# iDC-NEU/NeutronStarLite

Hardware: NVIDIA H100
Metric: gcn_aggregated_edges_per_sec (higher is better)
Workload: dtype f32

## Files before the change

include/nts_b200.h:

```cpp
#ifndef NTS_B200_H
#define NTS_B200_H

#include <stddef.h>
#include <stdint.h>

#ifdef __cplusplus
extern "C" {
#endif

typedef uint32_t nts_vid_t;

int nts_version(void);
const char *nts_last_error(void);
int nts_device_count(void);
int nts_set_device(int device);
int nts_device_sm_count(int *sm_count);
int nts_device_synchronize(void);
int nts_device_reset(void);

void *nts_malloc_device(size_t bytes);
int nts_free_device(void *ptr);
void *nts_malloc_pinned(size_t bytes);
int nts_free_pinned(void *ptr);
void *nts_pinned_device_pointer(void *host_ptr);
int nts_memcpy_h2d(void *dst_device, const void *src_host, size_t bytes, void *stream, int sync);
int nts_memcpy_d2h(void *dst_host, const void *src_device, size_t bytes, void *stream, int sync);
int nts_memcpy_d2d(void *dst_device, const void *src_device, size_t bytes, void *stream);
int nts_zero(void *device_ptr, size_t bytes, void *stream);

void *nts_stream_create(int non_blocking);
int nts_stream_destroy(void *stream);
int nts_stream_synchronize(void *stream);
void *nts_event_create(int with_timing);
int nts_event_destroy(void *event);
int nts_event_record(void *event, void *stream);
int nts_stream_wait_event(void *stream, void *event);
int nts_event_elapsed_ms(void *start, void *stop, float *ms);

int nts_segment_gather_sum(const float *input, float *output, const float *weight,
                           const nts_vid_t *indices, const nts_vid_t *offsets, nts_vid_t index_base,
                           nts_vid_t n_rows, uint64_t n_edges, nts_vid_t feature_size, void *stream);

int nts_gather_by_dst_from_src(const float *input, float *output, const float *weight_forward,
                               const nts_vid_t *row_indices, const nts_vid_t *column_offset,
                               nts_vid_t src_start, nts_vid_t src_end, nts_vid_t dst_start,
                               nts_vid_t dst_end, nts_vid_t edges, nts_vid_t batch_size,
                               nts_vid_t feature_size, int with_weight, void *stream);

int nts_gather_by_src_from_dst(const float *input, float *output, const float *weight_backward,
                               const nts_vid_t *row_offset, const nts_vid_t *column_indices,
                               nts_vid_t src_start, nts_vid_t src_end, nts_vid_t dst_start,
                               nts_vid_t dst_end, nts_vid_t edges, nts_vid_t batch_size,
                               nts_vid_t feature_size, int with_weight, void *stream);

int nts_segment_gather_sum_range(const float *input, float *output, const float *weight, const nts_vid_t *indices,
                                 const nts_vid_t *offsets, const nts_vid_t *slot_of, nts_vid_t index_base,
                                 nts_vid_t n_rows, uint64_t edge_begin, uint64_t edge_end, nts_vid_t feature_size,
                                 void *stream);

typedef struct nts_gather_plan nts_gather_plan;
int nts_gather_plan_pick_slabs(nts_vid_t gather_rows, uint64_t n_edges, nts_vid_t n_rows, nts_vid_t feature_size,
                               uint64_t l2_budget_bytes );
nts_gather_plan *nts_gather_plan_create_hybrid(const nts_vid_t *offsets, const nts_vid_t *indices,
                                               const float *weight, const nts_vid_t *slot_of, nts_vid_t index_base,
                                               nts_vid_t n_rows, uint64_t n_edges, nts_vid_t gather_rows, int n_slabs,
                                               int n_hub_cols, int n_hub_rows, void *stream);
nts_gather_plan *nts_gather_plan_create_tuned_ex(const nts_vid_t *offsets, const nts_vid_t *indices,
                                                 const float *weight, const nts_vid_t *slot_of, nts_vid_t index_base,
                                                 nts_vid_t n_rows, uint64_t n_edges, nts_vid_t gather_rows,
                                                 nts_vid_t feature_size, int gather_dtype, int run_flags,
                                                 void *stream);
typedef struct nts_plan_part {
  const nts_vid_t *offsets, *indices;
  const float *weight;
  const nts_vid_t *slot_of;
  nts_vid_t index_base, index_add, n_rows, row_add;
  uint64_t n_edges;
} nts_plan_part;
nts_gather_plan *nts_gather_plan_create_parts(const nts_plan_part *parts, int n_parts, nts_vid_t n_rows,
                                              nts_vid_t gather_rows, int n_slabs, nts_vid_t feature_size, void *stream);
float nts_gather_plan_tuned_ms(const nts_gather_plan *plan);
int nts_gather_plan_destroy(nts_gather_plan *plan);
int nts_gather_plan_slabs(const nts_gather_plan *plan);
int nts_gather_plan_hubs(const nts_gather_plan *plan, int *cols, int *rows);
int nts_gather_plan_overlap(const nts_gather_plan *plan);
int nts_gather_plan_set_overlap(nts_gather_plan *plan, int overlap);
uint64_t nts_gather_plan_bytes(const nts_gather_plan *plan);
enum { NTS_PLAN_ACCUMULATE = 0, NTS_PLAN_OVERWRITE = 1, NTS_PLAN_COPY_INPUT = 2 };
int nts_gather_plan_run_ex(nts_gather_plan *plan, const float *input, nts_vid_t input_ld, float *output,
                           nts_vid_t feature_size, int flags, void *stream);
int nts_gather_plan_last_launch(const nts_gather_plan *plan, int *launches, int *grid, int *k, int *u, int *outv);
enum { NTS_DTYPE_F32 = 0, NTS_DTYPE_BF16 = 1 };
int nts_gather_plan_run_bf16_ex(nts_gather_plan *plan, const void *input, int input_dtype, nts_vid_t input_ld,
                                float *output, nts_vid_t feature_size, int flags, void *stream);
int nts_gather_plan_set_tuning(int u, int min_blocks, int edges_per_warp);
int nts_gather_plan_set_variant(int variant);

int nts_segment_gather_sum_slots(const float *input, float *output, const float *weight,
                                 const nts_vid_t *indices, const nts_vid_t *offsets,
                                 const nts_vid_t *slot_of, nts_vid_t n_rows, uint64_t n_edges,
                                 nts_vid_t feature_size, void *stream);

int nts_segment_gather_sum_heads(const float *input, float *output, const float *weight,
                                 const nts_vid_t *indices, const nts_vid_t *offsets, const nts_vid_t *slot_of,
                                 nts_vid_t index_base, nts_vid_t n_rows, uint64_t n_edges,
                                 nts_vid_t feature_size, nts_vid_t heads, void *stream);

int nts_aggregate_set_variant(int variant, int edges_per_warp);
int nts_aggregate_last_launch(int *grid, int *block, int *smem_bytes, int *variant);
int nts_aggregate_last_shape(int *vec, int *k, int *u, int *min_blocks, int *tiles);
uint64_t nts_kernel_launch_count(void);

int nts_scatter_src_mirror_to_msg(float *message, const float *src_mirror_feature,
                                  const nts_vid_t *row_indices, const nts_vid_t *column_offset,
                                  const nts_vid_t *mirror_index, nts_vid_t batch_size,
                                  nts_vid_t feature_size, void *stream);
int nts_gather_msg_to_src_mirror(float *src_mirror_feature, const float *message,
                                 const nts_vid_t *row_indices, const nts_vid_t *column_offset,
                                 const nts_vid_t *mirror_index, nts_vid_t batch_size,
                                 nts_vid_t feature_size, void *stream);
int nts_scatter_dst_to_msg(float *message, const float *dst_feature, const nts_vid_t *row_indices,
                           const nts_vid_t *column_offset, nts_vid_t batch_size,
                           nts_vid_t feature_size, void *stream);
int nts_gather_msg_to_dst(float *dst_feature, const float *message, const nts_vid_t *row_indices,
                          const nts_vid_t *column_offset, nts_vid_t batch_size,
                          nts_vid_t feature_size, void *stream);
int nts_edge_softmax_forward(float *msg_output, const float *msg_input, float *msg_cached,
                             const nts_vid_t *row_indices, const nts_vid_t *column_offset,
                             nts_vid_t batch_size, nts_vid_t feature_size, void *stream);
int nts_edge_softmax_backward(float *msg_input_grad, const float *msg_output_grad,
                              const float *msg_cached, const nts_vid_t *row_indices,
                              const nts_vid_t *column_offset, nts_vid_t batch_size,
                              nts_vid_t feature_size, void *stream);
int nts_scatter_grad_back_to_message(const float *input, float *message_grad,
                                     const nts_vid_t *row_indices, const nts_vid_t *column_offset,
                                     nts_vid_t batch_size, nts_vid_t feature_size, void *stream);

int nts_aggregate_dst_fuse_weight_backward(float *mirror_grad, float *edge_weight_grad,
                                           const float *mirror, const float *edge_weight,
                                           const float *dst_grad, const nts_vid_t *row_indices,
                                           const nts_vid_t *column_offset,
                                           const nts_vid_t *mirror_index, nts_vid_t batch_size,
                                           nts_vid_t feature_size, void *stream);
int nts_aggregate_dst_fuse_weight_backward_heads(float *mirror_grad, float *edge_weight_grad,
                                                 const float *mirror, const float *edge_weight,
                                                 const float *dst_grad, const nts_vid_t *row_indices,
                                                 const nts_vid_t *column_offset,
                                                 const nts_vid_t *mirror_index, nts_vid_t batch_size,
                                                 nts_vid_t feature_size, nts_vid_t heads, void *stream);

int nts_gat_softmax_stats(float *seg_max, float *seg_sum, const float *src_score, const float *dst_score,
                          const nts_vid_t *row_indices, const nts_vid_t *column_offset,
                          const nts_vid_t *mirror_index, nts_vid_t batch_size, nts_vid_t heads,
                          float negative_slope, void *stream);
int nts_gat_fused_aggregate_forward(const float *mirror, float *output, const float *src_score,
                                    const float *dst_score, const float *seg_max, const float *seg_sum,
                                    const nts_vid_t *row_indices, const nts_vid_t *column_offset,
                                    const nts_vid_t *mirror_index, nts_vid_t batch_size, uint64_t n_edges,
                                    nts_vid_t feature_size, nts_vid_t heads, float negative_slope, void *stream);
int nts_gat_fused_aggregate_backward(float *mirror_grad, float *src_score_grad, float *dst_score_grad,
                                     const float *mirror, const float *src_score, const float *dst_score,
                                     const float *seg_max, const float *seg_sum, const float *out_dot_grad,
                                     const float *dst_grad, const nts_vid_t *row_indices,
                                     const nts_vid_t *column_offset, const nts_vid_t *mirror_index,
                                     nts_vid_t batch_size, nts_vid_t feature_size, nts_vid_t heads,
                                     float negative_slope, void *stream);
int nts_gat_fused_aggregate_backward_two_pass(float *mirror_grad, float *src_score_grad, float *dst_score_grad,
                                              float *dst_pack, const float *mirror, const float *src_score,
                                              const float *dst_score, const float *seg_max, const float *seg_sum,
                                              const float *out_dot_grad, const float *dst_grad,
                                              const nts_vid_t *row_indices, const nts_vid_t *column_offset,
                                              const nts_vid_t *mirror_index, const nts_vid_t *slot_row_offset,
                                              const nts_vid_t *slot_column_indices, nts_vid_t batch_size,
                                              nts_vid_t mirror_size, nts_vid_t feature_size, nts_vid_t heads,
                                              float negative_slope, void *stream);
int nts_gat_fused_aggregate_forward_bf16(const void *mirror, float *output, const float *src_score,
                                         const float *dst_score, const float *seg_max, const float *seg_sum,
                                         const nts_vid_t *row_indices, const nts_vid_t *column_offset,
                                         const nts_vid_t *mirror_index, nts_vid_t batch_size, uint64_t n_edges,
                                         nts_vid_t feature_size, nts_vid_t ld, nts_vid_t heads, float negative_slope,
                                         void *stream);
int nts_gat_fused_aggregate_backward_two_pass_bf16(float *mirror_grad, float *src_score_grad, float *dst_score_grad,
                                                   float *dst_pack, const void *mirror, const float *src_score,
                                                   const float *dst_score, const float *seg_max, const float *seg_sum,
                                                   const float *out_dot_grad, const void *dst_grad,
                                                   const nts_vid_t *row_indices, const nts_vid_t *column_offset,
                                                   const nts_vid_t *mirror_index, const nts_vid_t *slot_row_offset,
                                                   const nts_vid_t *slot_column_indices, nts_vid_t batch_size,
                                                   nts_vid_t mirror_size, nts_vid_t feature_size, nts_vid_t ld,
                                                   nts_vid_t heads, float negative_slope, void *stream);
int nts_rows_to_bf16(const void *src, int src_dtype, nts_vid_t lds, void *dst, nts_vid_t n_rows, nts_vid_t feature_size,
                     nts_vid_t ld, void *stream);

int nts_deserialize_records(float *mirror, const float *records, nts_vid_t n_records,
                            nts_vid_t feature_size, nts_vid_t partition_start,
                            nts_vid_t partition_end, void *stream);
int nts_aggregate_records(float *aggregate, const float *records, nts_vid_t n_records,
                          nts_vid_t feature_size, nts_vid_t partition_start,
                          nts_vid_t partition_end, void *stream);

int nts_gather_rows(float *dst, const float *src, const nts_vid_t *rows, nts_vid_t n_rows,
                    nts_vid_t feature_size, void *stream);
int nts_scatter_add_rows(float *dst, const float *src, const nts_vid_t *rows, nts_vid_t n_rows,
                         nts_vid_t feature_size, void *stream);
int nts_scatter_add_rows_atomic(float *dst, const float *src, const nts_vid_t *rows, nts_vid_t n_rows,
                                nts_vid_t feature_size, void *stream);

int nts_adam_update(float *W, float *M, float *V, const float *grad, uint64_t n, float weight_decay, float beta1,
                    float beta2, float alpha, float epsilon, void *stream);

#define NTS_IPC_HANDLE_BYTES 64
int nts_ipc_get_handle(void *device_ptr, unsigned char handle[NTS_IPC_HANDLE_BYTES]);
void *nts_ipc_open_handle(const unsigned char handle[NTS_IPC_HANDLE_BYTES]);
int nts_ipc_close_handle(void *peer_ptr);
int nts_signal_set(uint32_t *flag, uint32_t value, void *stream);
int nts_signal_wait_geq(const uint32_t *flag, uint32_t value, void *stream);

typedef struct nts_exchange nts_exchange;
typedef struct nts_exchange_chunk {
  const nts_vid_t *column_offset;
  const nts_vid_t *slots;
  const float *weight_forward;
  const nts_vid_t *row_offset_compact;
  const nts_vid_t *column_indices;
  const float *weight_backward;
  uint64_t edges;
} nts_exchange_chunk;
typedef struct nts_exchange_desc {
  int partitions, rank;
  nts_vid_t owned_vertices, dst_start;
  const nts_vid_t *local_column_offset, *local_row_indices, *local_row_offset, *local_column_indices;
  const float *local_weight_forward, *local_weight_backward;
  nts_vid_t local_edges;
  const nts_exchange_chunk *chunks;
  const nts_vid_t *need_count;
  const nts_vid_t *send_count;
  const nts_vid_t *send_rows_all;
  const nts_vid_t *fwd_push_offset;
  const nts_vid_t *bwd_push_offset;
  const nts_vid_t *local_need;
  nts_vid_t local_need_count;
} nts_exchange_desc;

nts_exchange *nts_exchange_create(const nts_exchange_desc *desc);
int nts_exchange_destroy(nts_exchange *ex);
uint64_t nts_exchange_required_floats(const nts_exchange *ex, nts_vid_t feature_size);
uint64_t nts_exchange_required_floats_bf16(const nts_exchange *ex, nts_vid_t feature_size);
// ... 132 lines not shown
```

neutronstarlite_b200/_lib.py:

```python
from __future__ import annotations

import ctypes as C
import os
import re

PKG = os.path.dirname(os.path.abspath(__file__))
ROOT = os.path.dirname(PKG)
LIB_PATH = os.path.join(PKG, "lib", "libnts_b200.so")
HEADER = os.path.join(ROOT, "include", "nts_b200.h")

_vp = C.c_void_p
_u32 = C.c_uint32
_u64 = C.c_uint64
_int = C.c_int
_sz = C.c_size_t

SIGNATURES = {
    "nts_version": (_int, []),
    "nts_last_error": (C.c_char_p, []),
    "nts_device_count": (_int, []),
    "nts_set_device": (_int, [_int]),
    "nts_device_sm_count": (_int, [C.POINTER(_int)]),
    "nts_device_synchronize": (_int, []),
    "nts_device_reset": (_int, []),
    "nts_malloc_device": (_vp, [_sz]),
    "nts_free_device": (_int, [_vp]),
    "nts_malloc_pinned": (_vp, [_sz]),
    "nts_free_pinned": (_int, [_vp]),
    "nts_pinned_device_pointer": (_vp, [_vp]),
    "nts_memcpy_h2d": (_int, [_vp, _vp, _sz, _vp, _int]),
    "nts_memcpy_d2h": (_int, [_vp, _vp, _sz, _vp, _int]),
    "nts_memcpy_d2d": (_int, [_vp, _vp, _sz, _vp]),
    "nts_zero": (_int, [_vp, _sz, _vp]),
    "nts_stream_create": (_vp, [_int]),
    "nts_stream_destroy": (_int, [_vp]),
    "nts_stream_synchronize": (_int, [_vp]),
    "nts_event_create": (_vp, [_int]),
    "nts_event_destroy": (_int, [_vp]),
    "nts_event_record": (_int, [_vp, _vp]),
    "nts_stream_wait_event": (_int, [_vp, _vp]),
    "nts_event_elapsed_ms": (_int, [_vp, _vp, C.POINTER(C.c_float)]),
    "nts_segment_gather_sum": (_int, [_vp, _vp, _vp, _vp, _vp, _u32, _u32, _u64, _u32, _vp]),
    "nts_gather_by_dst_from_src": (_int, [_vp, _vp, _vp, _vp, _vp, _u32, _u32, _u32, _u32, _u32, _u32, _u32, _int, _vp]),
    "nts_gather_by_src_from_dst": (_int, [_vp, _vp, _vp, _vp, _vp, _u32, _u32, _u32, _u32, _u32, _u32, _u32, _int, _vp]),
    "nts_segment_gather_sum_range": (_int, [_vp, _vp, _vp, _vp, _vp, _vp, _u32, _u32, _u64, _u64, _u32, _vp]),
    "nts_gather_plan_pick_slabs": (_int, [_u32, _u64, _u32, _u32, _u64]),
    "nts_gather_plan_create_hybrid": (_vp, [_vp, _vp, _vp, _vp, _u32, _u32, _u64, _u32, _int, _int, _int, _vp]),
    "nts_gather_plan_create_parts": (_vp, [_vp, _int, _u32, _u32, _int, _u32, _vp]),
    "nts_gather_plan_tuned_ms": (C.c_float, [_vp]),
    "nts_gather_plan_destroy": (_int, [_vp]),
    "nts_gather_plan_slabs": (_int, [_vp]),
    "nts_gather_plan_hubs": (_int, [_vp, C.POINTER(_int), C.POINTER(_int)]),
    "nts_gather_plan_overlap": (_int, [_vp]),
    "nts_gather_plan_set_overlap": (_int, [_vp, _int]),
    "nts_gather_plan_bytes": (_u64, [_vp]),
    "nts_gather_plan_run_ex": (_int, [_vp, _vp, _u32, _vp, _u32, _int, _vp]),
    "nts_gather_plan_run_bf16_ex": (_int, [_vp, _vp, _int, _u32, _vp, _u32, _int, _vp]),
    "nts_gather_plan_create_tuned_ex": (_vp, [_vp, _vp, _vp, _vp, _u32, _u32, _u64, _u32, _u32, _int, _int, _vp]),
    "nts_gather_plan_last_launch": (_int, [_vp] + [C.POINTER(_int)] * 5),
    "nts_gather_plan_set_tuning": (_int, [_int, _int, _int]),
    "nts_gather_plan_set_variant": (_int, [_int]),
    "nts_segment_gather_sum_slots": (_int, [_vp, _vp, _vp, _vp, _vp, _vp, _u32, _u64, _u32, _vp]),
    "nts_segment_gather_sum_heads": (_int, [_vp, _vp, _vp, _vp, _vp, _vp, _u32, _u32, _u64, _u32, _u32, _vp]),
    "nts_aggregate_set_variant": (_int, [_int, _int]),
    "nts_aggregate_last_launch": (_int, [C.POINTER(_int)] * 4),
    "nts_aggregate_last_shape": (_int, [C.POINTER(_int)] * 5),
    "nts_kernel_launch_count": (_u64, []),
    "nts_scatter_src_mirror_to_msg": (_int, [_vp, _vp, _vp, _vp, _vp, _u32, _u32, _vp]),
    "nts_gather_msg_to_src_mirror": (_int, [_vp, _vp, _vp, _vp, _vp, _u32, _u32, _vp]),
    "nts_scatter_dst_to_msg": (_int, [_vp, _vp, _vp, _vp, _u32, _u32, _vp]),
    "nts_gather_msg_to_dst": (_int, [_vp, _vp, _vp, _vp, _u32, _u32, _vp]),
    "nts_edge_softmax_forward": (_int, [_vp, _vp, _vp, _vp, _vp, _u32, _u32, _vp]),
    "nts_edge_softmax_backward": (_int, [_vp, _vp, _vp, _vp, _vp, _u32, _u32, _vp]),
    "nts_scatter_grad_back_to_message": (_int, [_vp, _vp, _vp, _vp, _u32, _u32, _vp]),
    "nts_aggregate_dst_fuse_weight_backward": (_int, [_vp, _vp, _vp, _vp, _vp, _vp, _vp, _vp, _u32, _u32, _vp]),
    "nts_aggregate_dst_fuse_weight_backward_heads": (_int, [_vp] * 8 + [_u32, _u32, _u32, _vp]),
    "nts_gat_softmax_stats": (_int, [_vp] * 7 + [_u32, _u32, C.c_float, _vp]),
    "nts_gat_fused_aggregate_forward": (_int, [_vp] * 9 + [_u32, _u64, _u32, _u32, C.c_float, _vp]),
    "nts_gat_fused_aggregate_backward": (_int, [_vp] * 13 + [_u32, _u32, _u32, C.c_float, _vp]),
    "nts_gat_fused_aggregate_backward_two_pass": (_int, [_vp] * 16 + [_u32, _u32, _u32, _u32, C.c_float, _vp]),
    "nts_gat_fused_aggregate_forward_bf16": (_int, [_vp] * 9 + [_u32, _u64, _u32, _u32, _u32, C.c_float, _vp]),
    "nts_gat_fused_aggregate_backward_two_pass_bf16": (_int, [_vp] * 16 + [_u32] * 5 + [C.c_float, _vp]),
    "nts_rows_to_bf16": (_int, [_vp, _int, _u32, _vp, _u32, _u32, _u32, _vp]),
    "nts_deserialize_records": (_int, [_vp, _vp, _u32, _u32, _u32, _u32, _vp]),
    "nts_aggregate_records": (_int, [_vp, _vp, _u32, _u32, _u32, _u32, _vp]),
    "nts_gather_rows": (_int, [_vp, _vp, _vp, _u32, _u32, _vp]),
    "nts_scatter_add_rows": (_int, [_vp, _vp, _vp, _u32, _u32, _vp]),
    "nts_scatter_add_rows_atomic": (_int, [_vp, _vp, _vp, _u32, _u32, _vp]),
    "nts_ipc_get_handle": (_int, [_vp, C.c_char_p]),
    "nts_ipc_open_handle": (_vp, [C.c_char_p]),
    "nts_ipc_close_handle": (_int, [_vp]),
    "nts_adam_update": (_int, [_vp, _vp, _vp, _vp, _u64] + [C.c_float] * 5 + [_vp]),
    "nts_signal_set": (_int, [_vp, _u32, _vp]),
    "nts_signal_wait_geq": (_int, [_vp, _u32, _vp]),
    "nts_host_degrees": (_int, [_vp, _u64, _u32, _vp, _vp]),
    "nts_host_partition_offsets": (_int, [_vp, _u64, _u32, _int, _vp]),
    "nts_host_chunk_edge_counts": (_int, [_vp, _u64, _vp, _int, _int, _vp]),
    "nts_host_build_chunk": (_int, [_vp, _u64, _u32, _vp, _int, _int, _int, _vp, _vp, _vp, _vp, _vp, _vp, _vp, _vp, _vp]),
    "nts_host_mirror_index": (_int, [_vp, _u64, _u32, _vp, _int, _vp, _vp]),
    "nts_host_read_feature_label_mask": (_int, [C.c_char_p, C.c_char_p, C.c_char_p, _u32, _u32, _u32, _vp, _vp, _vp]),
    "nts_host_read_feature_binary": (_int, [C.c_char_p, _u32, _u32, _u32, _vp]),
    "nts_graph_build_from_file": (_vp, [C.c_char_p, _u32, _int, _int, _vp, _u64, _int, _vp]),
    "nts_graph_build_from_device": (_vp, [_vp, _vp, _int, _u64, _u32, _int, _int, _vp, _vp, _vp, _int, _vp]),
    "nts_graph_build_info": (_int, [_vp] * 6),
    "nts_graph_build_export_chunk": (_int, [_vp, _int] + [_vp] * 8),
    "nts_graph_build_export_dist": (_int, [_vp] * 5),
    "nts_graph_build_export_degrees": (_int, [_vp] * 4),
    "nts_graph_build_destroy": (_int, [_vp]),
}



class ExchangeChunk(C.Structure):
    _fields_ = [
        ("column_offset", _vp), ("slots", _vp), ("weight_forward", _vp), ("row_offset_compact", _vp),
        ("column_indices", _vp), ("weight_backward", _vp), ("edges", _u64),
    ]


class ExchangeDesc(C.Structure):
    _fields_ = [
        ("partitions", _int), ("rank", _int), ("owned_vertices", _u32), ("dst_start", _u32),
        ("local_column_offset", _vp), ("local_row_indices", _vp), ("local_row_offset", _vp),
        ("local_column_indices", _vp), ("local_weight_forward", _vp), ("local_weight_backward", _vp),
        ("local_edges", _u32),
        ("chunks", C.POINTER(ExchangeChunk)),
        ("need_count", C.POINTER(_u32)), ("send_count", C.POINTER(_u32)),
        ("send_rows_all", _vp), ("fwd_push_offset", C.POINTER(_u32)), ("bwd_push_offset", C.POINTER(_u32)),
        ("local_need", _vp), ("local_need_count", _u32),
    ]


class DeviceChunk(C.Structure):
    _fields_ = [
        ("column_offset", _vp), ("row_indices", _vp), ("row_offset", _vp), ("column_indices", _vp),
        ("edge_weight_forward", _vp), ("edge_weight_backward", _vp),
    ]


SIGNATURES.update({
    "nts_exchange_create": (_vp, [C.POINTER(ExchangeDesc)]),
    "nts_exchange_destroy": (_int, [_vp]),
    "nts_exchange_required_floats": (_u64, [_vp, _u32]),
    "nts_exchange_capacity_floats": (_u64, [_vp]),
    "nts_exchange_release_peers": (_int, [_vp]),
    "nts_exchange_reserve": (_int, [_vp, _u64, _int]),
    "nts_exchange_handles": (_int, [_vp, C.c_char_p, C.c_char_p]),
    "nts_exchange_open_peers": (_int, [_vp, C.c_char_p, C.c_char_p]),
    "nts_exchange_forward": (_int, [_vp, _vp, _vp, _u32, _vp]),
    "nts_exchange_backward": (_int, [_vp, _vp, _vp, _u32, _vp]),
    "nts_exchange_forward_bf16": (_int, [_vp, _vp, _int, _vp, _u32, _vp]),
    "nts_exchange_backward_bf16": (_int, [_vp, _vp, _vp, _u32, _vp]),
    "nts_exchange_required_floats_bf16": (_u64, [_vp, _u32]),
    "nts_exchange_set_trace": (_int, [_vp, _int]),
    "nts_exchange_last_timeline": (_int, [_vp, C.POINTER(C.c_float), _int]),
    "nts_exchange_fetch_mirrors": (_int, [_vp, _vp, _vp, _u32, _vp]),
    "nts_exchange_return_mirror_grads": (_int, [_vp, _vp, _vp, _u32, _vp]),
})



class HostChunk(C.Structure):
    _fields_ = [
        ("column_offset", _vp), ("row_indices", _vp), ("row_offset", _vp), ("column_indices", _vp),
        ("edge_weight_forward", _vp), ("edge_weight_backward", _vp),
        ("src_start", _u32), ("src_end", _u32), ("dst_start", _u32), ("dst_end", _u32), ("edges", _u64),
    ]


class ExchangePlanView(C.Structure):
    _fields_ = [
        ("partitions", _int), ("rank", _int),
        ("owned_vertices", _u32), ("recv_total", _u32), ("send_total", _u32), ("backward_rows", _u32),
        ("remote_edges", _u64),
        ("need_count", C.POINTER(_u32)), ("send_count", C.POINTER(_u32)), ("peer_bwd_offset", C.POINTER(_u32)),
        ("fwd_push_offset", C.POINTER(_u32)), ("bwd_push_offset", C.POINTER(_u32)),
        ("remote_column_offset", C.POINTER(_u32)), ("remote_slots", C.POINTER(_u32)),
        ("remote_weight", C.POINTER(C.c_float)),
        ("backward_offsets", C.POINTER(_u32)), ("backward_indices", C.POINTER(_u32)),
        ("backward_weight", C.POINTER(C.c_float)),
        ("send_rows_all", C.POINTER(_u32)),
    ]


SIGNATURES.update({
    "nts_exchange_plan_create": (_vp, [C.POINTER(HostChunk), _int, _int]),
    "nts_exchange_plan_destroy": (None, [_vp]),
    "nts_exchange_plan_need": (C.POINTER(_u32), [_vp, _int, C.POINTER(_u32)]),
    "nts_exchange_plan_packed_rows": (_u64, [_vp]),
    "nts_exchange_plan_pack_needs": (_int, [_vp, _vp, _vp]),
    "nts_exchange_plan_set_peer_needs": (_int, [_vp, _int, _vp, _vp]),
    "nts_exchange_plan_finalize": (_int, [_vp]),
    "nts_exchange_plan_get_view": (_int, [_vp, C.POINTER(ExchangePlanView)]),
    "nts_exchange_plan_chunk": (_int, [_vp, _int, C.POINTER(C.POINTER(_u32)), C.POINTER(C.POINTER(_u32))]),
    "nts_exchange_create_from_plan": (_vp, [_vp, C.POINTER(DeviceChunk)]),
})


class SampleHopView(C.Structure):
    _fields_ = [
        ("n_dst", _u32), ("n_src", _u32), ("n_edges", _u64),
        ("dst", _vp), ("column_offset", _vp), ("row_indices", _vp), ("row_global", _vp), ("weight", _vp),
        ("src", _vp), ("row_offset", _vp), ("column_indices", _vp), ("weight_backward", _vp),
    ]


SIGNATURES.update({
    "nts_sampler_create": (_vp, [_vp, _vp, _vp, _u32, _u64, _u32, _int, C.POINTER(_int), _vp]),
    "nts_sampler_create_ex": (_vp, [_vp, _vp, _vp, _u32, _u64, _u32, _int, C.POINTER(_int), _u32, _vp]),
    "nts_sampler_sample": (_int, [_vp, _vp, _u32, _u64, _u64, _vp]),
# ... 46 lines not shown
```

neutronstarlite_b200/csrc/nts_common.cuh:

```cuda
#pragma once
#include <cuda_bf16.h>
#include <cuda_runtime.h>
#include <stdint.h>
#include <stdio.h>
#include <stdlib.h>
#include <string.h>

#include <functional>

#include "nts_b200.h"

namespace nts {

char *last_error_buffer();
bool abort_on_error();
void count_launch();

inline int fail(int code, const char *what, const char *file, int line) {
  snprintf(last_error_buffer(), 512, "%s (%s:%d)", what, file, line);
  if (abort_on_error()) {
    fprintf(stderr, "libnts_b200: %s\n", last_error_buffer());
    exit(1);
  }
  return code;
}

#define NTS_CUDA_OK(expr)                                                                         \
  do {                                                                                            \
    cudaError_t nts_e_ = (expr);                                                                  \
    if (nts_e_ != cudaSuccess)                                                                    \
      return ::nts::fail((int)nts_e_, cudaGetErrorString(nts_e_), __FILE__, __LINE__);            \
  } while (0)

#define NTS_ARG_CHECK(cond, msg)                                                                  \
  do {                                                                                            \
    if (!(cond))                                                                                  \
      return ::nts::fail(-1, msg, __FILE__, __LINE__);                                            \
  } while (0)

#define NTS_LAUNCH_CHECK()                                                                        \
  do {                                                                                            \
    ::nts::count_launch();                                                                        \
    NTS_CUDA_OK(cudaGetLastError());                                                              \
  } while (0)

inline cudaStream_t as_stream(void *s) { return reinterpret_cast<cudaStream_t>(s); }

inline bool aligned_to(const void *p, size_t a) { return (reinterpret_cast<uintptr_t>(p) & (a - 1)) == 0; }

int sm_count();

int time_min_of_two(const std::function<int()> &run, cudaStream_t st, float *ms);

int run_plan(nts_gather_plan *pl, const float *input, uint32_t lds, float *output, uint32_t F, int flags,
             cudaStream_t st);
int run_plan_bf16(nts_gather_plan *pl, const void *input, int dtype, uint32_t lds, float *output, uint32_t F,
                  cudaStream_t st, int flags = 0);
int to_bf16_rows(const void *src, int dtype, uint32_t lds, void *dst, uint32_t n_rows, uint32_t F, uint32_t ld,
                 cudaStream_t st);

int check_gat_bf16_layout(uint32_t F, uint32_t ld, uint32_t heads);

struct __align__(16) float8v {
  float4 lo, hi;
};

template <int VEC> struct Vec;
template <> struct Vec<1> { using type = float; };
template <> struct Vec<2> { using type = float2; };
template <> struct Vec<4> { using type = float4; };
template <> struct Vec<8> { using type = float8v; };

template <class T, int VEC> struct Ld { using type = typename Vec<VEC>::type; };
template <> struct Ld<__nv_bfloat16, 2> { using type = uint32_t; };
template <> struct Ld<__nv_bfloat16, 4> { using type = uint2; };
template <> struct Ld<__nv_bfloat16, 8> { using type = uint4; };
__device__ __forceinline__ float widen(float v) { return v; }
__device__ __forceinline__ float2 widen(float2 v) { return v; }
__device__ __forceinline__ float4 widen(float4 v) { return v; }
__device__ __forceinline__ float2 widen(uint32_t u) {
  return make_float2(__uint_as_float(u << 16), __uint_as_float(u & 0xffff0000u));
}
__device__ __forceinline__ float4 widen(uint2 u) {
  const float2 a = widen(u.x), b = widen(u.y);
  return make_float4(a.x, a.y, b.x, b.y);
}
__device__ __forceinline__ float8v widen(uint4 u) { return {widen(make_uint2(u.x, u.y)), widen(make_uint2(u.z, u.w))}; }

nts_gather_plan *tune_plan(const nts_plan_part *parts, int n_parts, nts_vid_t n_rows, nts_vid_t gather_rows,
                           nts_vid_t feature_size, bool bf16, int run_flags, bool hubs_allowed, cudaStream_t st);

}
```

neutronstarlite_b200/csrc/nts_exchange.cu:

```cuda
#include <algorithm>
#include <vector>

#include "nts_common.cuh"

namespace nts {
constexpr int kMaxPeers = 32;

struct PushTarget {
  const uint32_t *rows;
  uint32_t n_rows, src_row0;
  float *dst;
  uint32_t *pushed_flag;
  const uint32_t *consumed_flag;
};
struct PushArgs {
  PushTarget t[kMaxPeers];
  int n;
  uint32_t epoch, wait_epoch;
};
}

struct nts_exchange {
  int P = 1, p = 0;
  nts_exchange_desc d;
// ... 173 lines not shown

#define NTS_TRY(expr)                                                                                               \
  do {                                                                                                              \
    int nts_rc_ = (expr);                                                                                           \
    if (nts_rc_ != 0)                                                                                               \
      return nts_rc_;                                                                                               \
  } while (0)

static int grow(float **buf, size_t *cap, size_t floats) {
  if (floats <= *cap)
    return 0;
  if (*buf)
    NTS_CUDA_OK(cudaFree(*buf));
  *buf = nullptr;
  NTS_CUDA_OK(cudaMalloc(reinterpret_cast<void **>(buf), floats * sizeof(float)));
  *cap = floats;
  return 0;
}

static int check_wait_error(nts_exchange *ex, int rc) {
  if (ex->err_host && ex->err_host[0]) {
    char msg[256];
    snprintf(msg, sizeof(msg),
             "exchange wait timed out on rank %d: %s %d (wanted epoch %d, saw %d) - a peer died, failed or fell out of step",
             ex->p, ex->err_host[0] == 1 ? "no rows pushed by partition" : "window not consumed by push target",
             ex->err_host[1], ex->err_host[2], ex->err_host[3]);
    return fail(rc ? rc : -1, msg, __FILE__, __LINE__);
  }
  return rc;
}

static int launch_push(nts_exchange *ex, const PushArgs &a, const float *src, uint32_t F, cudaStream_t st) {
  int vec = 1;
  bool a16 = aligned_to(src, 16), a8 = aligned_to(src, 8);
  for (int k = 0; k < a.n; k++) {
    a16 = a16 && aligned_to(a.t[k].dst, 16);
    a8 = a8 && aligned_to(a.t[k].dst, 8);
  }
  if (F % 4 == 0 && a16)
    vec = 4;
  else if (F % 2 == 0 && a8)
    vec = 2;
  const int ctas = ex->push_ctas;
  if (vec == 4)
    push_rows_kernel<4><<<ctas, 256, 0, st>>>(a, src, F, ex->tickets, ex->timeout_ns, ex->err_dev);
  else if (vec == 2)
    push_rows_kernel<2><<<ctas, 256, 0, st>>>(a, src, F, ex->tickets, ex->timeout_ns, ex->err_dev);
  else
    push_rows_kernel<1><<<ctas, 256, 0, st>>>(a, src, F, ex->tickets, ex->timeout_ns, ex->err_dev);
  NTS_LAUNCH_CHECK();
  return 0;
}

static int dma_push(nts_exchange *ex, int j, const float *src, size_t dst_row, uint32_t n_rows, uint32_t F, size_t buf,
                    uint32_t epoch, uint32_t wait_epoch, cudaStream_t from) {
  cudaStream_t st = ex->dma[j];
  NTS_CUDA_OK(cudaEventRecord(ex->ev_dma[j], from));
  NTS_CUDA_OK(cudaStreamWaitEvent(st, ex->ev_dma[j], 0));
  ex->dma_used[j] = 1;
  if (n_rows) {
    if (wait_epoch) {
      wait_consumed_kernel<<<1, 1, 0, st>>>(ex->flags + ex->P + j, wait_epoch, ex->timeout_ns, ex->err_dev, j);
      NTS_LAUNCH_CHECK();
    }
    NTS_CUDA_OK(cudaMemcpyAsync(ex->peer_window[j] + buf + dst_row * F, src, (size_t)n_rows * F * sizeof(float),
                                cudaMemcpyDeviceToDevice, st));
  }
  signal_pushed_kernel<<<1, 1, 0, st>>>(ex->peer_flags[j] + ex->p, epoch);
  NTS_LAUNCH_CHECK();
  return 0;
}

static int dma_join(nts_exchange *ex, cudaStream_t into) {
  for (int j = 0; j < ex->P; j++)
    if (ex->dma_used[j]) {
      NTS_CUDA_OK(cudaEventRecord(ex->ev_dma[j], ex->dma[j]));
      NTS_CUDA_OK(cudaStreamWaitEvent(into, ex->ev_dma[j], 0));
      ex->dma_used[j] = 0;
    }
  return 0;
}

static int push_my_rows(nts_exchange *ex, const float *x, uint32_t F, size_t buf, uint32_t epoch, uint32_t wait_epoch) {
  const int P = ex->P, p = ex->p;
  PushArgs a;
  a.n = 0;
  a.epoch = epoch;
  a.wait_epoch = wait_epoch;
  for (int s = 1; s < P; s++) {
    const int j = (p - s + P) % P;
    if (ex->send_all[j]) {
      if (a.n) {
        NTS_TRY(launch_push(ex, a, x, F, ex->comm));
        a.n = 0;
      }
      NTS_TRY(dma_push(ex, j, x, ex->fwd_push_off[j], ex->send_count[j], F, buf, epoch, wait_epoch, ex->comm));
      continue;
    }
    PushTarget &t = a.t[a.n++];
    t.rows = ex->d.send_rows_all + ex->srecv_offs[j];
    t.n_rows = ex->send_count[j];
    t.src_row0 = 0;
    t.dst = ex->peer_window[j] + buf + (size_t)ex->fwd_push_off[j] * F;
    t.pushed_flag = ex->peer_flags[j] + p;
    t.consumed_flag = ex->flags + P + j;
  }
  if (a.n)
    NTS_TRY(launch_push(ex, a, x, F, ex->comm));
  return 0;
}

struct GatherType {
  bool bf16;
  uint32_t ld;
};
static int plan_key(uint32_t F, bool bf16) { return bf16 ? -(int)F : (int)F; }

static int aggregate_chunk(nts_exchange *ex, int i, bool forward, const void *in_rows, float *out, uint32_t F,
                           cudaStream_t st, GatherType gt = {false, 0}) {
  const float *in = static_cast<const float *>(in_rows);
  const nts_exchange_chunk &c = ex->chunks[i];
  const bool local = i == ex->p;
  const uint32_t n_rows = (forward || local) ? ex->d.owned_vertices : ex->need_count[i];
  const uint32_t gather_rows = (forward && !local) ? ex->need_count[i] : ex->d.owned_vertices;
  if (!c.edges || !n_rows)
    return 0;
  const nts_vid_t *off = forward ? c.column_offset : c.row_offset_compact;
  const nts_vid_t *idx = forward ? c.slots : c.column_indices;
  const float *w = forward ? c.weight_forward : c.weight_backward;
  const uint32_t base = (forward && !local) ? 0u : ex->d.dst_start;
  if (c.edges >= ex->plan_min_edges || gt.bf16) {
    std::vector<std::pair<int, nts_gather_plan *>> &plans = (forward ? ex->plan_fwd : ex->plan_bwd)[i];
    nts_gather_plan *pl = nullptr;
    for (auto &e : plans)
      if (e.first == plan_key(F, gt.bf16))
        pl = e.second;
    if (!pl) {
      const nts_plan_part pt = {off, idx, w, nullptr, base, 0, n_rows, 0, c.edges};
      pl = tune_plan(&pt, 1, n_rows, gather_rows, F, gt.bf16, 0, true, st);
      if (!pl)
        return -1;
      int hc = 0, hr = 0, ehc = 0, ehr = 0;
      nts_gather_plan_hubs(pl, &hc, &hr);
      for (auto &e : plans)
        if (nts_gather_plan_slabs(e.second) == nts_gather_plan_slabs(pl) &&
            nts_gather_plan_hubs(e.second, &ehc, &ehr) == 0 && ehc == hc && ehr == hr) {
          nts_gather_plan_destroy(pl);
          pl = e.second;
          break;
        }
      plans.emplace_back(plan_key(F, gt.bf16), pl);
    }
    if (gt.bf16)
      return run_plan_bf16(pl, in_rows, NTS_DTYPE_BF16, gt.ld, out, F, st);
    return run_plan(pl, in, F, out, F, 0, st);
  }
  return nts_segment_gather_sum(in, out, w, idx, off, base, n_rows, c.edges, F, st);
}

static int decide_mode(nts_exchange *ex, bool forward, uint32_t F, cudaStream_t st, nts_exchange::Mode **out,
                       GatherType gt = {false, 0}) {
  std::vector<nts_exchange::Mode> &modes = forward ? ex->mode_fwd : ex->mode_bwd;
  for (auto &m : modes)
    if (m.F == (int)F && m.bf16 == gt.bf16) {
      *out = &m;
      return 0;
    }
  modes.push_back({(int)F, 1, gt.bf16, nullptr, 0.f, 0.f});
  nts_exchange::Mode &m = modes.back();
  *out = &m;
  const int P = ex->P, p = ex->p;
  const uint32_t Vp = ex->d.owned_vertices;
  uint64_t remote_edges = 0;
  int n_remote = 0;
  for (int i = 0; i < P; i++)
    if (i != p && ex->chunks[i].edges && ex->need_count[i]) {
      remote_edges += ex->chunks[i].edges;
      n_remote++;
    }
  if (ex->forced_mode == 1 || n_remote < 2 || !Vp || !ex->recv_total)
    return 0;
  std::vector<nts_plan_part> parts;
  for (int i = 0; i < P; i++) {
    if (i == p || !ex->chunks[i].edges || !ex->need_count[i])
      continue;
    const nts_exchange_chunk &c = ex->chunks[i];
    nts_plan_part pt = {};
    if (forward) {
      pt.offsets = c.column_offset, pt.indices = c.slots, pt.weight = c.weight_forward;
      pt.index_base = 0, pt.index_add = ex->recv_offs[i], pt.n_rows = Vp, pt.row_add = 0;
    } else {
      pt.offsets = c.row_offset_compact, pt.indices = c.column_indices, pt.weight = c.weight_backward;
      pt.index_base = ex->d.dst_start, pt.index_add = 0, pt.n_rows = ex->need_count[i], pt.row_add = ex->recv_offs[i];
    }
    pt.n_edges = c.edges;
    parts.push_back(pt);
  }
  const uint32_t out_rows = forward ? Vp : ex->recv_total, in_rows = forward ? ex->recv_total : Vp;
  m.merged = tune_plan(parts.data(), (int)parts.size(), out_rows, in_rows, F, gt.bf16, 0, false, st);
  if (!m.merged)
    return -1;
  if (ex->forced_mode == 2) {
    m.mode = 2;
    return 0;
  }
  const size_t rows_max = std::max<size_t>(ex->recv_total, Vp);
  const size_t a_bytes = rows_max * std::max<size_t>((size_t)F * sizeof(float), gt.bf16 ? (size_t)gt.ld * 2 : 0);
  float *a = nullptr, *b = nullptr;
  NTS_CUDA_OK(cudaMalloc(reinterpret_cast<void **>(&a), a_bytes));
  if (cudaMalloc(reinterpret_cast<void **>(&b), rows_max * F * sizeof(float)) != cudaSuccess) {
    cudaFree(a);
    return fail(-1, "scratch allocation for the exchange mode measurement failed", __FILE__, __LINE__);
  }
  cudaMemsetAsync(a, 0, a_bytes, st);
  cudaMemsetAsync(b, 0, rows_max * F * sizeof(float), st);
  float L = 0.f, M = 0.f, sum_c = 0.f;
  int rc = time_min_of_two([&]() { return aggregate_chunk(ex, p, forward, a, b, F, st, gt); }, st, &L);
  if (!rc)
    rc = time_min_of_two([&]() {
      return gt.bf16 ? run_plan_bf16(m.merged, a, NTS_DTYPE_BF16, gt.ld, b, F, st) : run_plan(m.merged, a, F, b, F, 0, st);
    }, st, &M);
  for (int i = 0; i < P && !rc; i++) {
    if (i == p || !ex->chunks[i].edges || !ex->need_count[i])
      continue;
    float c = 0.f;
    rc = time_min_of_two([&]() { return aggregate_chunk(ex, i, forward, a, b, F, st, gt); }, st, &c);
    sum_c += c;
  }
  cudaFree(a);
  cudaFree(b);
  if (rc)
    return rc;
  if (!ex->chunks[p].edges)
    L = 0.f;
  const double row_bytes = (forward && gt.bf16) ? gt.ld * 2.0 : F * 4.0;
  const float T = (float)((double)ex->recv_total * row_bytes / 300e9 * 1e3);
  if (forward) {
    m.pipeline_ms = L + std::max(sum_c, T - L);
    m.merged_ms = std::max(L, T) + M;
  } else {
    m.pipeline_ms = sum_c + std::max(L, T / (float)(P - 1));
    m.merged_ms = M + std::max(L, T);
  }
  m.mode = m.merged_ms < m.pipeline_ms ? 2 : 1;
  if (m.mode == 1) {
    nts_gather_plan_destroy(m.merged);
    m.merged = nullptr;
  }
  return 0;
}

extern "C" {

nts_exchange *nts_exchange_create(const nts_exchange_desc *desc) {
  if (!desc || desc->partitions < 1 || desc->partitions > kMaxPeers || desc->rank < 0 ||
      desc->rank >= desc->partitions) {
    fail(-1, "bad exchange descriptor (1 <= partitions <= 32)", __FILE__, __LINE__);
    return nullptr;
  }
  nts_exchange *ex = new nts_exchange();
  ex->d = *desc;
  const int P = ex->P = desc->partitions, p = ex->p = desc->rank;
  if (P > 1 && !(desc->chunks && desc->need_count && desc->send_count && desc->fwd_push_offset &&
                 desc->bwd_push_offset)) {
    fail(-1, "exchange descriptor lacks the per-partition arrays", __FILE__, __LINE__);
    delete ex;
    return nullptr;
  }
  ex->need_count.assign(P, 0), ex->send_count.assign(P, 0), ex->fwd_push_off.assign(P, 0), ex->bwd_push_off.assign(P, 0);
  ex->chunks.assign(P, nts_exchange_chunk{});
  for (int i = 0; i < P && P > 1; i++) {
    if (i == p)
      continue;
    ex->need_count[i] = desc->need_count[i];
    ex->send_count[i] = desc->send_count[i];
    ex->fwd_push_off[i] = desc->fwd_push_offset[i];
    ex->bwd_push_off[i] = desc->bwd_push_offset[i];
    ex->chunks[i] = desc->chunks[i];
  }
  {
    nts_exchange_chunk &c = ex->chunks[p];
    c.column_offset = desc->local_column_offset;
    c.slots = desc->local_row_indices;
    c.weight_forward = desc->local_weight_forward;
    c.row_offset_compact = desc->local_row_offset;
    c.column_indices = desc->local_column_indices;
    c.weight_backward = desc->local_weight_backward;
    c.edges = desc->local_edges;
  }
  ex->recv_offs.assign(P + 1, 0), ex->srecv_offs.assign(P + 1, 0);
  for (int i = 0; i < P; i++) {
    ex->recv_offs[i + 1] = ex->recv_offs[i] + ex->need_count[i];
    ex->srecv_offs[i + 1] = ex->srecv_offs[i] + ex->send_count[i];
  }
  ex->recv_total = ex->recv_offs[P];
  ex->send_total = ex->srecv_offs[P];
  ex->send_all.assign(P, 0);
  if (P > 1 && ex->send_total && desc->send_rows_all && !getenv("NTS_EXCHANGE_NO_DMA")) {
    std::vector<uint32_t> rows(ex->send_total);
    if (cudaMemcpy(rows.data(), desc->send_rows_all, rows.size() * sizeof(uint32_t), cudaMemcpyDeviceToHost) == cudaSuccess)
      for (int j = 0; j < P; j++) {
        if (j == p || ex->send_count[j] != desc->owned_vertices || !desc->owned_vertices)
          continue;
        bool ident = true;
        const uint32_t *r = rows.data() + ex->srecv_offs[j];
        for (uint32_t k = 0; k < ex->send_count[j] && ident; k++)
          ident = r[k] == k;
        ex->send_all[j] = ident;
      }
  }
  ex->peer_window.assign(P, nullptr);
  ex->peer_flags.assign(P, nullptr);
  ex->plan_fwd.resize(P), ex->plan_bwd.resize(P);
  ex->ev_peer.assign(P, nullptr);
  if (const char *t = getenv("NTS_EXCHANGE_TIMEOUT_MS")) {
    const long ms = atol(t);
    if (ms > 0)
      ex->timeout_ns = (unsigned long long)ms * 1000000ull;
  }
  if (const char *t = getenv("NTS_EXCHANGE_MODE"))
    ex->forced_mode = !strcmp(t, "pipeline") ? 1 : (!strcmp(t, "merged") ? 2 : 0);
  if (const char *t = getenv("NTS_EXCHANGE_PLAN_MIN_EDGES"))
    ex->plan_min_edges = strtoull(t, nullptr, 10);
  ex->push_ctas = std::max(8, sm_count() / 2);
  if (const char *t = getenv("NTS_EXCHANGE_PUSH_CTAS")) {
    const int n = atoi(t);
    if (n > 0)
      ex->push_ctas = n;
  }
  int lo = 0, hi = 0;
  bool ok = cudaDeviceGetStreamPriorityRange(&lo, &hi) == cudaSuccess &&
            cudaMalloc(reinterpret_cast<void **>(&ex->flags), sizeof(uint32_t) * 2 * P) == cudaSuccess &&
            cudaMemset(ex->flags, 0, sizeof(uint32_t) * 2 * P) == cudaSuccess &&
            cudaMalloc(reinterpret_cast<void **>(&ex->tickets), sizeof(uint32_t) * kMaxPeers) == cudaSuccess &&
            cudaMemset(ex->tickets, 0, sizeof(uint32_t) * kMaxPeers) == cudaSuccess &&
            cudaMalloc(reinterpret_cast<void **>(&ex->d_peer_flags), sizeof(uint32_t *) * P) == cudaSuccess &&
            cudaHostAlloc(reinterpret_cast<void **>(&ex->err_host), 4 * sizeof(int), cudaHostAllocMapped) == cudaSuccess &&
            cudaHostGetDevicePointer(reinterpret_cast<void **>(&ex->err_dev), ex->err_host, 0) == cudaSuccess &&
            cudaStreamCreateWithPriority(&ex->comm, cudaStreamNonBlocking, hi) == cudaSuccess &&
            cudaEventCreateWithFlags(&ex->ev_main, cudaEventDisableTiming) == cudaSuccess &&
            cudaEventCreateWithFlags(&ex->ev_comm, cudaEventDisableTiming) == cudaSuccess;
  for (int i = 0; i < P && ok; i++)
    ok = cudaEventCreateWithFlags(&ex->ev_peer[i], cudaEventDisableTiming) == cudaSuccess;
  ex->dma.assign(P, nullptr), ex->ev_dma.assign(P, nullptr), ex->dma_used.assign(P, 0);
  for (int i = 0; i < P && ok && P > 1; i++)
    ok = cudaStreamCreateWithPriority(&ex->dma[i], cudaStreamNonBlocking, hi) == cudaSuccess &&
         cudaEventCreateWithFlags(&ex->ev_dma[i], cudaEventDisableTiming) == cudaSuccess;
  if (ok) {
    memset(ex->err_host, 0, 4 * sizeof(int));
    ok = cudaDeviceSynchronize() == cudaSuccess;
  }
  if (!ok) {
    fail(-1, "exchange resource allocation failed", __FILE__, __LINE__);
    delete ex;
    return nullptr;
  }
  return ex;
}

int nts_exchange_release_peers(nts_exchange *ex) {
  NTS_ARG_CHECK(ex != nullptr, "null engine");
  NTS_CUDA_OK(cudaDeviceSynchronize());
  if (ex->peers_open) {
    for (int j = 0; j < ex->P; j++)
      if (j != ex->p) {
        NTS_CUDA_OK(cudaIpcCloseMemHandle(ex->peer_window[j]));
        NTS_CUDA_OK(cudaIpcCloseMemHandle(ex->peer_flags[j]));
      }
    ex->peers_open = false;
  }
  return 0;
}

// ... 32 lines not shown
  if (ex->ev_main)
    cudaEventDestroy(ex->ev_main);
  if (ex->ev_comm)
    cudaEventDestroy(ex->ev_comm);
  for (cudaEvent_t e : ex->ev_peer)
    if (e)
      cudaEventDestroy(e);
  for (cudaEvent_t e : ex->tev)
    if (e)
      cudaEventDestroy(e);
  for (cudaStream_t q : ex->dma)
    if (q)
      cudaStreamDestroy(q);
  for (cudaEvent_t e : ex->ev_dma)
    if (e)
      cudaEventDestroy(e);
  delete ex;
  return 0;
}

uint64_t nts_exchange_required_floats(const nts_exchange *ex, nts_vid_t feature_size) {
  uint64_t rows = std::max(ex->recv_total, ex->send_total);
  if (rows == 0)
    rows = 1;
  return rows * (uint64_t)feature_size;
}

uint64_t nts_exchange_required_floats_bf16(const nts_exchange *ex, nts_vid_t feature_size) {
  const uint64_t row16 = ((feature_size + 7ull) / 8ull) * 4ull;
  return std::max<uint64_t>(std::max<uint64_t>(ex->recv_total, 1) * row16, nts_exchange_required_floats(ex, feature_size));
}

uint64_t nts_exchange_capacity_floats(const nts_exchange *ex) { return ex ? ex->buf_floats : 0; }

int nts_exchange_reserve(nts_exchange *ex, uint64_t floats_per_buffer, int n_buffers) {
  NTS_ARG_CHECK(ex && (n_buffers == 1 || n_buffers == 2), "bad argument (n_buffers must be 1 or 2)");
  NTS_ARG_CHECK(!ex->peers_open, "nts_exchange_release_peers (and a barrier) must precede nts_exchange_reserve");
  NTS_CUDA_OK(cudaDeviceSynchronize());
  if (ex->window)
    NTS_CUDA_OK(cudaFree(ex->window));
  ex->window = nullptr;
  ex->buf_floats = 0;
  NTS_CUDA_OK(cudaMalloc(reinterpret_cast<void **>(&ex->window), floats_per_buffer * n_buffers * sizeof(float)));
  ex->buf_floats = floats_per_buffer;
  ex->n_buffers = n_buffers;
  return 0;
}

int nts_exchange_handles(nts_exchange *ex, unsigned char window_handle[NTS_IPC_HANDLE_BYTES],
                         unsigned char flags_handle[NTS_IPC_HANDLE_BYTES]) {
  NTS_ARG_CHECK(ex && ex->window && ex->flags, "window not allocated");
  cudaIpcMemHandle_t h;
  NTS_CUDA_OK(cudaIpcGetMemHandle(&h, ex->window));
  memcpy(window_handle, &h, sizeof(h));
  NTS_CUDA_OK(cudaIpcGetMemHandle(&h, ex->flags));
  memcpy(flags_handle, &h, sizeof(h));
  return 0;
}

int nts_exchange_open_peers(nts_exchange *ex, const unsigned char *window_handles, const unsigned char *flag_handles) {
  NTS_ARG_CHECK(ex && window_handles && flag_handles, "null argument");
  NTS_ARG_CHECK(!ex->peers_open, "peers already open");
  const int P = ex->P, p = ex->p;
  for (int j = 0; j < P; j++) {
    if (j == p) {
      ex->peer_window[j] = ex->window;
      ex->peer_flags[j] = ex->flags;
      continue;
    }
    cudaIpcMemHandle_t h;
    void *ptr = nullptr;
    memcpy(&h, window_handles + (size_t)j * NTS_IPC_HANDLE_BYTES, sizeof(h));
    NTS_CUDA_OK(cudaIpcOpenMemHandle(&ptr, h, cudaIpcMemLazyEnablePeerAccess));
    ex->peer_window[j] = static_cast<float *>(ptr);
    memcpy(&h, flag_handles + (size_t)j * NTS_IPC_HANDLE_BYTES, sizeof(h));
    NTS_CUDA_OK(cudaIpcOpenMemHandle(&ptr, h, cudaIpcMemLazyEnablePeerAccess));
    ex->peer_flags[j] = static_cast<uint32_t *>(ptr);
  }
  NTS_CUDA_OK(cudaMemcpy(ex->d_peer_flags, ex->peer_flags.data(), sizeof(uint32_t *) * P, cudaMemcpyHostToDevice));
  ex->peers_open = true;
  return 0;
}

static int ready_for(nts_exchange *ex, nts_vid_t F, bool bf16 = false) {
  NTS_ARG_CHECK(ex->peers_open && ex->n_buffers >= 1 &&
                    (bf16 ? nts_exchange_required_floats_bf16(ex, F) : nts_exchange_required_floats(ex, F)) <=
                        ex->buf_floats,
                "exchange window not reserved / peers not opened for this feature width");
  return 0;
}

static int stage_bf16(nts_exchange *ex, const void *src, int dtype, uint32_t F, GatherType gt, cudaStream_t st,
                      const void **rows) {
  const uint32_t n = ex->d.owned_vertices;
  if (dtype == NTS_DTYPE_BF16 && gt.ld == F && aligned_to(src, 16)) {
    *rows = src;
    return 0;
  }
  NTS_TRY(grow(&ex->stage16, &ex->stage16_cap, (size_t)(n ? n : 1) * (gt.ld / 2)));
  NTS_TRY(to_bf16_rows(src, dtype, F, ex->stage16, n, F, gt.ld, st));
  *rows = ex->stage16;
  return 0;
}

static int forward_impl(nts_exchange *ex, const void *x_in, int x_dtype, float *y, nts_vid_t F, void *stream,
                        bool bf16 = false) {
  const nts_exchange_desc &d = ex->d;
  const float *x = static_cast<const float *>(x_in);
  NTS_ARG_CHECK(d.owned_vertices == 0 || (x && y), "null feature pointer");
  cudaStream_t st = as_stream(stream);
  const int P = ex->P, p = ex->p;
  NTS_ARG_CHECK(!bf16 || P > 1, "BF16 gathers on one partition run through nts_gather_plan_run_bf16_ex");
  if (P == 1)
    return nts_gather_by_dst_from_src(x, y, d.local_weight_forward, d.local_row_indices, d.local_column_offset,
                                      d.dst_start, d.dst_start + d.owned_vertices, d.dst_start,
                                      d.dst_start + d.owned_vertices, d.local_edges, d.owned_vertices, F, 1, stream);
  NTS_TRY(ready_for(ex, F, bf16));
  const GatherType gt = {bf16, bf16 ? ((F + 7u) & ~7u) : F};
  const uint32_t Fw = bf16 ? gt.ld / 2 : F;
  if (bf16 && d.owned_vertices) {
    const void *rows = nullptr;
    NTS_TRY(stage_bf16(ex, x_in, x_dtype, F, gt, st, &rows));
    x = static_cast<const float *>(rows);
  }
  const uint32_t epoch = ++ex->epoch;
  const size_t buf = (size_t)(epoch % ex->n_buffers) * ex->buf_floats;
  const uint32_t wait_epoch = epoch > (uint32_t)ex->n_buffers ? epoch - ex->n_buffers : 0u;
  const bool tr = ex->trace && (int)ex->tev.size() >= 4 + 2 * (P - 1);
  NTS_CUDA_OK(cudaEventRecord(ex->ev_main, st));
  if (tr)
    NTS_CUDA_OK(cudaEventRecord(ex->tev[0], st));
  NTS_CUDA_OK(cudaStreamWaitEvent(ex->comm, ex->ev_main, 0));
  if (tr)
    NTS_CUDA_OK(cudaEventRecord(ex->tev[1], ex->comm));
  NTS_TRY(push_my_rows(ex, x, Fw, buf, epoch, wait_epoch));
  NTS_TRY(dma_join(ex, ex->comm));
  if (tr)
    NTS_CUDA_OK(cudaEventRecord(ex->tev[2], ex->comm));
  nts_exchange::Mode *mode = nullptr;
  NTS_TRY(decide_mode(ex, true, F, st, &mode, gt));
  NTS_TRY(aggregate_chunk(ex, p, true, x, y, F, st, gt));
  if (tr)
    NTS_CUDA_OK(cudaEventRecord(ex->tev[3], st));
  if (mode->mode == 2) {
    uint32_t mask = 0;
    for (int j = 0; j < P; j++)
      if (j != p)
        mask |= 1u << j;
    wait_pushed_kernel<<<1, 32, 0, st>>>(ex->flags, mask, epoch, ex->timeout_ns, ex->err_dev);
    NTS_LAUNCH_CHECK();
    if (tr)
      NTS_CUDA_OK(cudaEventRecord(ex->tev[4], st));
    if (bf16)
      NTS_TRY(run_plan_bf16(mode->merged, ex->window + buf, NTS_DTYPE_BF16, gt.ld, y, F, st));
    else
      NTS_TRY(run_plan(mode->merged, ex->window + buf, F, y, F, 0, st));
    if (tr)
      for (int s = 1; s < P; s++) {
        NTS_CUDA_OK(cudaEventRecord(ex->tev[5 + 2 * (s - 1)], st));
        if (s + 1 < P)
          NTS_CUDA_OK(cudaEventRecord(ex->tev[4 + 2 * s], st));
      }
  } else {
    for (int s = 1; s < P; s++) {
      const int i = (p + s) % P;
      wait_pushed_kernel<<<1, 32, 0, st>>>(ex->flags, 1u << i, epoch, ex->timeout_ns, ex->err_dev);
      NTS_LAUNCH_CHECK();
      if (tr)
        NTS_CUDA_OK(cudaEventRecord(ex->tev[4 + 2 * (s - 1)], st));
      if (ex->need_count[i])
        NTS_TRY(aggregate_chunk(ex, i, true, ex->window + buf + (size_t)ex->recv_offs[i] * Fw, y, F, st, gt));
      if (tr)
        NTS_CUDA_OK(cudaEventRecord(ex->tev[5 + 2 * (s - 1)], st));
    }
  }
  signal_consumed_kernel<<<1, 32, 0, st>>>(ex->d_peer_flags, P, p, epoch);
  NTS_LAUNCH_CHECK();
  NTS_CUDA_OK(cudaEventRecord(ex->ev_comm, ex->comm));
  NTS_CUDA_OK(cudaStreamWaitEvent(st, ex->ev_comm, 0));
  return 0;
}

static int backward_impl(nts_exchange *ex, const float *g, float *dx, nts_vid_t F, void *stream, bool bf16 = false) {
  const nts_exchange_desc &d = ex->d;
  NTS_ARG_CHECK(d.owned_vertices == 0 || (g && dx), "null gradient pointer");
  cudaStream_t st = as_stream(stream);
  const int P = ex->P, p = ex->p;
  NTS_ARG_CHECK(!bf16 || P > 1, "BF16 gathers on one partition run through nts_gather_plan_run_bf16_ex");
  if (P == 1)
    return nts_gather_by_src_from_dst(g, dx, d.local_weight_backward, d.local_row_offset, d.local_column_indices,
                                      d.dst_start, d.dst_start + d.owned_vertices, d.dst_start,
                                      d.dst_start + d.owned_vertices, d.local_edges, d.owned_vertices, F, 1, stream);
  NTS_TRY(ready_for(ex, F, bf16));
  const GatherType gt = {bf16, bf16 ? ((F + 7u) & ~7u) : F};
  const void *gin = g;
  if (bf16 && d.owned_vertices)
    NTS_TRY(stage_bf16(ex, g, NTS_DTYPE_F32, F, gt, st, &gin));
  const uint32_t epoch = ++ex->epoch;
  const size_t buf = (size_t)(epoch % ex->n_buffers) * ex->buf_floats;
  const uint32_t wait_epoch = epoch > (uint32_t)ex->n_buffers ? epoch - ex->n_buffers : 0u;
  NTS_TRY(grow(&ex->bsend, &ex->bsend_cap, (size_t)(ex->recv_total ? ex->recv_total : 1) * F));
  if (ex->recv_total)
    NTS_CUDA_OK(cudaMemsetAsync(ex->bsend, 0, (size_t)ex->recv_total * F * sizeof(float), st));
  nts_exchange::Mode *mode = nullptr;
  NTS_TRY(decide_mode(ex, false, F, st, &mode, gt));
  if (mode->mode == 2) {
    if (bf16)
      NTS_TRY(run_plan_bf16(mode->merged, gin, NTS_DTYPE_BF16, gt.ld, ex->bsend, F, st));
    else
      NTS_TRY(run_plan(mode->merged, g, F, ex->bsend, F, 0, st));
    NTS_CUDA_OK(cudaEventRecord(ex->ev_peer[p], st));
    NTS_CUDA_OK(cudaStreamWaitEvent(ex->comm, ex->ev_peer[p], 0));
    for (int s = 1; s < P; s++) {
      const int i = (p + s) % P;
      NTS_TRY(dma_push(ex, i, ex->bsend + (size_t)ex->recv_offs[i] * F, ex->bwd_push_off[i], ex->need_count[i], F, buf,
                       epoch, wait_epoch, ex->comm));
    }
  } else {
    for (int s = 1; s < P; s++) {
      const int i = (p + s) % P;
      float *slice = ex->bsend + (size_t)ex->recv_offs[i] * F;
      if (ex->need_count[i])
        NTS_TRY(aggregate_chunk(ex, i, false, gin, slice, F, st, gt));
      NTS_CUDA_OK(cudaEventRecord(ex->ev_peer[i], st));
      NTS_CUDA_OK(cudaStreamWaitEvent(ex->comm, ex->ev_peer[i], 0));
      NTS_TRY(dma_push(ex, i, ex->bsend + (size_t)ex->recv_offs[i] * F, ex->bwd_push_off[i], ex->need_count[i], F, buf,
                       epoch, wait_epoch, ex->comm));
    }
  }
  NTS_TRY(aggregate_chunk(ex, p, false, gin, dx, F, st, gt));
  uint32_t mask = 0;
  for (int j = 0; j < P; j++)
    if (j != p)
      mask |= 1u << j;
  wait_pushed_kernel<<<1, 32, 0, st>>>(ex->flags, mask, epoch, ex->timeout_ns, ex->err_dev);
  NTS_LAUNCH_CHECK();
  if (ex->send_total)
    NTS_TRY(nts_scatter_add_rows_atomic(dx, ex->window + buf, d.send_rows_all, ex->send_total, F, st));
  signal_consumed_kernel<<<1, 32, 0, st>>>(ex->d_peer_flags, P, p, epoch);
  NTS_LAUNCH_CHECK();
  NTS_TRY(dma_join(ex, ex->comm));
  NTS_CUDA_OK(cudaEventRecord(ex->ev_comm, ex->comm));
  NTS_CUDA_OK(cudaStreamWaitEvent(st, ex->ev_comm, 0));
  return 0;
}

static int fetch_impl(nts_exchange *ex, const float *x, float *mirror, nts_vid_t F, void *stream) {
  const nts_exchange_desc &d = ex->d;
  cudaStream_t st = as_stream(stream);
  const int P = ex->P, p = ex->p;
  const uint32_t own = d.local_need_count;
  NTS_ARG_CHECK(own == 0 || d.local_need, "exchange descriptor lacks local_need (rows of this partition it reads itself)");
  if (P == 1)
    return own ? nts_gather_rows(mirror, x, d.local_need, own, F, stream) : 0;
  NTS_TRY(ready_for(ex, F));
  const uint32_t epoch = ++ex->epoch;
  const size_t buf = (size_t)(epoch % ex->n_buffers) * ex->buf_floats;
  const uint32_t wait_epoch = epoch > (uint32_t)ex->n_buffers ? epoch - ex->n_buffers : 0u;
  NTS_CUDA_OK(cudaEventRecord(ex->ev_main, st));
  NTS_CUDA_OK(cudaStreamWaitEvent(ex->comm, ex->ev_main, 0));
  NTS_TRY(push_my_rows(ex, x, F, buf, epoch, wait_epoch));
  NTS_TRY(dma_join(ex, ex->comm));
  const size_t before = ex->recv_offs[p];
  if (own)
    NTS_TRY(nts_gather_rows(mirror + before * F, x, d.local_need, own, F, st));
  uint32_t mask = 0;
  for (int j = 0; j < P; j++)
    if (j != p)
      mask |= 1u << j;
  wait_pushed_kernel<<<1, 32, 0, st>>>(ex->flags, mask, epoch, ex->timeout_ns, ex->err_dev);
  NTS_LAUNCH_CHECK();
  if (before)
    NTS_CUDA_OK(cudaMemcpyAsync(mirror, ex->window + buf, before * F * sizeof(float), cudaMemcpyDeviceToDevice, st));
  if (ex->recv_total > before)
    NTS_CUDA_OK(cudaMemcpyAsync(mirror + (before + own) * F, ex->window + buf + before * F,
                                (ex->recv_total - before) * (size_t)F * sizeof(float), cudaMemcpyDeviceToDevice, st));
  signal_consumed_kernel<<<1, 32, 0, st>>>(ex->d_peer_flags, P, p, epoch);
  NTS_LAUNCH_CHECK();
  NTS_CUDA_OK(cudaEventRecord(ex->ev_comm, ex->comm));
  NTS_CUDA_OK(cudaStreamWaitEvent(st, ex->ev_comm, 0));
  return 0;
}

static int return_impl(nts_exchange *ex, const float *gm, float *dx, nts_vid_t F, void *stream) {
  const nts_exchange_desc &d = ex->d;
  cudaStream_t st = as_stream(stream);
  const int P = ex->P, p = ex->p;
  const uint32_t own = d.local_need_count;
  NTS_ARG_CHECK(own == 0 || d.local_need, "exchange descriptor lacks local_need");
  if (P == 1)
    return own ? nts_scatter_add_rows(dx, gm, d.local_need, own, F, stream) : 0;
  NTS_TRY(ready_for(ex, F));
  const uint32_t epoch = ++ex->epoch;
  const size_t buf = (size_t)(epoch % ex->n_buffers) * ex->buf_floats;
  const size_t before = ex->recv_offs[p];
  const uint32_t wait_epoch = epoch > (uint32_t)ex->n_buffers ? epoch - ex->n_buffers : 0u;
  NTS_CUDA_OK(cudaEventRecord(ex->ev_main, st));
  NTS_CUDA_OK(cudaStreamWaitEvent(ex->comm, ex->ev_main, 0));
  for (int s = 1; s < P; s++) {
    const int i = (p + s) % P;
    NTS_TRY(dma_push(ex, i, gm + (size_t)(ex->recv_offs[i] + (i > p ? own : 0u)) * F, ex->bwd_push_off[i],
                     ex->need_count[i], F, buf, epoch, wait_epoch, ex->comm));
  }
  if (own)
    NTS_TRY(nts_scatter_add_rows(dx, gm + before * F, d.local_need, own, F, st));
  uint32_t mask = 0;
  for (int j = 0; j < P; j++)
    if (j != p)
      mask |= 1u << j;
  wait_pushed_kernel<<<1, 32, 0, st>>>(ex->flags, mask, epoch, ex->timeout_ns, ex->err_dev);
  NTS_LAUNCH_CHECK();
  if (ex->send_total)
    NTS_TRY(nts_scatter_add_rows_atomic(dx, ex->window + buf, d.send_rows_all, ex->send_total, F, st));
  signal_consumed_kernel<<<1, 32, 0, st>>>(ex->d_peer_flags, P, p, epoch);
  NTS_LAUNCH_CHECK();
  NTS_TRY(dma_join(ex, ex->comm));
  NTS_CUDA_OK(cudaEventRecord(ex->ev_comm, ex->comm));
  NTS_CUDA_OK(cudaStreamWaitEvent(st, ex->ev_comm, 0));
  return 0;
}

int nts_exchange_set_trace(nts_exchange *ex, int enable) {
  NTS_ARG_CHECK(ex != nullptr, "null engine");
  if (enable && ex->tev.empty()) {
    ex->tev.assign(4 + 2 * (ex->P > 1 ? ex->P - 1 : 0), nullptr);
    for (cudaEvent_t &e : ex->tev)
      NTS_CUDA_OK(cudaEventCreate(&e));
  }
  ex->trace = enable != 0;
  return 0;
}

int nts_exchange_last_timeline(nts_exchange *ex, float *ms, int capacity) {
  NTS_ARG_CHECK(ex && ms && ex->trace && !ex->tev.empty(), "tracing is not enabled");
  const int P = ex->P, n = 2 * P + 1;
  NTS_ARG_CHECK(capacity >= n, "timeline buffer too small (2P+1 floats)");
  NTS_CUDA_OK(cudaDeviceSynchronize());
  NTS_CUDA_OK(cudaEventElapsedTime(&ms[0], ex->tev[1], ex->tev[2]));
  NTS_CUDA_OK(cudaEventElapsedTime(&ms[1], ex->tev[0], ex->tev[3]));
  cudaEvent_t prev = ex->tev[3];
  for (int s = 1; s < P; s++) {
    NTS_CUDA_OK(cudaEventElapsedTime(&ms[2 * s], prev, ex->tev[4 + 2 * (s - 1)]));
    NTS_CUDA_OK(cudaEventElapsedTime(&ms[2 * s + 1], ex->tev[4 + 2 * (s - 1)], ex->tev[5 + 2 * (s - 1)]));
    prev = ex->tev[5 + 2 * (s - 1)];
  }
  NTS_CUDA_OK(cudaEventElapsedTime(&ms[2 * P], ex->tev[0], prev));
  return 0;
}

int nts_exchange_fetch_mirrors(nts_exchange *ex, const float *x, float *mirror, nts_vid_t F, void *stream) {
  NTS_ARG_CHECK(ex && (x || ex->d.owned_vertices == 0) && (mirror || ex->recv_total + ex->d.local_need_count == 0),
                "null argument");
  return check_wait_error(ex, fetch_impl(ex, x, mirror, F, stream));
}

int nts_exchange_return_mirror_grads(nts_exchange *ex, const float *mirror_grad, float *dx, nts_vid_t F, void *stream) {
  NTS_ARG_CHECK(ex && (mirror_grad || ex->recv_total + ex->d.local_need_count == 0) &&
                    (dx || ex->d.owned_vertices == 0),
                "null argument");
  return check_wait_error(ex, return_impl(ex, mirror_grad, dx, F, stream));
}

int nts_exchange_forward(nts_exchange *ex, const float *x, float *y, nts_vid_t F, void *stream) {
// ... 22 lines not shown
```

neutronstarlite_b200/csrc/nts_plan.cu:

```cuda
#include <cub/cub.cuh>
#include <cuda_bf16.h>

#include <algorithm>
#include <type_traits>
#include <vector>

#include "nts_common.cuh"

struct nts_gather_plan {
  uint32_t n_rows = 0;
  uint64_t n_edges = 0;
  uint32_t gather_rows = 0;
  int slabs = 1;
  uint32_t slab_rows = 0;
  uint2 *pairs = nullptr;
  uint32_t *voff = nullptr;
  std::vector<uint64_t> slab_edge;
  float *workspace = nullptr;
  size_t workspace_floats = 0;
  __nv_bfloat16 *workspace_bf16 = nullptr;
  size_t workspace_bf16_elems = 0;
  int hub_cols = 0, hub_rows = 0;
  uint32_t *hub_col_ids = nullptr;
  uint32_t *hub_row_ids = nullptr;
// ... 104 lines not shown
    for (int o = 16; o > 0; o >>= 1)
      s += __shfl_xor_sync(0xffffffffu, s, o);
    if (lane == 0)
      dense[__ldg(cell_key + run) - n_keys] = s;
  }
}

__global__ void pad_rows_kernel(const float *__restrict__ src, uint32_t lds, float *__restrict__ dst, uint32_t n_rows,
                                uint32_t F, uint32_t ld) {
  const uint64_t total = (uint64_t)n_rows * ld;
  for (uint64_t i = (uint64_t)blockIdx.x * blockDim.x + threadIdx.x; i < total; i += (uint64_t)gridDim.x * blockDim.x) {
    const uint64_t r = i / ld;
    const uint32_t c = (uint32_t)(i - r * ld);
    dst[i] = c < F ? __ldg(src + r * lds + c) : 0.f;
  }
}

template <class S>
__global__ void bf16_rows_kernel(const S *__restrict__ src, uint32_t lds, uint4 *__restrict__ dst, uint32_t n_rows,
                                 uint32_t F, uint32_t ld) {
  const uint32_t ld8 = ld / 8;
  const uint64_t total = (uint64_t)n_rows * ld8;
  for (uint64_t i = (uint64_t)blockIdx.x * blockDim.x + threadIdx.x; i < total; i += (uint64_t)gridDim.x * blockDim.x) {
    const uint64_t r = i / ld8;
    const uint32_t c = (uint32_t)(i - r * ld8) * 8;
    const S *s = src + r * lds;
    uint32_t w[4];
#pragma unroll
    for (int j = 0; j < 4; j++) {
      const uint32_t c0 = c + 2 * j, c1 = c0 + 1;
      if constexpr (std::is_same<S, float>::value) {
        const __nv_bfloat162 h = __floats2bfloat162_rn(c0 < F ? __ldg(s + c0) : 0.f, c1 < F ? __ldg(s + c1) : 0.f);
        w[j] = *reinterpret_cast<const uint32_t *>(&h);
      } else {
        const uint16_t *u = reinterpret_cast<const uint16_t *>(s);
        w[j] = (c0 < F ? (uint32_t)__ldg(u + c0) : 0u) | ((c1 < F ? (uint32_t)__ldg(u + c1) : 0u) << 16);
      }
    }
    dst[i] = make_uint4(w[0], w[1], w[2], w[3]);
  }
}

__device__ __forceinline__ uint32_t p_smem_u32(const void *p) { return (uint32_t)__cvta_generic_to_shared(p); }
__device__ __forceinline__ void p_mbar_init(uint64_t *bar, uint32_t count) {
  asm volatile("mbarrier.init.shared::cta.b64 [%0], %1;" ::"r"(p_smem_u32(bar)), "r"(count));
}
__device__ __forceinline__ void p_mbar_expect_tx(uint64_t *bar, uint32_t bytes) {
  asm volatile("mbarrier.arrive.expect_tx.shared::cta.b64 _, [%0], %1;" ::"r"(p_smem_u32(bar)), "r"(bytes) : "memory");
}
__device__ __forceinline__ void p_mbar_wait(uint64_t *bar, uint32_t parity) {
  asm volatile("{\n\t"
               ".reg .pred p;\n\t"
               "WAIT_%=:\n\t"
               "mbarrier.try_wait.parity.shared::cta.b64 p, [%0], %1;\n\t"
               "@p bra DONE_%=;\n\t"
               "bra WAIT_%=;\n\t"
               "DONE_%=:\n\t"
               "}" ::"r"(p_smem_u32(bar)),
               "r"(parity)
               : "memory");
}
__device__ __forceinline__ void p_bulk_g2s(void *smem_dst, const void *gmem_src, uint32_t bytes, uint64_t *bar) {
  asm volatile("cp.async.bulk.shared::cluster.global.mbarrier::complete_tx::bytes [%0], [%1], %2, [%3];" ::"r"(
                   p_smem_u32(smem_dst)),
               "l"(gmem_src), "r"(bytes), "r"(p_smem_u32(bar))
               : "memory");
}

constexpr int kPlanWarps = 8;

template <int OUTV, bool ATOMIC>
__device__ __forceinline__ void flush_chunk(float *__restrict__ orow, uint32_t col, uint32_t F, float4 a) {
  if constexpr (OUTV == 4) {
    float4 *p = reinterpret_cast<float4 *>(orow + col);
    if constexpr (ATOMIC) {
      asm volatile("red.global.add.v4.f32 [%0], {%1, %2, %3, %4};" ::"l"(p), "f"(a.x), "f"(a.y), "f"(a.z), "f"(a.w)
                   : "memory");
    } else {
      float4 o = *p;
      o.x += a.x, o.y += a.y, o.z += a.z, o.w += a.w;
      *p = o;
    }
  } else if constexpr (OUTV == 2) {
    float2 *p = reinterpret_cast<float2 *>(orow + col);
    if constexpr (ATOMIC) {
      asm volatile("red.global.add.v2.f32 [%0], {%1, %2};" ::"l"(p), "f"(a.x), "f"(a.y) : "memory");
      if (col + 2 < F)
        asm volatile("red.global.add.v2.f32 [%0], {%1, %2};" ::"l"(p + 1), "f"(a.z), "f"(a.w) : "memory");
    } else {
      float2 o = p[0];
      o.x += a.x, o.y += a.y;
      p[0] = o;
      if (col + 2 < F) {
        float2 o1 = p[1];
        o1.x += a.z, o1.y += a.w;
        p[1] = o1;
      }
    }
  } else {
    const float v[4] = {a.x, a.y, a.z, a.w};
#pragma unroll
    for (int i = 0; i < 4; i++)
      if (col + i < F) {
        if constexpr (ATOMIC)
          atomicAdd(orow + col + i, v[i]);
        else
          orow[col + i] += v[i];
      }
  }
}

template <int OUTV>
__device__ __forceinline__ void store_chunk(float *__restrict__ orow, uint32_t col, uint32_t F, float4 a) {
  if constexpr (OUTV == 4) {
    *reinterpret_cast<float4 *>(orow + col) = a;
  } else if constexpr (OUTV == 2) {
    float2 *p = reinterpret_cast<float2 *>(orow + col);
    p[0] = make_float2(a.x, a.y);
    if (col + 2 < F)
      p[1] = make_float2(a.z, a.w);
  } else {
    const float v[4] = {a.x, a.y, a.z, a.w};
#pragma unroll
    for (int i = 0; i < 4; i++)
      if (col + i < F)
        orow[col + i] = v[i];
  }
}

template <class T> struct GatherT;
template <> struct GatherT<float> {
  using chunk = float4;
  static constexpr int V = 4;
  __device__ static __forceinline__ void widen(const float4 &c, float (&v)[4]) {
    v[0] = c.x, v[1] = c.y, v[2] = c.z, v[3] = c.w;
  }
};
template <> struct GatherT<__nv_bfloat16> {
  using chunk = uint4;
  static constexpr int V = 8;
  __device__ static __forceinline__ void widen(const uint4 &c, float (&v)[8]) {
    const uint32_t u[4] = {c.x, c.y, c.z, c.w};
#pragma unroll
    for (int i = 0; i < 4; i++) {
      v[2 * i] = __uint_as_float(u[i] << 16);
      v[2 * i + 1] = __uint_as_float(u[i] & 0xffff0000u);
    }
  }
};

template <class T, int K, int U, int OUTV, int G>
__device__ __forceinline__ void planned_gather_body(unsigned char *smem_raw, uint32_t vblock,
                                                    const typename GatherT<T>::chunk *__restrict__ in, uint32_t ldc,
                                                    float *__restrict__ out, uint32_t F,
                                                    const uint2 *__restrict__ pairs, const uint32_t *__restrict__ off,
                                                    uint32_t n_rows, uint32_t e_begin, uint32_t e_end, uint32_t Q,
                                                    uint32_t tiles, uint32_t tile_vecs) {
  static_assert(G == 1 || K == 1, "virtual warps are for rows narrower than a warp");
  using Chunk = typename GatherT<T>::chunk;
  constexpr int V = GatherT<T>::V;
  constexpr uint32_t GS = 32 / G;
  const uint32_t lane = threadIdx.x & (GS - 1);
  const uint32_t vwarp_in_block = threadIdx.x / GS;
  const uint64_t gwarp = (uint64_t)vblock * (kPlanWarps * G) + vwarp_in_block;
  const uint32_t tile = (uint32_t)(gwarp % tiles);
  const uint64_t q = gwarp / tiles;
  const uint64_t e0_64 = e_begin + q * (uint64_t)Q;

  uint64_t *bar = reinterpret_cast<uint64_t *>(smem_raw);
  uint2 *s_pair = reinterpret_cast<uint2 *>(smem_raw + 16);
  uint32_t cta_e_base = 0, bulk_bytes = 0;
  {
    const uint64_t cta_w0 = (uint64_t)vblock * (kPlanWarps * G);
    const uint64_t first_q = cta_w0 / tiles;
    const uint64_t last_q = (cta_w0 + kPlanWarps * G - 1) / tiles;
    uint64_t ce0 = e_begin + first_q * (uint64_t)Q;
    uint64_t ce1 = e_begin + (last_q + 1) * (uint64_t)Q;
    if (ce1 > e_end)
      ce1 = e_end;
    if (ce0 < ce1) {
      cta_e_base = (uint32_t)(ce0 & ~1ull);
      const uint32_t n_el = (uint32_t)(ce1 - cta_e_base);
      bulk_bytes = (n_el * 8u) & ~15u;
      if (threadIdx.x == 0) {
        p_mbar_init(bar, 1);
        asm volatile("fence.mbarrier_init.release.cluster;" ::: "memory");
        if (n_el & 1u)
          s_pair[n_el - 1] = __ldg(pairs + cta_e_base + n_el - 1);
      }
      __syncthreads();
      if (threadIdx.x == 0 && bulk_bytes) {
        p_mbar_expect_tx(bar, bulk_bytes);
        p_bulk_g2s(s_pair, pairs + cta_e_base, bulk_bytes, bar);
      }
    }
  }
  if (e0_64 >= e_end)
    return;
  const uint32_t e0 = (uint32_t)e0_64;
  const uint32_t e1 = (e0_64 + Q < e_end) ? e0 + Q : e_end;

  const uint32_t c0 = tile * tile_vecs + lane;
  bool act[K];
#pragma unroll
  for (int k = 0; k < K; k++)
    act[k] = (k * GS + lane) < tile_vecs && (c0 + k * GS) < ldc;

  uint32_t row = plan_find_row(off, n_rows, e0);
  uint32_t row_end = __ldg(off + row + 1);
  bool row_started_inside = __ldg(off + row) >= e0;

  float acc[K][V];
#pragma unroll
  for (int k = 0; k < K; k++)
#pragma unroll
    for (int j = 0; j < V; j++)
      acc[k][j] = 0.f;

  auto flush = [&](bool whole) {
    float *orow = out + (size_t)row * F;
#pragma unroll
    for (int k = 0; k < K; k++) {
#pragma unroll
      for (int h = 0; h < V; h += 4) {
        const uint32_t col = (c0 + k * GS) * V + h;
        const float4 a = make_float4(acc[k][h], acc[k][h + 1], acc[k][h + 2], acc[k][h + 3]);
        if (act[k] && col < F) {
          if (whole)
            flush_chunk<OUTV, false>(orow, col, F, a);
          else
            flush_chunk<OUTV, true>(orow, col, F, a);
        }
      }
#pragma unroll
      for (int j = 0; j < V; j++)
        acc[k][j] = 0.f;
    }
  };
  auto advance = [&](uint32_t ee) {
    flush(row_started_inside);
    do {
      row++;
      row_end = __ldg(off + row + 1);
    } while (ee >= row_end);
    row_started_inside = true;
  };

  if (bulk_bytes)
    p_mbar_wait(bar, 0);

  const uint2 *sp = s_pair - cta_e_base;
  uint32_t e = e0;
  auto fma_chunk = [&](int k, float w, const Chunk &c) {
    float x[V];
    GatherT<T>::widen(c, x);
#pragma unroll
    for (int j = 0; j < V; j++)
      acc[k][j] = fmaf(w, x[j], acc[k][j]);
  };
  for (; e + U <= e1; e += U) {
    Chunk v[U][K];
    float wu[U];
#pragma unroll
    for (int u = 0; u < U; u++) {
      const uint2 pr = sp[e + u];
      wu[u] = __uint_as_float(pr.y);
      const Chunk *p = in + (size_t)pr.x * ldc + c0;
#pragma unroll
      for (int k = 0; k < K; k++)
        if (act[k])
          v[u][k] = __ldg(p + k * GS);
    }
#pragma unroll
    for (int u = 0; u < U; u++) {
      if (e + u >= row_end)
        advance(e + u);
#pragma unroll
      for (int k = 0; k < K; k++)
        if (act[k])
          fma_chunk(k, wu[u], v[u][k]);
    }
  }
  for (; e < e1; e++) {
    const uint2 pr = sp[e];
    const float wj = __uint_as_float(pr.y);
    const Chunk *p = in + (size_t)pr.x * ldc + c0;
    Chunk v1[K];
#pragma unroll
    for (int k = 0; k < K; k++)
      if (act[k])
        v1[k] = __ldg(p + k * GS);
    if (e >= row_end)
      advance(e);
#pragma unroll
    for (int k = 0; k < K; k++)
      if (act[k])
        fma_chunk(k, wj, v1[k]);
  }
  flush(row_started_inside && row_end <= e1);
}

template <class T, int K, int U, int OUTV, int MINB, int G = 1>
__global__ void __launch_bounds__(kPlanWarps * 32, MINB)
    planned_gather_sum_kernel(const typename GatherT<T>::chunk *__restrict__ in, uint32_t ldc, float *__restrict__ out,
                              uint32_t F, const uint2 *__restrict__ pairs, const uint32_t *__restrict__ off,
                              uint32_t n_rows, uint32_t e_begin, uint32_t e_end, uint32_t Q, uint32_t tiles,
                              uint32_t tile_vecs) {
  extern __shared__ __align__(16) unsigned char smem_raw[];
  planned_gather_body<T, K, U, OUTV, G>(smem_raw, blockIdx.x, in, ldc, out, F, pairs, off, n_rows, e_begin, e_end, Q,
                                        tiles, tile_vecs);
}

struct PlanShape;
template <int K, int STAGES, int OUTV, int MINB>
__global__ void __launch_bounds__(kPlanWarps * 32, MINB)
    planned_gather_sum_tma_kernel(const float4 *__restrict__ in, uint32_t ld4, float *__restrict__ out, uint32_t F,
                                  const uint2 *__restrict__ pairs, const uint32_t *__restrict__ off, uint32_t n_rows,
                                  uint32_t e_begin, uint32_t e_end, uint32_t Q, uint32_t tiles, uint32_t tile_vecs,
                                  uint32_t pair_bytes) {
  const uint32_t lane = threadIdx.x & 31;
  const uint32_t warp_in_block = threadIdx.x >> 5;
  const uint64_t gwarp = (uint64_t)blockIdx.x * kPlanWarps + warp_in_block;
  const uint32_t tile = (uint32_t)(gwarp % tiles);
  const uint64_t q = gwarp / tiles;
  const uint64_t e0_64 = e_begin + q * (uint64_t)Q;

  extern __shared__ __align__(16) unsigned char smem_raw[];
  uint64_t *bar = reinterpret_cast<uint64_t *>(smem_raw);
  uint2 *s_pair = reinterpret_cast<uint2 *>(smem_raw + 16);
  const uint32_t ring_bytes = 8u * STAGES + 8u * (STAGES & 1) + STAGES * tile_vecs * 16u;
  unsigned char *ring = smem_raw + 16 + pair_bytes + (size_t)warp_in_block * ring_bytes;
  uint64_t *sbar = reinterpret_cast<uint64_t *>(ring);
  float4 *sbuf = reinterpret_cast<float4 *>(ring + 8u * STAGES + 8u * (STAGES & 1));
  uint32_t cta_e_base = 0, bulk_bytes = 0;
  {
    const uint64_t cta_w0 = (uint64_t)blockIdx.x * kPlanWarps;
    const uint64_t first_q = cta_w0 / tiles;
    const uint64_t last_q = (cta_w0 + kPlanWarps - 1) / tiles;
    uint64_t ce0 = e_begin + first_q * (uint64_t)Q;
    uint64_t ce1 = e_begin + (last_q + 1) * (uint64_t)Q;
    if (ce1 > e_end)
      ce1 = e_end;
    if (lane == 0)
      for (int s = 0; s < STAGES; s++)
        p_mbar_init(sbar + s, 1);
    if (ce0 < ce1) {
      cta_e_base = (uint32_t)(ce0 & ~1ull);
      const uint32_t n_el = (uint32_t)(ce1 - cta_e_base);
      bulk_bytes = (n_el * 8u) & ~15u;
      if (threadIdx.x == 0) {
        p_mbar_init(bar, 1);
        if (n_el & 1u)
          s_pair[n_el - 1] = __ldg(pairs + cta_e_base + n_el - 1);
      }
    }
    asm volatile("fence.mbarrier_init.release.cluster;" ::: "memory");
    __syncthreads();
    if (threadIdx.x == 0 && bulk_bytes) {
      p_mbar_expect_tx(bar, bulk_bytes);
      p_bulk_g2s(s_pair, pairs + cta_e_base, bulk_bytes, bar);
    }
  }
  if (e0_64 >= e_end)
    return;
  const uint32_t e0 = (uint32_t)e0_64;
  const uint32_t e1 = (e0_64 + Q < e_end) ? e0 + Q : e_end;
  const uint32_t c0 = tile * tile_vecs + lane;
  const uint32_t my_vecs = min(tile_vecs, ld4 - tile * tile_vecs);
  const uint32_t row_bytes = my_vecs * 16u;
  bool act[K];
#pragma unroll
  for (int k = 0; k < K; k++)
    act[k] = (k * 32 + lane) < my_vecs;

  uint32_t row = plan_find_row(off, n_rows, e0);
  uint32_t row_end = __ldg(off + row + 1);
  bool row_started_inside = __ldg(off + row) >= e0;
  float4 acc[K];
#pragma unroll
  for (int k = 0; k < K; k++)
    acc[k] = make_float4(0.f, 0.f, 0.f, 0.f);
  auto flush = [&](bool whole) {
    float *orow = out + (size_t)row * F;
#pragma unroll
    for (int k = 0; k < K; k++) {
      const uint32_t col = (c0 + k * 32) * 4;
      if (act[k] && col < F) {
        if (whole)
          flush_chunk<OUTV, false>(orow, col, F, acc[k]);
        else
          flush_chunk<OUTV, true>(orow, col, F, acc[k]);
      }
      acc[k] = make_float4(0.f, 0.f, 0.f, 0.f);
    }
  };
  auto advance = [&](uint32_t ee) {
    flush(row_started_inside);
    do {
      row++;
      row_end = __ldg(off + row + 1);
    } while (ee >= row_end);
    row_started_inside = true;
  };
  if (bulk_bytes)
    p_mbar_wait(bar, 0);
  const uint2 *sp = s_pair - cta_e_base;
  auto issue = [&](uint32_t e, uint32_t stage) {
    const uint32_t src_row = sp[e].x;
    p_mbar_expect_tx(sbar + stage, row_bytes);
    p_bulk_g2s(sbuf + (size_t)stage * tile_vecs, in + (size_t)src_row * ld4 + tile * tile_vecs, row_bytes, sbar + stage);
  };
  if (lane == 0)
    for (uint32_t s = 0; s < STAGES && e0 + s < e1; s++)
      issue(e0 + s, s);
  uint32_t stage = 0, parity = 0;
  for (uint32_t e = e0; e < e1; e++) {
    const float w = __uint_as_float(sp[e].y);
    p_mbar_wait(sbar + stage, parity);
    const float4 *b = sbuf + (size_t)stage * tile_vecs + lane;
    float4 v[K];
#pragma unroll
    for (int k = 0; k < K; k++)
      if (act[k])
        v[k] = b[k * 32];
    if (e >= row_end)
      advance(e);
#pragma unroll
    for (int k = 0; k < K; k++)
      if (act[k]) {
        acc[k].x = fmaf(w, v[k].x, acc[k].x);
        acc[k].y = fmaf(w, v[k].y, acc[k].y);
        acc[k].z = fmaf(w, v[k].z, acc[k].z);
        acc[k].w = fmaf(w, v[k].w, acc[k].w);
      }
    __syncwarp();
    if (lane == 0 && e + STAGES < e1)
      issue(e + STAGES, stage);
    if (++stage == STAGES) {
      stage = 0;
      parity ^= 1u;
    }
  }
  flush(row_started_inside && row_end <= e1);
}

template <int K, int STAGES, int OUTV, int MINB>
static int launch_planned_tma(nts_gather_plan *pl, const PlanShape &sh, const float4 *in, uint32_t ld4, float *out,
                              uint32_t F, uint32_t Q, cudaStream_t st);

struct PlanShape {
  int k, u, outv, minb, g;
  uint32_t tiles, tile_vecs;
};

template <class T, int K, int U, int OUTV, int MINB, int G = 1>
static int launch_planned(nts_gather_plan *pl, const PlanShape &sh, const T *in_rows, uint32_t ldc, float *out,
                          uint32_t F, uint32_t Q, cudaStream_t st) {
  auto kern = planned_gather_sum_kernel<T, K, U, OUTV, MINB, G>;
  const auto *in = reinterpret_cast<const typename GatherT<T>::chunk *>(in_rows);
  const size_t smem = 16 + ((size_t)kPlanWarps * G * Q + 4) * 8;
  NTS_CUDA_OK(cudaFuncSetAttribute(kern, cudaFuncAttributeMaxDynamicSharedMemorySize, (int)smem));
  pl->last_launches = 0;
  for (int s = 0; s < pl->slabs; s++) {
    const uint64_t eb = pl->slab_edge[s], ee = pl->slab_edge[s + 1];
    if (ee <= eb)
      continue;
    const uint64_t quanta = (ee - eb + Q - 1) / Q;
    const uint64_t blocks = (quanta * sh.tiles + kPlanWarps * G - 1) / (kPlanWarps * G);
    NTS_ARG_CHECK(blocks <= 0x7fffffffull, "aggregation grid too large");
    kern<<<(unsigned)blocks, kPlanWarps * 32, smem, st>>>(in, ldc, out, F, pl->pairs, pl->voff + (size_t)s * pl->n_rows,
                                                          pl->n_rows, (uint32_t)eb, (uint32_t)ee, Q, sh.tiles,
                                                          sh.tile_vecs);
    NTS_LAUNCH_CHECK();
    pl->last_grid = (int)blocks;
    pl->last_launches++;
  }
  return 0;
}

template <int K, int STAGES, int OUTV, int MINB>
static int launch_planned_tma(nts_gather_plan *pl, const PlanShape &sh, const float4 *in, uint32_t ld4, float *out,
                              uint32_t F, uint32_t Q, cudaStream_t st) {
  auto kern = planned_gather_sum_tma_kernel<K, STAGES, OUTV, MINB>;
  const uint32_t pair_bytes = (kPlanWarps * Q + 4) * 8;
  const uint32_t ring_bytes = 8u * STAGES + 8u * (STAGES & 1) + STAGES * sh.tile_vecs * 16u;
  const size_t smem = 16 + pair_bytes + (size_t)kPlanWarps * ring_bytes;
  NTS_ARG_CHECK(smem <= 227 * 1024, "row-staging ring does not fit shared memory");
  NTS_CUDA_OK(cudaFuncSetAttribute(kern, cudaFuncAttributeMaxDynamicSharedMemorySize, (int)smem));
  pl->last_launches = 0;
  for (int s = 0; s < pl->slabs; s++) {
    const uint64_t eb = pl->slab_edge[s], ee = pl->slab_edge[s + 1];
    if (ee <= eb)
      continue;
    const uint64_t quanta = (ee - eb + Q - 1) / Q;
    const uint64_t blocks = (quanta * sh.tiles + kPlanWarps - 1) / kPlanWarps;
    NTS_ARG_CHECK(blocks <= 0x7fffffffull, "aggregation grid too large");
    kern<<<(unsigned)blocks, kPlanWarps * 32, smem, st>>>(in, ld4, out, F, pl->pairs, pl->voff + (size_t)s * pl->n_rows,
                                                          pl->n_rows, (uint32_t)eb, (uint32_t)ee, Q, sh.tiles,
                                                          sh.tile_vecs, pair_bytes);
    NTS_LAUNCH_CHECK();
    pl->last_grid = (int)blocks;
    pl->last_launches++;
  }
  return 0;
}

#define NTS_PLAN_TMA_CASE(K_, S_, B_)                                                                               \
  if (sh.k == K_ && stages == S_ && sh.minb == B_) {                                                                \
    if (sh.outv == 4)                                                                                               \
      return launch_planned_tma<K_, S_, 4, B_>(pl, sh, in4, ld4, out, F, Q, st);                                    \
    if (sh.outv == 2)                                                                                               \
      return launch_planned_tma<K_, S_, 2, B_>(pl, sh, in4, ld4, out, F, Q, st);                                    \
    return launch_planned_tma<K_, S_, 1, B_>(pl, sh, in4, ld4, out, F, Q, st);                                      \
  }

#define NTS_PLAN_CASE_G(U_, B_, G_)                                                                                 \
  if (sh.k == 1 && sh.u == U_ && sh.minb == B_ && sh.g == G_) {                                                     \
    if (sh.outv == 4)                                                                                               \
      return launch_planned<T, 1, U_, 4, B_, G_>(pl, sh, in, ldc, out, F, Q, st);                                   \
    if (sh.outv == 2)                                                                                               \
      return launch_planned<T, 1, U_, 2, B_, G_>(pl, sh, in, ldc, out, F, Q, st);                                   \
    return launch_planned<T, 1, U_, 1, B_, G_>(pl, sh, in, ldc, out, F, Q, st);                                     \
  }

#define NTS_PLAN_CASE(K_, U_, B_)                                                                                   \
  if (sh.k == K_ && sh.u == U_ && sh.minb == B_) {                                                                  \
    if (sh.outv == 4)                                                                                               \
      return launch_planned<T, K_, U_, 4, B_>(pl, sh, in, ldc, out, F, Q, st);                                       \
    if (sh.outv == 2)                                                                                               \
      return launch_planned<T, K_, U_, 2, B_>(pl, sh, in, ldc, out, F, Q, st);                                       \
    return launch_planned<T, K_, U_, 1, B_>(pl, sh, in, ldc, out, F, Q, st);                                         \
  }

constexpr int kHubBM = 128, kHubBN = 128, kHubBK = 16, kHubThreads = 256;

__device__ __forceinline__ void p_cp_async16(void *smem_dst, const void *gmem_src, bool full) {
  asm volatile("cp.async.cg.shared.global [%0], [%1], 16, %2;" ::"r"(p_smem_u32(smem_dst)), "l"(gmem_src),
               "r"(full ? 16 : 0)
               : "memory");
}

template <int TN, class TB> struct HubSmem {
  static constexpr uint32_t kBN = 16 * TN;
  float As[2][kHubBK][kHubBM];
  TB Bs[2][kHubBK][kBN];
};

template <class TB, int OUTV, bool SPLIT, bool STORE, int TN, int KKU>
__device__ __forceinline__ void hub_gemm_tile(HubSmem<TN, TB> &sm, uint32_t tile, const float *__restrict__ At,
                                              uint32_t lda, uint32_t M, uint32_t k_lo, uint32_t k_hi, uint32_t k_split,
                                              const TB *__restrict__ B, uint32_t ldb,
                                              const uint32_t *__restrict__ colmap, float *__restrict__ out, uint32_t F,
                                              const uint32_t *__restrict__ rowmap, uint32_t m_tiles, uint32_t n_tiles) {
  static_assert(!(SPLIT && STORE), "split-K partials must be added, not stored");
  constexpr bool kBf16 = std::is_same<TB, __nv_bfloat16>::value;
  constexpr uint32_t kBV = 16 / sizeof(TB);
  constexpr uint32_t kBN = HubSmem<TN, TB>::kBN;
  constexpr uint32_t kBChunks = kHubBK * kBN / kBV;
  auto &As = sm.As;
  auto &Bs = sm.Bs;
  const uint32_t t = threadIdx.x;
  const uint32_t n_tile = tile % n_tiles, rest = tile / n_tiles;
  const uint32_t m0 = (rest % m_tiles) * kHubBM, n0 = n_tile * kBN;
  const uint32_t k_begin = k_lo + (rest / m_tiles) * k_split;
  const uint32_t k_end = min(k_hi, k_begin + k_split);
  if (k_begin >= k_end)
    return;
  const uint32_t n_kt = (k_end - k_begin + kHubBK - 1) / kHubBK;

  auto load = [&](uint32_t kt, int buf) {
#pragma unroll
    for (int i = 0; i < 2; i++) {
      const uint32_t c = t + i * kHubThreads, kk = c >> 5, c4 = (c & 31) * 4;
      const uint32_t k = k_begin + kt * kHubBK + kk;
      const bool a_ok = k < k_end && m0 + c4 < lda;
      p_cp_async16(&As[buf][kk][c4], a_ok ? At + (size_t)k * lda + m0 + c4 : At, a_ok);
    }
#pragma unroll
    for (int i = 0; i < (int)((kBChunks + kHubThreads - 1) / kHubThreads); i++) {
      constexpr uint32_t kRowChunks = kBN / kBV;
      const uint32_t c = t + i * kHubThreads, kk = c / kRowChunks, cv = (c % kRowChunks) * kBV;
      if (kBChunks % kHubThreads != 0 && c >= kBChunks)
        break;
      const uint32_t k = k_begin + kt * kHubBK + kk;
      const bool b_ok = k < k_end && n0 + cv < ldb;
      const uint32_t brow = b_ok ? (colmap ? __ldg(colmap + k) : k) : 0;
      p_cp_async16(&Bs[buf][kk][cv], B + (size_t)brow * ldb + (b_ok ? n0 + cv : 0), b_ok);
    }
    asm volatile("cp.async.commit_group;" ::: "memory");
  };
  auto read_b4 = [&](int buf, int kk, uint32_t n) -> float4 {
    if constexpr (kBf16) {
      const uint2 u = *reinterpret_cast<const uint2 *>(&Bs[buf][kk][n]);
      return make_float4(__uint_as_float(u.x << 16), __uint_as_float(u.x & 0xffff0000u), __uint_as_float(u.y << 16),
                         __uint_as_float(u.y & 0xffff0000u));
    } else {
      return *reinterpret_cast<const float4 *>(&Bs[buf][kk][n]);
    }
  };

  const uint32_t tx = t & 15, ty = t >> 4;
  float acc[8][TN];
#pragma unroll
  for (int i = 0; i < 8; i++)
#pragma unroll
    for (int j = 0; j < TN; j++)
      acc[i][j] = 0.f;

  load(0, 0);
  for (uint32_t kt = 0; kt < n_kt; kt++) {
    const int buf = kt & 1;
    if (kt + 1 < n_kt) {
      load(kt + 1, buf ^ 1);
      asm volatile("cp.async.wait_group 1;" ::: "memory");
    } else {
      asm volatile("cp.async.wait_group 0;" ::: "memory");
    }
    __syncthreads();
#pragma unroll(KKU)
    for (int kk = 0; kk < kHubBK; kk++) {
      const float4 a0 = *reinterpret_cast<const float4 *>(&As[buf][kk][ty * 4]);
      const float4 a1 = *reinterpret_cast<const float4 *>(&As[buf][kk][64 + ty * 4]);
      const float a[8] = {a0.x, a0.y, a0.z, a0.w, a1.x, a1.y, a1.z, a1.w};
      float b[TN];
#pragma unroll
      for (int h = 0; h < TN / 4; h++) {
        const float4 bh = read_b4(buf, kk, h * 64 + tx * 4);
        b[4 * h] = bh.x, b[4 * h + 1] = bh.y, b[4 * h + 2] = bh.z, b[4 * h + 3] = bh.w;
      }
#pragma unroll
      for (int i = 0; i < 8; i++)
#pragma unroll
        for (int j = 0; j < TN; j++)
          acc[i][j] = fmaf(a[i], b[j], acc[i][j]);
    }
    __syncthreads();
  }

#pragma unroll
  for (int i = 0; i < 8; i++) {
    const uint32_t m = m0 + (i >> 2) * 64 + ty * 4 + (i & 3);
    if (m >= M)
      continue;
    float *orow = out + (size_t)(rowmap ? __ldg(rowmap + m) : m) * F;
#pragma unroll
    for (int j = 0; j < TN / 4; j++) {
      const uint32_t col = n0 + j * 64 + tx * 4;
      const float4 a = make_float4(acc[i][j * 4], acc[i][j * 4 + 1], acc[i][j * 4 + 2], acc[i][j * 4 + 3]);
      if (col < F) {
        if constexpr (STORE)
          store_chunk<OUTV>(orow, col, F, a);
        else
          flush_chunk<OUTV, SPLIT>(orow, col, F, a);
      }
    }
  }
}

template <class TB, int OUTV, bool SPLIT, bool STORE>
__global__ void __launch_bounds__(kHubThreads, 2)
    hub_block_gemm_kernel(const float *__restrict__ At, uint32_t lda, uint32_t M, uint32_t K, uint32_t k_split,
                          const TB *__restrict__ B, uint32_t ldb, const uint32_t *__restrict__ colmap,
                          float *__restrict__ out, uint32_t F, const uint32_t *__restrict__ rowmap, uint32_t m_tiles,
                          uint32_t n_tiles) {
  __shared__ __align__(16) HubSmem<8, TB> sm;
  hub_gemm_tile<TB, OUTV, SPLIT, STORE, 8, kHubBK>(sm, blockIdx.x, At, lda, M, 0, K, k_split, B, ldb, colmap, out, F,
                                                   rowmap, m_tiles, n_tiles);
}

static uint32_t hub_row_k_split(uint32_t K, uint32_t m_tiles, uint32_t n_tiles) {
  const uint64_t want = (uint64_t)sm_count() * 2 * 4;
  const uint64_t splits = (want + (uint64_t)m_tiles * n_tiles - 1) / ((uint64_t)m_tiles * n_tiles);
  const uint32_t k_split = (uint32_t)((K + splits - 1) / splits);
  return std::max<uint32_t>((k_split + kHubBK - 1) / kHubBK * kHubBK, 16 * kHubBK);
}

template <class TB, int OUTV>
static int launch_hub_blocks(nts_gather_plan *pl, const TB *in, uint32_t ldb, float *out, uint32_t F, bool rows,
                             bool overwrite, cudaStream_t st) {
  const uint32_t n_tiles = (F + kHubBN - 1) / kHubBN;
  if (pl->hub_cols) {
    const uint32_t m_tiles = (pl->n_rows + kHubBM - 1) / kHubBM;
    const uint64_t blocks = (uint64_t)m_tiles * n_tiles;
    NTS_ARG_CHECK(blocks <= 0x7fffffffull, "hub column block grid too large");
    auto kern = overwrite ? hub_block_gemm_kernel<TB, OUTV, false, true> : hub_block_gemm_kernel<TB, OUTV, false, false>;
    kern<<<(unsigned)blocks, kHubThreads, 0, st>>>(pl->dense, pl->lda_c, pl->n_rows, (uint32_t)pl->hub_cols,
                                                   (uint32_t)pl->hub_cols, in, ldb, pl->hub_col_ids, out, F, nullptr,
                                                   m_tiles, n_tiles);
    NTS_LAUNCH_CHECK();
  }
  if (pl->hub_rows && rows) {
    const uint32_t m_tiles = (pl->hub_rows + kHubBM - 1) / kHubBM;
    const uint32_t K = pl->gather_rows;
    const uint32_t k_split = hub_row_k_split(K, m_tiles, n_tiles);
    const uint64_t splits = (K + k_split - 1) / k_split;
    hub_block_gemm_kernel<TB, OUTV, true, false><<<(unsigned)(splits * m_tiles * n_tiles), kHubThreads, 0, st>>>(
        pl->dense + (size_t)pl->hub_cols * pl->lda_c, pl->lda_r, (uint32_t)pl->hub_rows, K, k_split, in, ldb, nullptr,
        out, F, pl->hub_row_ids, m_tiles, n_tiles);
    NTS_LAUNCH_CHECK();
  }
  return 0;
}

struct HubRowArgs {
  const float *At;
  uint32_t lda, M;
  uint32_t k_lo, k_hi, k_split;
  const uint32_t *rowmap;
  uint32_t m_tiles, n_tiles, n_gemm;
  uint32_t period;
};

template <class T, int K, int U, int OUTV, int MINB, int G>
__global__ void __launch_bounds__(kPlanWarps * 32, MINB)
    planned_slab_hub_kernel(const typename GatherT<T>::chunk *__restrict__ in, uint32_t ldc, float *__restrict__ out,
                            uint32_t F, const uint2 *__restrict__ pairs, const uint32_t *__restrict__ off,
                            uint32_t n_rows, uint32_t e_begin, uint32_t e_end, uint32_t Q, uint32_t tiles,
                            uint32_t tile_vecs, const HubRowArgs hub) {
  static_assert(kPlanWarps * 32 == kHubThreads, "both bodies run 256 threads");
  constexpr int TN = MINB <= 2 ? 8 : 4;
  extern __shared__ __align__(16) unsigned char smem_raw[];
  const uint32_t b = blockIdx.x, grp = b / hub.period;
  if (grp < hub.n_gemm && b - grp * hub.period == hub.period - 1)
    hub_gemm_tile<T, OUTV, true, false, TN, TN == 8 ? kHubBK : 4>(
        *reinterpret_cast<HubSmem<TN, T> *>(smem_raw), grp, hub.At, hub.lda, hub.M, hub.k_lo, hub.k_hi, hub.k_split,
        reinterpret_cast<const T *>(in), ldc * GatherT<T>::V, nullptr, out, F, hub.rowmap, hub.m_tiles, hub.n_tiles);
  else
    planned_gather_body<T, K, U, OUTV, G>(smem_raw, b - min(grp, hub.n_gemm), in, ldc, out, F, pairs, off, n_rows,
                                          e_begin, e_end, Q, tiles, tile_vecs);
}

template <class T, int K, int U, int OUTV, int MINB, int G = 1>
static int launch_fused(nts_gather_plan *pl, const PlanShape &sh, const T *in_rows, uint32_t ldc, float *out,
                        uint32_t F, uint32_t Q, cudaStream_t st) {
  constexpr int TN = MINB <= 2 ? 8 : 4;
  auto kern = planned_slab_hub_kernel<T, K, U, OUTV, MINB, G>;
  const auto *in = reinterpret_cast<const typename GatherT<T>::chunk *>(in_rows);
  const size_t smem = std::max(16 + ((size_t)kPlanWarps * G * Q + 4) * 8, sizeof(HubSmem<TN, T>));
  NTS_CUDA_OK(cudaFuncSetAttribute(kern, cudaFuncAttributeMaxDynamicSharedMemorySize, (int)smem));
  HubRowArgs hub;
  hub.At = pl->dense + (size_t)pl->hub_cols * pl->lda_c;
  hub.lda = pl->lda_r;
  hub.M = (uint32_t)pl->hub_rows;
  hub.rowmap = pl->hub_row_ids;
  hub.m_tiles = (hub.M + kHubBM - 1) / kHubBM;
  hub.n_tiles = (F + 16 * TN - 1) / (16 * TN);
  hub.k_split = hub_row_k_split(pl->gather_rows, hub.m_tiles, hub.n_tiles);
  pl->last_launches = 0;
  for (int s = 0; s < pl->slabs; s++) {
    hub.k_lo = (uint32_t)std::min<uint64_t>((uint64_t)s * pl->slab_rows, pl->gather_rows);
    hub.k_hi = s + 1 == pl->slabs ? pl->gather_rows
                                  : (uint32_t)std::min<uint64_t>((uint64_t)(s + 1) * pl->slab_rows, pl->gather_rows);
    const uint64_t splits = hub.k_hi > hub.k_lo ? (hub.k_hi - hub.k_lo + hub.k_split - 1) / hub.k_split : 0;
    const uint64_t n_gemm = splits * hub.m_tiles * hub.n_tiles;
    const uint64_t eb = pl->slab_edge[s], ee = pl->slab_edge[s + 1];
    const uint64_t quanta = ee > eb ? (ee - eb + Q - 1) / Q : 0;
    const uint64_t blocks = n_gemm + (quanta * sh.tiles + kPlanWarps * G - 1) / (kPlanWarps * G);
    if (!blocks)
      continue;
    NTS_ARG_CHECK(blocks <= 0x7fffffffull, "aggregation grid too large");
    hub.n_gemm = (uint32_t)n_gemm;
    hub.period = n_gemm ? (uint32_t)(blocks / n_gemm) : 1;
    kern<<<(unsigned)blocks, kPlanWarps * 32, smem, st>>>(in, ldc, out, F, pl->pairs, pl->voff + (size_t)s * pl->n_rows,
                                                          pl->n_rows, (uint32_t)eb, (uint32_t)ee, Q, sh.tiles,
                                                          sh.tile_vecs, hub);
    NTS_LAUNCH_CHECK();
    pl->last_grid = (int)blocks;
    pl->last_launches++;
  }
  return 0;
}

#define NTS_PLAN_FUSED_CASE(K_, U_, B_, G_)                                                                         \
  if (sh.k == K_ && sh.u == U_ && sh.minb == B_ && sh.g == G_) {                                                    \
    if (sh.outv == 4)                                                                                               \
      return launch_fused<T, K_, U_, 4, B_, G_>(pl, sh, in, ldc, out, F, Q, st);                                    \
    if (sh.outv == 2)                                                                                               \
      return launch_fused<T, K_, U_, 2, B_, G_>(pl, sh, in, ldc, out, F, Q, st);                                    \
    return launch_fused<T, K_, U_, 1, B_, G_>(pl, sh, in, ldc, out, F, Q, st);                                      \
  }

template <class T>
static int run_gather(nts_gather_plan *pl, const T *in, uint32_t ld, float *output, uint32_t F, bool overwrite,
                      cudaStream_t st) {
  constexpr bool kBf16 = std::is_same<T, __nv_bfloat16>::value;
  PlanShape sh;
  const uint32_t ldc = ld / GatherT<T>::V;
  const uint32_t chunks = (ldc + 31) / 32;
  const uint32_t kmax = 5;
  sh.tiles = (chunks + kmax - 1) / kmax;
  sh.tile_vecs = (ldc + sh.tiles - 1) / sh.tiles;
  sh.k = (int)((sh.tile_vecs + 31) / 32);
  sh.tiles = (ldc + sh.tile_vecs - 1) / sh.tile_vecs;
  sh.outv = (F % 4 == 0 && aligned_to(output, 16)) ? 4 : ((F % 2 == 0 && aligned_to(output, 8)) ? 2 : 1);
  const bool fused = pl->overlap && pl->hub_rows;
  NTS_ARG_CHECK(!fused || g_plan_variant == 0, "the fused slab launches use the register-staging gather (variant 0)");
  if (overwrite && !pl->hub_cols)
    NTS_CUDA_OK(cudaMemsetAsync(output, 0, (size_t)pl->n_rows * F * sizeof(float), st));
  if (pl->hub_cols || pl->hub_rows) {
    const int rc = sh.outv == 4   ? launch_hub_blocks<T, 4>(pl, in, ld, output, F, !fused, overwrite, st)
                   : sh.outv == 2 ? launch_hub_blocks<T, 2>(pl, in, ld, output, F, !fused, overwrite, st)
                                  : launch_hub_blocks<T, 1>(pl, in, ld, output, F, !fused, overwrite, st);
    if (rc)
      return rc;
  }
  sh.g = ldc <= 8 ? 4 : (ldc <= 16 ? 2 : 1);
  if (g_plan_variant == 1 || getenv("NTS_PLAN_NO_SUBWARP"))
    sh.g = 1;
  sh.minb = sh.k >= 3 ? 2 : (sh.k == 2 ? 3 : 4);
  sh.u = sh.k == 4 ? 2 : 4;
  if constexpr (kBf16) {
    sh.minb = sh.k >= 4 ? 2 : (sh.k >= 2 ? 3 : 4);
    sh.u = sh.k == 1 ? 4 : 2;
  }
  {
    static int env_read = 0;
    if (!env_read) {
      env_read = 1;
      if (const char *t = getenv("NTS_PLAN_TUNE"))
        sscanf(t, "%d,%d,%d", &g_plan_u, &g_plan_minb, &g_plan_q);
    }
    if (g_plan_u > 0)
      sh.u = g_plan_u;
    if (g_plan_minb > 0)
      sh.minb = g_plan_minb;
  }
  uint32_t Q = g_plan_q > 0 ? (uint32_t)g_plan_q : 512u / sh.g;
  if (g_plan_q <= 0) {
    const uint64_t per_slab = pl->slab_edge[pl->slabs] / (uint64_t)pl->slabs + 1;
    const uint64_t want_warps = (uint64_t)sm_count() * 64 * sh.g;
    while (Q > 32 && ((per_slab + Q - 1) / Q) * sh.tiles < want_warps)
      Q >>= 1;
  }
  Q = (Q + 31u) & ~31u;
  if (Q * sh.g > 1024)
    Q = (1024 / sh.g) & ~31u;
  pl->last_k = sh.k, pl->last_u = sh.u, pl->last_outv = sh.outv;
  float *out = output;
  if (fused) {
    if constexpr (kBf16) {
      NTS_PLAN_FUSED_CASE(1, 4, 4, 2)
      NTS_PLAN_FUSED_CASE(1, 4, 4, 4)
      NTS_PLAN_FUSED_CASE(1, 4, 4, 1)
      NTS_PLAN_FUSED_CASE(2, 2, 3, 1)
      NTS_PLAN_FUSED_CASE(3, 2, 3, 1)
      NTS_PLAN_FUSED_CASE(4, 2, 2, 1)
      NTS_PLAN_FUSED_CASE(5, 2, 2, 1)
    } else {
      NTS_PLAN_FUSED_CASE(1, 4, 4, 2)
      NTS_PLAN_FUSED_CASE(1, 4, 4, 4)
      NTS_PLAN_FUSED_CASE(1, 4, 4, 1)
      NTS_PLAN_FUSED_CASE(2, 4, 3, 1)
      NTS_PLAN_FUSED_CASE(3, 4, 2, 1)
      NTS_PLAN_FUSED_CASE(4, 2, 2, 1)
      NTS_PLAN_FUSED_CASE(5, 4, 2, 1)
    }
    return fail(-1, "no fused slab/hub-row instantiation for this (chunks, U, occupancy) point", __FILE__, __LINE__);
  }
  if constexpr (kBf16) {
    NTS_PLAN_CASE_G(4, 4, 2)
    NTS_PLAN_CASE_G(4, 4, 4)
    NTS_PLAN_CASE_G(8, 2, 2)
    NTS_PLAN_CASE_G(8, 2, 4)
    if (sh.g != 1)
      return fail(-1, "no BF16 virtual-warp instantiation for this (U, occupancy) point", __FILE__, __LINE__);
    NTS_PLAN_CASE(1, 4, 4)
    NTS_PLAN_CASE(1, 8, 2)
    NTS_PLAN_CASE(2, 2, 3)
    NTS_PLAN_CASE(2, 4, 2)
    NTS_PLAN_CASE(3, 4, 2)
    NTS_PLAN_CASE(3, 2, 3)
    NTS_PLAN_CASE(3, 6, 1)
    NTS_PLAN_CASE(4, 2, 2)
    NTS_PLAN_CASE(4, 4, 2)
    NTS_PLAN_CASE(5, 2, 2)
    return fail(-1, "no BF16 planned-aggregation instantiation for this (chunks, U, occupancy) point", __FILE__,
                __LINE__);
  } else {
  const float4 *in4 = reinterpret_cast<const float4 *>(in);
  const uint32_t ld4 = ldc;
  if (g_plan_variant == 1) {
    const int stages = sh.u >= 8 ? 8 : (sh.u >= 4 ? 4 : 2);
    NTS_PLAN_TMA_CASE(1, 8, 4)
    NTS_PLAN_TMA_CASE(1, 4, 4)
    NTS_PLAN_TMA_CASE(1, 8, 3)
    NTS_PLAN_TMA_CASE(2, 4, 3)
    NTS_PLAN_TMA_CASE(2, 4, 2)
    NTS_PLAN_TMA_CASE(3, 4, 2)
    NTS_PLAN_TMA_CASE(4, 4, 2)
    NTS_PLAN_TMA_CASE(4, 2, 2)
    NTS_PLAN_TMA_CASE(5, 4, 2)
    NTS_PLAN_TMA_CASE(5, 2, 2)
    NTS_PLAN_TMA_CASE(5, 4, 1)
    NTS_PLAN_TMA_CASE(5, 8, 1)
    return fail(-1, "no TMA row-staging instantiation for this (chunks, stages, occupancy) point", __FILE__, __LINE__);
  }
  NTS_PLAN_CASE_G(4, 4, 2)
  NTS_PLAN_CASE_G(4, 4, 4)
  NTS_PLAN_CASE_G(8, 3, 2)
  NTS_PLAN_CASE_G(8, 3, 4)
  if (sh.g != 1)
    return fail(-1, "no virtual-warp instantiation for this (U, occupancy) point", __FILE__, __LINE__);
  NTS_PLAN_CASE(1, 8, 4)
  NTS_PLAN_CASE(1, 4, 4)
  NTS_PLAN_CASE(1, 8, 3)
  NTS_PLAN_CASE(1, 16, 2)
  NTS_PLAN_CASE(2, 4, 3)
  NTS_PLAN_CASE(2, 8, 2)
  NTS_PLAN_CASE(3, 4, 3)
  NTS_PLAN_CASE(3, 4, 2)
  NTS_PLAN_CASE(4, 2, 2)
  NTS_PLAN_CASE(4, 4, 2)
  NTS_PLAN_CASE(5, 2, 2)
  NTS_PLAN_CASE(5, 1, 3)
  NTS_PLAN_CASE(5, 2, 3)
  NTS_PLAN_CASE(5, 4, 1)
  NTS_PLAN_CASE(5, 4, 2)
  return fail(-1, "no planned-aggregation instantiation for this (chunks, U, occupancy) point", __FILE__, __LINE__);
  }
}

template <class E> static int ensure_workspace(E *&ws, size_t &have, size_t elems) {
  if (elems <= have)
    return 0;
  if (ws)
    NTS_CUDA_OK(cudaFree(ws));
  ws = nullptr;
  have = 0;
  NTS_CUDA_OK(cudaMalloc(reinterpret_cast<void **>(&ws), elems * sizeof(E)));
  have = elems;
  return 0;
}

static int run_prologue(nts_gather_plan *pl, const void *input, uint32_t lds, float *output, uint32_t F, int flags,
                        bool *done, cudaStream_t st) {
  *done = true;
  NTS_ARG_CHECK((flags & ~(NTS_PLAN_OVERWRITE | NTS_PLAN_COPY_INPUT)) == 0, "unknown plan run flags");
  if (pl->n_rows == 0 || F == 0)
    return 0;
  if (pl->n_edges == 0) {
    if (flags & NTS_PLAN_OVERWRITE) {
      NTS_ARG_CHECK(output != nullptr, "null output pointer");
      NTS_CUDA_OK(cudaMemsetAsync(output, 0, (size_t)pl->n_rows * F * sizeof(float), st));
    }
    return 0;
  }
  NTS_ARG_CHECK(input && output, "null feature pointer");
  NTS_ARG_CHECK(lds >= F, "row stride below the feature width");
  *done = false;
  return 0;
}

int run_plan(nts_gather_plan *pl, const float *input, uint32_t lds, float *output, uint32_t F, int flags,
             cudaStream_t st) {
  bool done = false;
  if (const int rc = run_prologue(pl, input, lds, output, F, flags, &done, st))
    return rc;
  if (done)
    return 0;
  if (lds % 4 == 0 && aligned_to(input, 16) && !(flags & NTS_PLAN_COPY_INPUT))
    return run_gather<float>(pl, input, lds, output, F, flags & NTS_PLAN_OVERWRITE, st);
  const uint32_t ld = (F + 3u) & ~3u;
  if (const int rc = ensure_workspace(pl->workspace, pl->workspace_floats, (size_t)pl->gather_rows * ld))
    return rc;
  const uint64_t total = (uint64_t)pl->gather_rows * ld;
  const unsigned blocks = (unsigned)std::min<uint64_t>((total + 255) / 256, (uint64_t)sm_count() * 32);
  pad_rows_kernel<<<blocks, 256, 0, st>>>(input, lds, pl->workspace, pl->gather_rows, F, ld);
  NTS_LAUNCH_CHECK();
  return run_gather<float>(pl, pl->workspace, ld, output, F, flags & NTS_PLAN_OVERWRITE, st);
}

int to_bf16_rows(const void *src, int dtype, uint32_t lds, void *dst, uint32_t n_rows, uint32_t F, uint32_t ld,
                 cudaStream_t st) {
  NTS_ARG_CHECK(dtype == NTS_DTYPE_F32 || dtype == NTS_DTYPE_BF16, "input dtype must be NTS_DTYPE_F32 or NTS_DTYPE_BF16");
  NTS_ARG_CHECK(ld % 8 == 0 && ld >= F && lds >= F && aligned_to(dst, 16), "bad BF16 row layout");
  if (!n_rows || !F)
    return 0;
  const uint64_t total = (uint64_t)n_rows * (ld / 8);
  const unsigned blocks = (unsigned)std::min<uint64_t>((total + 255) / 256, (uint64_t)sm_count() * 32);
  uint4 *d = static_cast<uint4 *>(dst);
  if (dtype == NTS_DTYPE_F32)
    bf16_rows_kernel<float><<<blocks, 256, 0, st>>>(static_cast<const float *>(src), lds, d, n_rows, F, ld);
  else
    bf16_rows_kernel<__nv_bfloat16><<<blocks, 256, 0, st>>>(static_cast<const __nv_bfloat16 *>(src), lds, d, n_rows,
                                                            F, ld);
  NTS_LAUNCH_CHECK();
  return 0;
}

int run_plan_bf16(nts_gather_plan *pl, const void *input, int dtype, uint32_t lds, float *output, uint32_t F,
                  cudaStream_t st, int flags) {
  NTS_ARG_CHECK(dtype == NTS_DTYPE_F32 || dtype == NTS_DTYPE_BF16, "input dtype must be NTS_DTYPE_F32 or NTS_DTYPE_BF16");
  NTS_ARG_CHECK(g_plan_variant == 0, "the TMA row-staging variant (nts_gather_plan_set_variant(1)) gathers FP32 rows only");
  bool done = false;
  if (const int rc = run_prologue(pl, input, lds, output, F, flags, &done, st))
    return rc;
  if (done)
    return 0;
  const bool overwrite = flags & NTS_PLAN_OVERWRITE;
  if (dtype == NTS_DTYPE_BF16 && lds % 8 == 0 && aligned_to(input, 16) && !(flags & NTS_PLAN_COPY_INPUT))
    return run_gather<__nv_bfloat16>(pl, static_cast<const __nv_bfloat16 *>(input), lds, output, F, overwrite, st);
  const uint32_t ld = (F + 7u) & ~7u;
  if (const int rc = ensure_workspace(pl->workspace_bf16, pl->workspace_bf16_elems, (size_t)pl->gather_rows * ld))
    return rc;
  if (const int rc = to_bf16_rows(input, dtype, lds, pl->workspace_bf16, pl->gather_rows, F, ld, st))
    return rc;
  return run_gather<__nv_bfloat16>(pl, pl->workspace_bf16, ld, output, F, overwrite, st);
}

static int pick_slabs_for_rows(nts_vid_t gather_rows, uint64_t n_edges, nts_vid_t n_rows, uint64_t row_bytes,
                               uint64_t l2_budget_bytes) {
  if (!l2_budget_bytes)
    l2_budget_bytes = 16ull << 20;
  const uint64_t bytes = (uint64_t)gather_rows * row_bytes;
  uint64_t s = (bytes + l2_budget_bytes - 1) / l2_budget_bytes;
  const uint64_t by_degree = n_rows ? n_edges / ((uint64_t)n_rows * 16ull) : 1;
  if (s > by_degree)
    s = by_degree;
  if (s > 64)
    s = 64;
  return s < 1 ? 1 : (int)s;
}

static bool hub_counts(const nts_vid_t *offsets, const nts_vid_t *indices, const nts_vid_t *slot_of, nts_vid_t base,
                       uint32_t n_rows, uint32_t E, uint32_t gather_rows, std::vector<uint32_t> &col_cnt,
                       std::vector<uint32_t> &seg, cudaStream_t st) {
  uint32_t *cnt = nullptr;
  std::vector<uint32_t> off(n_rows + 1);
  col_cnt.assign(gather_rows, 0);
  const unsigned blocks = (unsigned)std::min<uint64_t>(((uint64_t)E + 255) / 256, (uint64_t)sm_count() * 32);
  bool ok = cudaMalloc(reinterpret_cast<void **>(&cnt), (size_t)gather_rows * 4) == cudaSuccess &&
            cudaMemsetAsync(cnt, 0, (size_t)gather_rows * 4, st) == cudaSuccess;
  if (ok && E) {
    plan_ref_count_kernel<<<blocks, 256, 0, st>>>(indices, slot_of, base, E, cnt);
    count_launch();
  }
  ok = ok && cudaMemcpyAsync(col_cnt.data(), cnt, (size_t)gather_rows * 4, cudaMemcpyDeviceToHost, st) == cudaSuccess &&
       cudaMemcpyAsync(off.data(), offsets, ((size_t)n_rows + 1) * 4, cudaMemcpyDeviceToHost, st) == cudaSuccess &&
       cudaStreamSynchronize(st) == cudaSuccess;
  cudaFree(cnt);
  seg.resize(n_rows);
  for (uint32_t r = 0; r < n_rows; r++)
    seg[r] = off[r + 1] - off[r];
  return ok;
}

static std::vector<uint32_t> top_ids(const std::vector<uint32_t> &cnt, size_t h) {
  std::vector<uint32_t> ids(cnt.size());
  for (size_t i = 0; i < ids.size(); i++)
    ids[i] = (uint32_t)i;
  h = std::min(h, ids.size());
  std::partial_sort(ids.begin(), ids.begin() + h, ids.end(),
                    [&](uint32_t a, uint32_t b) { return cnt[a] != cnt[b] ? cnt[a] > cnt[b] : a < b; });
  ids.resize(h);
  return ids;
}

static nts_gather_plan *refuse_plan(const char *what) {
  fail(-1, what, __FILE__, __LINE__);
  return nullptr;
}

template <class KeyT>
static bool sort_plan(nts_gather_plan *pl, const nts_plan_part *parts, int n_parts, const nts_plan_part *d_parts,
                      int n_hub_cols, int n_hub_rows, cudaStream_t st) {
  constexpr bool hubs = sizeof(KeyT) == 8;
  const uint32_t E = (uint32_t)pl->n_edges, n_rows = pl->n_rows, G = pl->gather_rows;
  const uint64_t n_keys = (uint64_t)pl->slabs * n_rows;
  uint64_t dc_cells = 0;
  uint32_t *d_col_slot = nullptr, *d_row_slot = nullptr, *d_runs = nullptr;
  bool ok = true;
  if (hubs) {
    const nts_plan_part &pt = parts[0];
    std::vector<uint32_t> col_cnt, seg;
    if (!hub_counts(pt.offsets, pt.indices, pt.slot_of, pt.index_base, n_rows, E, G, col_cnt, seg, st))
      return false;
    const std::vector<uint32_t> cols = top_ids(col_cnt, (size_t)n_hub_cols), rows = top_ids(seg, (size_t)n_hub_rows);
    pl->hub_cols = (int)cols.size();
    pl->hub_rows = (int)rows.size();
    pl->lda_c = (n_rows + 3u) & ~3u;
    pl->lda_r = ((uint32_t)pl->hub_rows + 3u) & ~3u;
    dc_cells = (uint64_t)pl->hub_cols * pl->lda_c;
    pl->dense_floats = dc_cells + (pl->hub_rows ? (uint64_t)G * pl->lda_r : 0);
    std::vector<uint32_t> col_slot(G, kNoHub), row_slot(n_rows, kNoHub);
    for (size_t i = 0; i < cols.size(); i++)
      col_slot[cols[i]] = (uint32_t)i;
    for (size_t i = 0; i < rows.size(); i++)
      row_slot[rows[i]] = (uint32_t)i;
    ok = cudaMalloc(reinterpret_cast<void **>(&pl->dense), pl->dense_floats * 4) == cudaSuccess &&
         cudaMalloc(reinterpret_cast<void **>(&pl->hub_col_ids), cols.size() * 4 + 4) == cudaSuccess &&
         cudaMalloc(reinterpret_cast<void **>(&pl->hub_row_ids), rows.size() * 4 + 4) == cudaSuccess &&
         cudaMalloc(reinterpret_cast<void **>(&d_col_slot), (size_t)G * 4 + 4) == cudaSuccess &&
         cudaMalloc(reinterpret_cast<void **>(&d_row_slot), (size_t)n_rows * 4 + 4) == cudaSuccess &&
         cudaMalloc(reinterpret_cast<void **>(&d_runs), 4) == cudaSuccess &&
         cudaMemcpyAsync(pl->hub_col_ids, cols.data(), cols.size() * 4, cudaMemcpyHostToDevice, st) == cudaSuccess &&
         cudaMemcpyAsync(pl->hub_row_ids, rows.data(), rows.size() * 4, cudaMemcpyHostToDevice, st) == cudaSuccess &&
         cudaMemcpyAsync(d_col_slot, col_slot.data(), (size_t)G * 4, cudaMemcpyHostToDevice, st) == cudaSuccess &&
         cudaMemcpyAsync(d_row_slot, row_slot.data(), (size_t)n_rows * 4, cudaMemcpyHostToDevice, st) == cudaSuccess &&
         cudaMemsetAsync(pl->dense, 0, pl->dense_floats * 4, st) == cudaSuccess;
  }
  int bits = 1;
  while (bits < (int)(8 * sizeof(KeyT)) && (1ull << bits) < n_keys + pl->dense_floats)
    bits++;
  KeyT *key_in = nullptr, *key_out = nullptr;
  uint32_t *val_in = nullptr, *val_out = nullptr;
  void *tmp = nullptr;
  size_t tmp_bytes = 0;
  ok = ok && cudaMalloc(reinterpret_cast<void **>(&key_in), (size_t)E * sizeof(KeyT)) == cudaSuccess &&
       cudaMalloc(reinterpret_cast<void **>(&key_out), (size_t)E * sizeof(KeyT)) == cudaSuccess &&
       cudaMalloc(reinterpret_cast<void **>(&val_in), (size_t)E * 4) == cudaSuccess &&
       cudaMalloc(reinterpret_cast<void **>(&val_out), (size_t)E * 4) == cudaSuccess &&
       cub::DeviceRadixSort::SortPairs(nullptr, tmp_bytes, key_in, key_out, val_in, val_out, (int64_t)E, 0, bits, st) ==
           cudaSuccess &&
       cudaMalloc(&tmp, tmp_bytes ? tmp_bytes : 16) == cudaSuccess;
  uint32_t e_off = 0;
  for (int k = 0; k < n_parts && ok; k++) {
    const nts_plan_part &pt = parts[k];
    if (!pt.n_edges)
      continue;
    const unsigned blocks = (unsigned)std::min<uint64_t>((pt.n_edges + 255) / 256, (uint64_t)sm_count() * 32);
    plan_keys_kernel<KeyT><<<blocks, 256, 0, st>>>(pt, e_off, n_rows, pl->slab_rows, (uint32_t)pl->slabs, d_col_slot,
                                                   d_row_slot, pl->lda_c, dc_cells, pl->lda_r, key_in, val_in);
    count_launch();
    e_off += (uint32_t)pt.n_edges;
  }
  ok = ok && cub::DeviceRadixSort::SortPairs(tmp, tmp_bytes, key_in, key_out, val_in, val_out, (int64_t)E, 0, bits,
                                             st) == cudaSuccess;
  if (ok) {
    const unsigned kb = (unsigned)std::min<uint64_t>((n_keys + 256) / 256, (uint64_t)sm_count() * 32);
    plan_offsets_kernel<KeyT><<<kb, 256, 0, st>>>(key_out, E, (uint32_t)n_keys, pl->voff);
    count_launch();
    std::vector<uint32_t> h(pl->slabs + 1);
    ok = cudaStreamSynchronize(st) == cudaSuccess;
    for (int s = 0; s <= pl->slabs && ok; s++)
      ok = cudaMemcpy(&h[s], pl->voff + (size_t)s * n_rows, 4, cudaMemcpyDeviceToHost) == cudaSuccess;
    for (int s = 0; s <= pl->slabs; s++)
      pl->slab_edge[s] = h[s];
  }
  const uint32_t n_res = (uint32_t)pl->slab_edge[pl->slabs], n_dense = E - n_res;
  if (ok && n_res) {
    const unsigned blocks = (unsigned)std::min<uint64_t>(((uint64_t)n_res + 255) / 256, (uint64_t)sm_count() * 32);
    plan_pairs_kernel<<<blocks, 256, 0, st>>>(val_out, d_parts, n_res, pl->pairs);
    count_launch();
  }
  if constexpr (hubs) {
    if (ok && n_dense) {
      uint32_t n_runs = 0;
      size_t b1 = 0, b2 = 0;
      ok = cub::DeviceRunLengthEncode::Encode(nullptr, b1, key_out + n_res, key_in, val_in, d_runs, (int64_t)n_dense,
                                              st) == cudaSuccess &&
           cub::DeviceScan::ExclusiveSum(nullptr, b2, val_in, d_col_slot, (int64_t)n_dense, st) == cudaSuccess;
      if (ok && std::max(b1, b2) > tmp_bytes) {
        cudaFree(tmp);
        tmp_bytes = std::max(b1, b2);
        ok = cudaMalloc(&tmp, tmp_bytes) == cudaSuccess;
      }
      uint32_t *run_start = nullptr;
      ok = ok && cudaMalloc(reinterpret_cast<void **>(&run_start), (size_t)n_dense * 4) == cudaSuccess &&
           cub::DeviceRunLengthEncode::Encode(tmp, b1, key_out + n_res, key_in, val_in, d_runs, (int64_t)n_dense, st) ==
               cudaSuccess &&
           cudaMemcpyAsync(&n_runs, d_runs, 4, cudaMemcpyDeviceToHost, st) == cudaSuccess &&
           cudaStreamSynchronize(st) == cudaSuccess &&
           cub::DeviceScan::ExclusiveSum(tmp, b2, val_in, run_start, (int64_t)n_runs, st) == cudaSuccess;
      if (ok) {
        const unsigned rb = (unsigned)std::min<uint64_t>(((uint64_t)n_runs * 32 + 255) / 256, (uint64_t)sm_count() * 32);
        plan_cell_sum_kernel<<<rb, 256, 0, st>>>(key_in, run_start, val_in, n_runs, val_out + n_res, parts[0].weight,
                                                 n_keys, pl->dense);
        count_launch();
        ok = cudaStreamSynchronize(st) == cudaSuccess;
      }
      cudaFree(run_start);
    }
  }
  cudaFree(key_in), cudaFree(key_out), cudaFree(val_in), cudaFree(val_out), cudaFree(tmp);
  cudaFree(d_col_slot), cudaFree(d_row_slot), cudaFree(d_runs);
  return ok;
}

static nts_gather_plan *build_plan(const nts_plan_part *parts, int n_parts, nts_vid_t n_rows, nts_vid_t gather_rows,
                                   int n_slabs, int n_hub_cols, int n_hub_rows, cudaStream_t st) {
  uint64_t total = 0;
  for (int k = 0; k < n_parts; k++)
    total += parts[k].n_edges;
  if (total >= 0xffffffffull)
    return refuse_plan("plan edge count must fit uint32 offsets");
  if (n_slabs < 1 || gather_rows == 0)
    n_slabs = 1;
  if ((uint64_t)n_slabs * n_rows >= 0xffffffffull)
    return refuse_plan("slabs * rows must fit 32-bit segment keys");
  const bool hubs = gather_rows > 0 && (n_hub_cols > 0 || n_hub_rows > 0);
  if (hubs && n_parts != 1)
    return refuse_plan("hub blocks need a plan of a single part");
  nts_gather_plan *pl = new nts_gather_plan();
  pl->n_rows = n_rows;
  pl->n_edges = total;
  pl->gather_rows = gather_rows;
  pl->slabs = n_slabs;
  pl->slab_rows = gather_rows ? (gather_rows + n_slabs - 1) / n_slabs : 1;
  pl->slab_edge.assign(n_slabs + 1, 0);
  if (n_rows == 0 || total == 0)
    return pl;
  const uint32_t E = (uint32_t)total;
  nts_plan_part *d_parts = nullptr;
  bool ok = cudaMalloc(reinterpret_cast<void **>(&pl->pairs), (size_t)E * sizeof(uint2)) == cudaSuccess &&
            cudaMalloc(reinterpret_cast<void **>(&pl->voff), ((size_t)n_slabs * n_rows + 1) * 4) == cudaSuccess &&
            cudaMalloc(reinterpret_cast<void **>(&d_parts), n_parts * sizeof(nts_plan_part)) == cudaSuccess &&
            cudaMemcpyAsync(d_parts, parts, n_parts * sizeof(nts_plan_part), cudaMemcpyHostToDevice, st) == cudaSuccess;
  if (ok && n_slabs == 1 && !hubs && n_parts == 1 && parts[0].row_add == 0 && parts[0].n_rows == n_rows) {
    const unsigned blocks = (unsigned)std::min<uint64_t>(((uint64_t)E + 255) / 256, (uint64_t)sm_count() * 32);
    plan_pairs_kernel<<<blocks, 256, 0, st>>>(nullptr, d_parts, E, pl->pairs);
    count_launch();
    ok = cudaMemcpyAsync(pl->voff, parts[0].offsets, ((size_t)n_rows + 1) * 4, cudaMemcpyDeviceToDevice, st) ==
         cudaSuccess;
    pl->slab_edge[1] = E;
  } else if (ok) {
    ok = hubs ? sort_plan<uint64_t>(pl, parts, n_parts, d_parts, n_hub_cols, n_hub_rows, st)
              : sort_plan<uint32_t>(pl, parts, n_parts, d_parts, 0, 0, st);
  }
  if (ok)
    ok = cudaStreamSynchronize(st) == cudaSuccess && cudaGetLastError() == cudaSuccess;
  cudaFree(d_parts);
  if (!ok) {
    nts_gather_plan_destroy(pl);
    return refuse_plan("nts_gather_plan: device allocation or preprocessing failed");
  }
  return pl;
}

static constexpr double kHubFloor = 0.05;
static constexpr int kHubMax = 512;

nts_gather_plan *tune_plan(const nts_plan_part *parts, int n_parts, nts_vid_t n_rows, nts_vid_t gather_rows,
                           nts_vid_t feature_size, bool bf16, int run_flags, bool hubs_allowed, cudaStream_t st) {
  uint64_t n_edges = 0;
  for (int k = 0; k < n_parts; k++)
    n_edges += parts[k].n_edges;
  const uint64_t row_bytes = bf16 ? ((feature_size + 7ull) & ~7ull) * 2ull : ((feature_size + 3ull) & ~3ull) * 4ull;
  const int s_max = pick_slabs_for_rows(gather_rows, n_edges, n_rows, row_bytes, 16ull << 20);
  const char *hub_env = getenv("NTS_PLAN_HUBS");
  const bool try_hubs = hubs_allowed && !(hub_env && strcmp(hub_env, "0") == 0) && n_rows > 0 && gather_rows > 0;
  nts_gather_plan *best = build_plan(parts, n_parts, n_rows, gather_rows, 1, 0, 0, st);
  if (!best || (s_max <= 1 && !try_hubs) || n_edges == 0 || feature_size == 0)
    return best;
  float *x = nullptr, *y = nullptr;
  const size_t xb = (size_t)gather_rows * feature_size * (bf16 ? 2 : sizeof(float)),
               yb = (size_t)n_rows * feature_size * sizeof(float);
  bool ok = cudaMalloc(reinterpret_cast<void **>(&x), xb) == cudaSuccess &&
            cudaMalloc(reinterpret_cast<void **>(&y), yb) == cudaSuccess &&
            cudaMemsetAsync(x, 0, xb, st) == cudaSuccess && cudaMemsetAsync(y, 0, yb, st) == cudaSuccess;
  auto time_plan = [&](nts_gather_plan *pl, float *ms) {
    return time_min_of_two([&] {
      return bf16 ? run_plan_bf16(pl, x, NTS_DTYPE_BF16, feature_size, y, feature_size, st, run_flags)
                  : run_plan(pl, x, feature_size, y, feature_size, run_flags, st);
    }, st, ms) == 0;
  };
  float best_ms = 0.f;
  ok = ok && time_plan(best, &best_ms);
  auto consider = [&](int s, int hc, int hr, float *ms, int overlap = 0) -> int {
    nts_gather_plan *pl = build_plan(parts, n_parts, n_rows, gather_rows, s, hc, hr, st);
    if (pl)
      pl->overlap = overlap;
    if (!pl || !time_plan(pl, ms)) {
      nts_gather_plan_destroy(pl);
      return -1;
    }
    if (*ms < best_ms) {
      nts_gather_plan_destroy(best);
      best = pl;
      best_ms = *ms;
      return 1;
    }
    nts_gather_plan_destroy(pl);
    return 0;
  };
  for (int s = 2; ok && s_max > 1; s *= 2) {
    const int cand = s > s_max ? s_max : s;
    float ms = 0.f;
    const int r = consider(cand, 0, 0, &ms);
    if (r < 0 || (r == 0 && ms > 1.1f * best_ms))
      break;
    if (cand == s_max)
      break;
  }
  if (ok && try_hubs) {
    const nts_plan_part &pt = parts[0];
    std::vector<uint32_t> col_cnt, seg;
    ok = hub_counts(pt.offsets, pt.indices, pt.slot_of, pt.index_base, n_rows, (uint32_t)n_edges, gather_rows, col_cnt,
                    seg, st);
    int n_c = 0, n_r = 0;
    for (uint32_t c : col_cnt)
      n_c += c > kHubFloor * n_rows;
    for (uint32_t s : seg)
      n_r += s > kHubFloor * gather_rows;
    const int plain_slabs = best->slabs;
    float ms = 0.f;
    for (int c = 32; ok && c <= std::min(n_c, kHubMax); c *= 2)
      if (consider(best->slabs, c, 0, &ms) != 1)
        break;
    for (int r = 32; ok && r <= std::min(n_r, kHubMax); r *= 2)
      if (consider(best->slabs, best->hub_cols, r, &ms) != 1)
        break;
    if (best->hub_cols || best->hub_rows) {
      const int hc = best->hub_cols, hr = best->hub_rows;
      for (int s : {plain_slabs / 2, std::min(plain_slabs * 2, s_max)})
        if (s >= 1 && s != plain_slabs && s != best->slabs)
          consider(s, hc, hr, &ms);
    }
    const char *ov_env = getenv("NTS_PLAN_OVERLAP");
    if (ok && best->hub_rows && !(ov_env && strcmp(ov_env, "0") == 0)) {
      best->overlap = 1;
      float fused_ms = 0.f;
      if (time_plan(best, &fused_ms) && fused_ms < best_ms) {
        best_ms = fused_ms;
        for (int r = 2 * best->hub_rows; r <= std::min(n_r, kHubMax); r *= 2)
          if (consider(best->slabs, best->hub_cols, r, &ms, 1) != 1)
            break;
      } else {
        best->overlap = 0;
      }
    }
  }
  cudaFree(x), cudaFree(y);
  best->tuned_ms = best_ms;
  return best;
}

}

using namespace nts;

extern "C" {

int nts_gather_plan_pick_slabs(nts_vid_t gather_rows, uint64_t n_edges, nts_vid_t n_rows, nts_vid_t feature_size,
                               uint64_t l2_budget_bytes) {
  return pick_slabs_for_rows(gather_rows, n_edges, n_rows, ((feature_size + 3ull) & ~3ull) * 4ull, l2_budget_bytes);
}

static bool chunk_part(const nts_vid_t *offsets, const nts_vid_t *indices, const float *weight,
                       const nts_vid_t *slot_of, nts_vid_t index_base, nts_vid_t n_rows, uint64_t n_edges,
                       nts_plan_part *pt) {
  if (n_rows && n_edges && !(offsets && indices)) {
    refuse_plan("null graph array");
    return false;
  }
  *pt = {offsets, indices, weight, slot_of, index_base, 0, n_rows, 0, n_edges};
  return true;
}

nts_gather_plan *nts_gather_plan_create_hybrid(const nts_vid_t *offsets, const nts_vid_t *indices,
                                               const float *weight, const nts_vid_t *slot_of, nts_vid_t index_base,
                                               nts_vid_t n_rows, uint64_t n_edges, nts_vid_t gather_rows, int n_slabs,
                                               int n_hub_cols, int n_hub_rows, void *stream) {
  nts_plan_part pt;
  if (!chunk_part(offsets, indices, weight, slot_of, index_base, n_rows, n_edges, &pt))
    return nullptr;
  if (n_hub_cols < 0 || n_hub_rows < 0)
    return refuse_plan("negative hub count");
  return build_plan(&pt, 1, n_rows, gather_rows, n_slabs, n_hub_cols, n_hub_rows, as_stream(stream));
}

nts_gather_plan *nts_gather_plan_create_tuned_ex(const nts_vid_t *offsets, const nts_vid_t *indices,
                                                 const float *weight, const nts_vid_t *slot_of, nts_vid_t index_base,
                                                 nts_vid_t n_rows, uint64_t n_edges, nts_vid_t gather_rows,
                                                 nts_vid_t feature_size, int gather_dtype, int run_flags,
                                                 void *stream) {
  if ((gather_dtype != NTS_DTYPE_F32 && gather_dtype != NTS_DTYPE_BF16) || (run_flags & ~NTS_PLAN_OVERWRITE))
    return refuse_plan("nts_gather_plan_create_tuned_ex: gather_dtype must be NTS_DTYPE_F32 or NTS_DTYPE_BF16, "
                       "run_flags 0 or NTS_PLAN_OVERWRITE");
  nts_plan_part pt;
  if (!chunk_part(offsets, indices, weight, slot_of, index_base, n_rows, n_edges, &pt))
    return nullptr;
  return tune_plan(&pt, 1, n_rows, gather_rows, feature_size, gather_dtype == NTS_DTYPE_BF16, run_flags, true,
                   as_stream(stream));
}

nts_gather_plan *nts_gather_plan_create_parts(const nts_plan_part *parts, int n_parts, nts_vid_t n_rows,
                                              nts_vid_t gather_rows, int n_slabs, nts_vid_t feature_size, void *stream) {
  if (!parts || n_parts < 1)
    return refuse_plan("no plan parts");
  for (int k = 0; k < n_parts; k++) {
    if (parts[k].n_edges && !(parts[k].offsets && parts[k].indices))
      return refuse_plan("null graph array in a plan part");
    if ((uint64_t)parts[k].row_add + parts[k].n_rows > n_rows)
      return refuse_plan("plan part rows exceed the output rows");
  }
  if (n_slabs >= 1)
    return build_plan(parts, n_parts, n_rows, gather_rows, n_slabs, 0, 0, as_stream(stream));
  return tune_plan(parts, n_parts, n_rows, gather_rows, feature_size, false, 0, false, as_stream(stream));
}

float nts_gather_plan_tuned_ms(const nts_gather_plan *pl) { return pl ? pl->tuned_ms : 0.f; }

int nts_gather_plan_destroy(nts_gather_plan *pl) {
  if (!pl)
    return 0;
  cudaFree(pl->pairs);
  cudaFree(pl->voff);
  cudaFree(pl->workspace);
  cudaFree(pl->workspace_bf16);
  cudaFree(pl->dense);
  cudaFree(pl->hub_col_ids);
  cudaFree(pl->hub_row_ids);
  delete pl;
  return 0;
}

int nts_gather_plan_slabs(const nts_gather_plan *pl) { return pl ? pl->slabs : 0; }

int nts_gather_plan_hubs(const nts_gather_plan *pl, int *cols, int *rows) {
  NTS_ARG_CHECK(pl != nullptr, "null plan");
  if (cols)
    *cols = pl->hub_cols;
  if (rows)
    *rows = pl->hub_rows;
  return 0;
}

int nts_gather_plan_overlap(const nts_gather_plan *pl) { return pl ? pl->overlap : 0; }

int nts_gather_plan_set_overlap(nts_gather_plan *pl, int overlap) {
  NTS_ARG_CHECK(pl != nullptr, "null plan");
  NTS_ARG_CHECK(overlap == 0 || overlap == 1, "overlap must be 0 (sequential) or 1 (fused slab launches)");
  pl->overlap = overlap;
  return 0;
}

uint64_t nts_gather_plan_bytes(const nts_gather_plan *pl) {
  if (!pl)
    return 0;
  return pl->n_edges * 8ull + ((uint64_t)pl->slabs * pl->n_rows + 1) * 4ull + pl->workspace_floats * 4ull +
         pl->workspace_bf16_elems * 2ull + pl->dense_floats * 4ull + ((uint64_t)pl->hub_cols + pl->hub_rows) * 4ull;
}

int nts_gather_plan_last_launch(const nts_gather_plan *pl, int *launches, int *grid, int *k, int *u, int *outv) {
  NTS_ARG_CHECK(pl != nullptr, "null plan");
  if (launches)
    *launches = pl->last_launches;
  if (grid)
    *grid = pl->last_grid;
  if (k)
    *k = pl->last_k;
  if (u)
    *u = pl->last_u;
  if (outv)
    *outv = pl->last_outv;
  return 0;
}

int nts_gather_plan_run_ex(nts_gather_plan *pl, const float *input, nts_vid_t input_ld, float *output,
                           nts_vid_t feature_size, int flags, void *stream) {
  NTS_ARG_CHECK(input_ld >= feature_size, "input row pitch below the feature width");
  NTS_ARG_CHECK(output != nullptr || feature_size == 0, "null output pointer");
  NTS_ARG_CHECK(pl != nullptr, "null plan");
  return run_plan(pl, input, input_ld, output, feature_size, flags, as_stream(stream));
}

int nts_gather_plan_run_bf16_ex(nts_gather_plan *pl, const void *input, int input_dtype, nts_vid_t input_ld,
                                float *output, nts_vid_t feature_size, int flags, void *stream) {
  NTS_ARG_CHECK(input_ld >= feature_size, "input row pitch below the feature width");
  NTS_ARG_CHECK(output != nullptr || feature_size == 0, "null output pointer");
  NTS_ARG_CHECK(pl != nullptr, "null plan");
  return run_plan_bf16(pl, input, input_dtype, input_ld, output, feature_size, as_stream(stream), flags);
}

int nts_rows_to_bf16(const void *src, int src_dtype, nts_vid_t lds, void *dst, nts_vid_t n_rows, nts_vid_t feature_size,
                     nts_vid_t ld, void *stream) {
  NTS_ARG_CHECK((src && dst) || n_rows == 0 || feature_size == 0, "null pointer passed to nts_rows_to_bf16");
  return to_bf16_rows(src, src_dtype, lds, dst, n_rows, feature_size, ld, as_stream(stream));
}

int nts_gather_plan_set_variant(int variant) {
  NTS_ARG_CHECK(variant == 0 || variant == 1, "variant must be 0 (register staging) or 1 (TMA row staging)");
  g_plan_variant = variant;
  return 0;
}

int nts_gather_plan_set_tuning(int u, int min_blocks, int edges_per_warp) {
  NTS_ARG_CHECK(u >= 0 && min_blocks >= 0 && edges_per_warp >= 0 && edges_per_warp <= 4096, "bad tuning point");
  g_plan_u = u;
  g_plan_minb = min_blocks;
  g_plan_q = edges_per_warp;
  return 0;
}

}
```

neutronstarlite_b200/ops.py:

```python
from __future__ import annotations

import ctypes as C
import time as _time

import torch

from . import _lib


def _stream():
    return torch.cuda.current_stream().cuda_stream


def row_pitched(t):
    return t.dim() == 2 and (t.is_contiguous() or (t.stride(1) == 1 and t.stride(0) >= t.shape[1]))


def _check_input(t, name="input", pitched=False):
    if not t.is_cuda:
        raise _lib.NtsError("%s must be a CUDA tensor (libnts_b200 has no CPU fallback)" % name)
    if t.dtype != torch.float32 or t.dim() != 2:
        raise _lib.NtsError("%s must be a 2-D float32 tensor" % name)
    if not (t.is_contiguous() or (pitched and row_pitched(t))):
        raise _lib.NtsError("%s must be contiguous" % name + (" or row-pitched" if pitched else ""))
    return t


def _check_gather_dtype(gather_dtype):
    if gather_dtype is not None and gather_dtype != torch.bfloat16:
        raise _lib.NtsError("gather_dtype must be None or torch.bfloat16, not %s" % (gather_dtype,))
    return gather_dtype


def _check_gathered(t, name, gather_dtype, pitched=False):
    if gather_dtype is None or (t.is_cuda and t.dtype == torch.float32):
        return _check_input(t, name, pitched)
    if not t.is_cuda:
        raise _lib.NtsError("%s must be a CUDA tensor (libnts_b200 has no CPU fallback)" % name)
    if t.dtype != torch.bfloat16 or t.dim() != 2:
        raise _lib.NtsError("%s must be a 2-D float32 or bfloat16 tensor" % name)
    if not (t.is_contiguous() or (pitched and row_pitched(t))):
        raise _lib.NtsError("%s must be contiguous" % name + (" or row-pitched" if pitched else ""))
    return t


_DTYPE_CODE = {torch.float32: 0, torch.bfloat16: 1}
PLAN_OVERWRITE, PLAN_COPY_INPUT = 1, 2


def _ptr(t):
    return 0 if t is None else t.data_ptr()


class KernelTimer:

    def __init__(self):
        self.records = []

    def bracket(self, tag, F, edges, rows):
        start = torch.cuda.Event(enable_timing=True)
        stop = torch.cuda.Event(enable_timing=True)
        self.records.append((tag, int(F), int(edges), int(rows), start, stop))
        return start, stop

    def summary(self):
        torch.cuda.synchronize()
        out = {}
        for tag, F, edges, rows, a, b in self.records:
            d = out.setdefault((tag, F), {"calls": 0, "ms": 0.0, "edges": 0, "rows": 0})
            d["calls"] += 1
            d["ms"] += a.elapsed_time(b)
            d["edges"] += edges
            d["rows"] += rows
        return out


_timer = None


def set_kernel_timer(timer):
    global _timer
    _timer = timer


class _timed:

    def __init__(self, tag, F, edges, rows):
        self.ev = _timer.bracket(tag, F, edges, rows) if _timer else None

    def __enter__(self):
        if self.ev:
            self.ev[0].record()

    def __exit__(self, *exc):
        if self.ev:
            self.ev[1].record()
        return False


def segment_gather_sum(out, x, weight, indices, offsets, index_base, n_rows, n_edges):
    _lib.call("nts_segment_gather_sum", _ptr(x), _ptr(out), _ptr(weight), _ptr(indices), _ptr(offsets),
              int(index_base), int(n_rows), int(n_edges), int(x.shape[1]), _stream())
    return out


class GatherPlan:

    def __init__(self, offsets, indices, weight, index_base, n_rows, n_edges, gather_rows, slabs, slot_of=None,
                 tune_for=0, hubs=(0, 0), gather_dtype=None, tune_accumulate=True):
        L = _lib.load()
        _check_gather_dtype(gather_dtype)
        t0 = _time.perf_counter()
        if slabs > 0:
            self.handle = L.nts_gather_plan_create_hybrid(_ptr(offsets), _ptr(indices), _ptr(weight), _ptr(slot_of),
                                                          int(index_base), int(n_rows), int(n_edges),
                                                          int(gather_rows), int(slabs), int(hubs[0]), int(hubs[1]),
                                                          _stream())
        else:
            self.handle = L.nts_gather_plan_create_tuned_ex(
                _ptr(offsets), _ptr(indices), _ptr(weight), _ptr(slot_of), int(index_base), int(n_rows), int(n_edges),
                int(gather_rows), int(tune_for), _DTYPE_CODE[gather_dtype or torch.float32],
                0 if tune_accumulate else PLAN_OVERWRITE, _stream())
        self.build_s = _time.perf_counter() - t0
        if not self.handle:
            raise _lib.NtsError("gather plan construction failed: " + L.nts_last_error().decode(errors="replace"))
        self.slabs = int(L.nts_gather_plan_slabs(self.handle))
        hc, hr = C.c_int(0), C.c_int(0)
        _lib.call("nts_gather_plan_hubs", self.handle, C.byref(hc), C.byref(hr))
        self.hub_cols, self.hub_rows = hc.value, hr.value
        self.n_rows, self.n_edges = int(n_rows), int(n_edges)

    @property
    def overlap(self):
        return bool(_lib.load().nts_gather_plan_overlap(self.handle))

    def set_overlap(self, overlap):
        _lib.call("nts_gather_plan_set_overlap", self.handle, int(bool(overlap)))

    def key(self):
        return ((self.slabs,) + ((self.hub_cols, self.hub_rows) if self.hub_cols or self.hub_rows else ())
                + (("overlap",) if self.overlap else ()))

    def run(self, x, out, gather_dtype=None, accumulate=True):
        if not row_pitched(x):
            raise _lib.NtsError("the gathered input must have contiguous rows (unit column stride)")
        F = int(x.shape[1])
        ld = F if x.is_contiguous() else int(x.stride(0))
        flags = 0 if accumulate else PLAN_OVERWRITE
        if ld != F and (x.storage_offset() + x.shape[0] * ld) * x.element_size() > x.untyped_storage().nbytes():
            flags |= PLAN_COPY_INPUT
        if _check_gather_dtype(gather_dtype) is not None:
            if x.dtype not in _DTYPE_CODE:
                raise _lib.NtsError("BF16 gathers take a float32 or bfloat16 input, not %s" % x.dtype)
            _lib.call("nts_gather_plan_run_bf16_ex", self.handle, _ptr(x), _DTYPE_CODE[x.dtype], ld, _ptr(out), F,
                      flags, _stream())
            return out
        if x.dtype == torch.bfloat16:
            raise _lib.NtsError("a bfloat16 input needs gather_dtype=torch.bfloat16")
        _lib.call("nts_gather_plan_run_ex", self.handle, _ptr(x), ld, _ptr(out), F, flags, _stream())
        return out

    def bytes(self):
        return int(_lib.load().nts_gather_plan_bytes(self.handle))

    def __del__(self):
        try:
            if getattr(self, "handle", None):
                _lib.load().nts_gather_plan_destroy(self.handle)
                self.handle = None
        except Exception:
            pass


import os as _os

PLAN_MIN_EDGES = 1 << 20
_plan_mode = {"0": "off", "1": "on"}.get(_os.environ.get("NTS_PLAN", ""), "auto")
_plan_slabs = int(_os.environ.get("NTS_PLAN_SLABS", "0"))


def set_plan_mode(mode, slabs=0):
    global _plan_mode, _plan_slabs
    if mode not in ("auto", "on", "off"):
        raise ValueError("plan mode must be auto, on or off")
    _plan_mode, _plan_slabs = mode, int(slabs)


def _chunk_plan(chunk, direction, F, gather_dtype=None):
    if gather_dtype is None and (_plan_mode == "off" or (_plan_mode == "auto" and chunk.edge_size < PLAN_MIN_EDGES)):
        return None
    if direction == "fwd":
        n_rows, gather_rows = chunk.batch_size_forward, chunk.batch_size_backward
    else:
        n_rows, gather_rows = chunk.batch_size_backward, chunk.batch_size_forward
    plans = chunk.__dict__.setdefault("_gather_plans", {})
    tuned = chunk.__dict__.setdefault("_gather_plan_for", {})
    key = (direction, _plan_slabs) if _plan_slabs else (direction, "F", int(F))
    if gather_dtype is not None and not _plan_slabs:
        key += ("bf16",)
    plan = plans.get(key) if _plan_slabs else tuned.get(key)
    if plan is None:
        if direction == "fwd":
            plan = GatherPlan(chunk.column_offset_gpu, chunk.row_indices_gpu, chunk.edge_weight_forward_gpu,
                              chunk.src_range[0], n_rows, chunk.edge_size, gather_rows, _plan_slabs, tune_for=int(F),
                              gather_dtype=gather_dtype, tune_accumulate=False)
        else:
            plan = GatherPlan(chunk.row_offset_gpu, chunk.column_indices_gpu, chunk.edge_weight_backward_gpu,
                              chunk.dst_range[0], n_rows, chunk.edge_size, gather_rows, _plan_slabs, tune_for=int(F),
                              gather_dtype=gather_dtype, tune_accumulate=False)
        share = (direction,) + plan.key()
        if share in plans:
            plan = plans[share]
        plans[share] = plan
        if not _plan_slabs:
            tuned[key] = plan
    return plan


def _bf16_plan(chunk, direction, F, with_weight, gather_dtype):
    if _check_gather_dtype(gather_dtype) is None:
        return _chunk_plan(chunk, direction, F) if with_weight else None
    if not with_weight:
        raise _lib.NtsError("BF16 gathers always apply the edge weights (with_weight=True)")
    return _chunk_plan(chunk, direction, F, gather_dtype)


def _plain_operands(out, x, accumulate):
    if not accumulate:
        out.zero_()
    return x.contiguous()


def gather_by_dst_from_src(chunk, out, x, with_weight=True, gather_dtype=None, accumulate=True):
    plan = _bf16_plan(chunk, "fwd", x.shape[1], with_weight, gather_dtype)
    ev = _timer.bracket("fwd", x.shape[1], chunk.edge_size, chunk.batch_size_forward) if _timer else None
    if ev:
        ev[0].record()
    if plan is not None:
        plan.run(x, out, gather_dtype, accumulate)
    else:
        x = _plain_operands(out, x, accumulate)
        _lib.call("nts_gather_by_dst_from_src", _ptr(x), _ptr(out), _ptr(chunk.edge_weight_forward_gpu),
                  _ptr(chunk.row_indices_gpu), _ptr(chunk.column_offset_gpu), chunk.src_range[0], chunk.src_range[1],
                  chunk.dst_range[0], chunk.dst_range[1], chunk.edge_size, chunk.batch_size_forward,
                  int(x.shape[1]), 1 if with_weight else 0, _stream())
    if ev:
        ev[1].record()
    return out


def gather_by_src_from_dst(chunk, out, grad, with_weight=True, gather_dtype=None, accumulate=True):
    plan = _bf16_plan(chunk, "bwd", grad.shape[1], with_weight, gather_dtype)
    ev = _timer.bracket("bwd", grad.shape[1], chunk.edge_size, chunk.batch_size_backward) if _timer else None
    if ev:
        ev[0].record()
    if plan is not None:
        plan.run(grad, out, gather_dtype, accumulate)
    else:
        grad = _plain_operands(out, grad, accumulate)
        _lib.call("nts_gather_by_src_from_dst", _ptr(grad), _ptr(out), _ptr(chunk.edge_weight_backward_gpu),
                  _ptr(chunk.row_offset_gpu), _ptr(chunk.column_indices_gpu), chunk.src_range[0], chunk.src_range[1],
                  chunk.dst_range[0], chunk.dst_range[1], chunk.edge_size, chunk.batch_size_backward,
                  int(grad.shape[1]), 1 if with_weight else 0, _stream())
    if ev:
        ev[1].record()
    return out


class ntsGraphOp:

    def __init__(self, partitioned_graph, active=None):
        self.partitioned_graph_ = partitioned_graph
        self.active_ = active

    def forward(self, f_input, f_input1=None):
        raise NotImplementedError

    def backward(self, output_grad):
        raise NotImplementedError

    def get_additional_grad(self):
        raise NotImplementedError("get_additional_grad is not implemented")


class ForwardSingleGPUfuseOp(ntsGraphOp):

    def __init__(self, partitioned_graph, active=None, gather_dtype=None):
        super().__init__(partitioned_graph, active)
        self.gather_dtype = _check_gather_dtype(gather_dtype)

    def forward(self, f_input, f_input1=None):
        x = _check_gathered(f_input, "input", self.gather_dtype, pitched=True)
        c = self.partitioned_graph_.graph_chunks[0]
        y = torch.empty((c.batch_size_forward, x.shape[1]), dtype=torch.float32, device=x.device)
        return gather_by_dst_from_src(c, y, x, gather_dtype=self.gather_dtype, accumulate=False)

    def backward(self, f_output_grad):
        g = _check_input(f_output_grad, "output_grad", pitched=True)
        c = self.partitioned_graph_.graph_chunks[0]
        dx = torch.empty((c.batch_size_backward, g.shape[1]), dtype=torch.float32, device=g.device)
        return gather_by_src_from_dst(c, dx, g, gather_dtype=self.gather_dtype, accumulate=False)


class MiniBatchFuseOp(ntsGraphOp):

    def __init__(self, sampled_subgraph, hop, table=False):
        super().__init__(sampled_subgraph, None)
        self.block = sampled_subgraph.blocks[hop]
        self.hop, self.table = int(hop), bool(table)
        self.vertices = getattr(sampled_subgraph, "vertices", None)
        if self.table and (self.block.row_global is None or self.vertices is None):
            raise _lib.NtsError("table=True needs the block's global source ids (row_global) and the graph's vertex "
                                "count (SampledSubgraph.vertices)")

    def forward(self, f_input, f_input1=None):
        x = _check_input(f_input, "input")
        b = self.block
        if self.table and x.shape[0] < self.vertices:
            raise _lib.NtsError("the feature table has %d rows, the sampled graph has %d vertices"
                                % (x.shape[0], self.vertices))
        if not self.table and x.shape[0] != b.n_src:
            raise _lib.NtsError("input has %d rows, hop %d has %d sources" % (x.shape[0], self.hop, b.n_src))
        y = torch.zeros((b.n_dst, x.shape[1]), dtype=torch.float32, device=x.device)
        with _timed("minibatch_fwd", x.shape[1], b.n_edges, b.n_dst):
            return segment_gather_sum(y, x, b.weight, b.row_global if self.table else b.row_indices,
                                      b.column_offset, 0, b.n_dst, b.n_edges)

    def backward(self, f_output_grad):
        if self.table:
            raise _lib.NtsError("a table gather (table=True) has no backward")
        g = _check_input(f_output_grad, "output_grad")
        b = self.block
        if g.shape[0] != b.n_dst:
            raise _lib.NtsError("output_grad has %d rows, hop %d has %d destinations" % (g.shape[0], self.hop, b.n_dst))
        dx = torch.zeros((b.n_src, g.shape[1]), dtype=torch.float32, device=g.device)
        with _timed("minibatch_bwd", g.shape[1], b.n_edges, b.n_src):
            return segment_gather_sum(dx, g, b.weight_backward, b.column_indices, b.row_offset, 0, b.n_src, b.n_edges)


class ForwardGPUfuseOp(ntsGraphOp):

    def __init__(self, partitioned_graph, active=None, exchange=None, gather_dtype=None):
        super().__init__(partitioned_graph, active)
        self.gather_dtype = _check_gather_dtype(gather_dtype)
        if exchange is None:
            from .exchange import default_exchange
            exchange = default_exchange(partitioned_graph)
        self.exchange = exchange

    def forward(self, f_input, f_input1=None):
        x = _check_gathered(f_input, "input", self.gather_dtype)
        if self.gather_dtype is None:
            return self.exchange.forward(x)
        return self.exchange.forward(x, gather_dtype=self.gather_dtype)

    def backward(self, f_output_grad):
        g = _check_input(f_output_grad, "output_grad")
        if self.gather_dtype is None:
            return self.exchange.backward(g)
        return self.exchange.backward(g, gather_dtype=self.gather_dtype)


class _EdgeOp(ntsGraphOp):
    def _topo(self):
        pg = self.partitioned_graph_
        if pg.column_offset_gpu is None or pg.row_indices_gpu is None:
            raise _lib.NtsError("whole-partition CSC missing: call PartitionedGraph.generate_all(dist=True, device=...)")
        return pg


class DistGPUGetDepNbrOp(ntsGraphOp):

    def __init__(self, partitioned_graph, active=None, exchange=None):
        super().__init__(partitioned_graph, active)
        if exchange is None:
            from .exchange import default_exchange
            exchange = default_exchange(partitioned_graph)
        self.exchange = exchange

    def forward(self, f_input, f_input1=None):
        return self.exchange.fetch_mirrors(_check_input(f_input))

    def backward(self, f_output_grad):
        return self.exchange.return_mirror_grads(_check_input(f_output_grad, "output_grad"))


class DistGPUScatterSrc(_EdgeOp):

    def forward(self, f_input, f_input1=None):
        pg = self._topo()
        x = _check_input(f_input)
        msg = torch.zeros((pg.owned_edges, x.shape[1]), dtype=torch.float32, device=x.device)
        _lib.call("nts_scatter_src_mirror_to_msg", _ptr(msg), _ptr(x), _ptr(pg.row_indices_gpu),
                  _ptr(pg.column_offset_gpu), _ptr(pg.mirror_index_gpu), pg.owned_vertices, x.shape[1], _stream())
        return msg

    def backward(self, f_output_grad):
        pg = self._topo()
        g = _check_input(f_output_grad, "output_grad")
        out = torch.zeros((pg.owned_mirrors, g.shape[1]), dtype=torch.float32, device=g.device)
        _lib.call("nts_gather_msg_to_src_mirror", _ptr(out), _ptr(g), _ptr(pg.row_indices_gpu),
                  _ptr(pg.column_offset_gpu), _ptr(pg.mirror_index_gpu), pg.owned_vertices, g.shape[1], _stream())
        return out


class DistGPUScatterDst(_EdgeOp):

    def forward(self, f_input, f_input1=None):
        pg = self._topo()
        x = _check_input(f_input)
        msg = torch.zeros((pg.owned_edges, x.shape[1]), dtype=torch.float32, device=x.device)
        _lib.call("nts_scatter_dst_to_msg", _ptr(msg), _ptr(x), _ptr(pg.row_indices_gpu),
                  _ptr(pg.column_offset_gpu), pg.owned_vertices, x.shape[1], _stream())
        return msg

    def backward(self, f_output_grad):
        pg = self._topo()
        g = _check_input(f_output_grad, "output_grad")
        out = torch.zeros((pg.owned_vertices, g.shape[1]), dtype=torch.float32, device=g.device)
        _lib.call("nts_gather_msg_to_dst", _ptr(out), _ptr(g), _ptr(pg.row_indices_gpu),
                  _ptr(pg.column_offset_gpu), pg.owned_vertices, g.shape[1], _stream())
        return out


class DistGPUAggregateDst(_EdgeOp):

    def forward(self, f_input, f_input1=None):
        pg = self._topo()
        m = _check_input(f_input)
        out = torch.zeros((pg.owned_vertices, m.shape[1]), dtype=torch.float32, device=m.device)
        _lib.call("nts_gather_msg_to_dst", _ptr(out), _ptr(m), _ptr(pg.row_indices_gpu),
                  _ptr(pg.column_offset_gpu), pg.owned_vertices, m.shape[1], _stream())
        return out

    def backward(self, f_output_grad):
        pg = self._topo()
        g = _check_input(f_output_grad, "output_grad")
        msg = torch.zeros((pg.owned_edges, g.shape[1]), dtype=torch.float32, device=g.device)
        _lib.call("nts_scatter_dst_to_msg", _ptr(msg), _ptr(g), _ptr(pg.row_indices_gpu),
                  _ptr(pg.column_offset_gpu), pg.owned_vertices, g.shape[1], _stream())
        return msg


class DistGPUEdgeSoftMax(_EdgeOp):

    def __init__(self, partitioned_graph, active=None):
        super().__init__(partitioned_graph, active)
        self.IntermediateResult = None

    def forward(self, f_input, f_input1=None):
        pg = self._topo()
        m = _check_input(f_input)
        out = torch.zeros_like(m)
        self.IntermediateResult = torch.zeros_like(m)
# ... 271 lines not shown
```

Measured before the change: 16.25 billion.

## Add output row pitch and padded outputs with L2 prefetch of destination rows

Threads an output leading dimension through the planned gather, hub GEMM and TMA kernels so outputs can be written into row-padded buffers. The single-GPU fuse op allocates outputs padded to a multiple of four floats when the feature width is not already aligned, which allows vectorized stores. The gather kernel also issues bulk L2 prefetches of the output row when a new row starts. This adds API surface and a strided output view, which downstream consumers may need to copy if they require contiguous tensors.

Result: faster. 16.69 billion, median of 6 (+2.7%).

```diff
diff --git a/include/nts_b200.h b/include/nts_b200.h
--- a/include/nts_b200.h
+++ b/include/nts_b200.h
@@ -86,13 +86,17 @@
 int nts_gather_plan_overlap(const nts_gather_plan *plan);
 int nts_gather_plan_set_overlap(nts_gather_plan *plan, int overlap);
 uint64_t nts_gather_plan_bytes(const nts_gather_plan *plan);
-enum { NTS_PLAN_ACCUMULATE = 0, NTS_PLAN_OVERWRITE = 1, NTS_PLAN_COPY_INPUT = 2 };
+enum { NTS_PLAN_ACCUMULATE = 0, NTS_PLAN_OVERWRITE = 1, NTS_PLAN_COPY_INPUT = 2, NTS_PLAN_PAD_OUTPUT = 4 };
 int nts_gather_plan_run_ex(nts_gather_plan *plan, const float *input, nts_vid_t input_ld, float *output,
                            nts_vid_t feature_size, int flags, void *stream);
+int nts_gather_plan_run_ld(nts_gather_plan *plan, const float *input, nts_vid_t input_ld, float *output,
+                           nts_vid_t output_ld, nts_vid_t feature_size, int flags, void *stream);
 int nts_gather_plan_last_launch(const nts_gather_plan *plan, int *launches, int *grid, int *k, int *u, int *outv);
 enum { NTS_DTYPE_F32 = 0, NTS_DTYPE_BF16 = 1 };
 int nts_gather_plan_run_bf16_ex(nts_gather_plan *plan, const void *input, int input_dtype, nts_vid_t input_ld,
                                 float *output, nts_vid_t feature_size, int flags, void *stream);
+int nts_gather_plan_run_bf16_ld(nts_gather_plan *plan, const void *input, int input_dtype, nts_vid_t input_ld,
+                                float *output, nts_vid_t output_ld, nts_vid_t feature_size, int flags, void *stream);
 int nts_gather_plan_set_tuning(int u, int min_blocks, int edges_per_warp);
 int nts_gather_plan_set_variant(int variant);
 
diff --git a/neutronstarlite_b200/_lib.py b/neutronstarlite_b200/_lib.py
--- a/neutronstarlite_b200/_lib.py
+++ b/neutronstarlite_b200/_lib.py
@@ -56,6 +56,8 @@
     "nts_gather_plan_bytes": (_u64, [_vp]),
     "nts_gather_plan_run_ex": (_int, [_vp, _vp, _u32, _vp, _u32, _int, _vp]),
     "nts_gather_plan_run_bf16_ex": (_int, [_vp, _vp, _int, _u32, _vp, _u32, _int, _vp]),
+    "nts_gather_plan_run_ld": (_int, [_vp, _vp, _u32, _vp, _u32, _u32, _int, _vp]),
+    "nts_gather_plan_run_bf16_ld": (_int, [_vp, _vp, _int, _u32, _vp, _u32, _u32, _int, _vp]),
     "nts_gather_plan_create_tuned_ex": (_vp, [_vp, _vp, _vp, _vp, _u32, _u32, _u64, _u32, _u32, _int, _int, _vp]),
     "nts_gather_plan_last_launch": (_int, [_vp] + [C.POINTER(_int)] * 5),
     "nts_gather_plan_set_tuning": (_int, [_int, _int, _int]),
diff --git a/neutronstarlite_b200/csrc/nts_common.cuh b/neutronstarlite_b200/csrc/nts_common.cuh
--- a/neutronstarlite_b200/csrc/nts_common.cuh
+++ b/neutronstarlite_b200/csrc/nts_common.cuh
@@ -52,10 +52,10 @@
 
 int time_min_of_two(const std::function<int()> &run, cudaStream_t st, float *ms);
 
-int run_plan(nts_gather_plan *pl, const float *input, uint32_t lds, float *output, uint32_t F, int flags,
+int run_plan(nts_gather_plan *pl, const float *input, uint32_t lds, float *output, uint32_t ldo, uint32_t F, int flags,
              cudaStream_t st);
-int run_plan_bf16(nts_gather_plan *pl, const void *input, int dtype, uint32_t lds, float *output, uint32_t F,
-                  cudaStream_t st, int flags = 0);
+int run_plan_bf16(nts_gather_plan *pl, const void *input, int dtype, uint32_t lds, float *output, uint32_t ldo,
+                  uint32_t F, cudaStream_t st, int flags = 0);
 int to_bf16_rows(const void *src, int dtype, uint32_t lds, void *dst, uint32_t n_rows, uint32_t F, uint32_t ld,
                  cudaStream_t st);
 
diff --git a/neutronstarlite_b200/csrc/nts_exchange.cu b/neutronstarlite_b200/csrc/nts_exchange.cu
--- a/neutronstarlite_b200/csrc/nts_exchange.cu
+++ b/neutronstarlite_b200/csrc/nts_exchange.cu
@@ -349,8 +349,8 @@
       plans.emplace_back(plan_key(F, gt.bf16), pl);
     }
     if (gt.bf16)
-      return run_plan_bf16(pl, in_rows, NTS_DTYPE_BF16, gt.ld, out, F, st);
-    return run_plan(pl, in, F, out, F, 0, st);
+      return run_plan_bf16(pl, in_rows, NTS_DTYPE_BF16, gt.ld, out, F, F, st);
+    return run_plan(pl, in, F, out, F, F, 0, st);
   }
   return nts_segment_gather_sum(in, out, w, idx, off, base, n_rows, c.edges, F, st);
 }
@@ -415,7 +415,8 @@
   int rc = time_min_of_two([&]() { return aggregate_chunk(ex, p, forward, a, b, F, st, gt); }, st, &L);
   if (!rc)
     rc = time_min_of_two([&]() {
-      return gt.bf16 ? run_plan_bf16(m.merged, a, NTS_DTYPE_BF16, gt.ld, b, F, st) : run_plan(m.merged, a, F, b, F, 0, st);
+      return gt.bf16 ? run_plan_bf16(m.merged, a, NTS_DTYPE_BF16, gt.ld, b, F, F, st)
+                     : run_plan(m.merged, a, F, b, F, F, 0, st);
     }, st, &M);
   for (int i = 0; i < P && !rc; i++) {
     if (i == p || !ex->chunks[i].edges || !ex->need_count[i])
@@ -754,9 +755,9 @@
     if (tr)
       NTS_CUDA_OK(cudaEventRecord(ex->tev[4], st));
     if (bf16)
-      NTS_TRY(run_plan_bf16(mode->merged, ex->window + buf, NTS_DTYPE_BF16, gt.ld, y, F, st));
+      NTS_TRY(run_plan_bf16(mode->merged, ex->window + buf, NTS_DTYPE_BF16, gt.ld, y, F, F, st));
     else
-      NTS_TRY(run_plan(mode->merged, ex->window + buf, F, y, F, 0, st));
+      NTS_TRY(run_plan(mode->merged, ex->window + buf, F, y, F, F, 0, st));
     if (tr)
       for (int s = 1; s < P; s++) {
         NTS_CUDA_OK(cudaEventRecord(ex->tev[5 + 2 * (s - 1)], st));
@@ -808,9 +809,9 @@
   NTS_TRY(decide_mode(ex, false, F, st, &mode, gt));
   if (mode->mode == 2) {
     if (bf16)
-      NTS_TRY(run_plan_bf16(mode->merged, gin, NTS_DTYPE_BF16, gt.ld, ex->bsend, F, st));
+      NTS_TRY(run_plan_bf16(mode->merged, gin, NTS_DTYPE_BF16, gt.ld, ex->bsend, F, F, st));
     else
-      NTS_TRY(run_plan(mode->merged, g, F, ex->bsend, F, 0, st));
+      NTS_TRY(run_plan(mode->merged, g, F, ex->bsend, F, F, 0, st));
     NTS_CUDA_OK(cudaEventRecord(ex->ev_peer[p], st));
     NTS_CUDA_OK(cudaStreamWaitEvent(ex->comm, ex->ev_peer[p], 0));
     for (int s = 1; s < P; s++) {
diff --git a/neutronstarlite_b200/csrc/nts_plan.cu b/neutronstarlite_b200/csrc/nts_plan.cu
--- a/neutronstarlite_b200/csrc/nts_plan.cu
+++ b/neutronstarlite_b200/csrc/nts_plan.cu
@@ -280,10 +280,10 @@
 template <class T, int K, int U, int OUTV, int G>
 __device__ __forceinline__ void planned_gather_body(unsigned char *smem_raw, uint32_t vblock,
                                                     const typename GatherT<T>::chunk *__restrict__ in, uint32_t ldc,
-                                                    float *__restrict__ out, uint32_t F,
+                                                    float *__restrict__ out, uint32_t ldo, uint32_t F,
                                                     const uint2 *__restrict__ pairs, const uint32_t *__restrict__ off,
                                                     uint32_t n_rows, uint32_t e_begin, uint32_t e_end, uint32_t Q,
-                                                    uint32_t tiles, uint32_t tile_vecs) {
+                                                    uint32_t tiles, uint32_t tile_vecs, uint32_t prefetch) {
   static_assert(G == 1 || K == 1, "virtual warps are for rows narrower than a warp");
   using Chunk = typename GatherT<T>::chunk;
   constexpr int V = GatherT<T>::V;
@@ -345,8 +345,19 @@
     for (int j = 0; j < V; j++)
       acc[k][j] = 0.f;
 
+  auto prefetch_row = [&]() {
+    if constexpr (OUTV == 4) {
+      if (prefetch && (threadIdx.x & (GS - 1)) == 0 && c0 * V < F)
+        asm volatile("cp.async.bulk.prefetch.L2.global [%0], %1;" ::"l"(out + (size_t)row * ldo + c0 * V),
+                     "r"(min(prefetch, (F - c0 * V) * 4u))
+                     : "memory");
+    }
+  };
+  if (row_started_inside)
+    prefetch_row();
+
   auto flush = [&](bool whole) {
-    float *orow = out + (size_t)row * F;
+    float *orow = out + (size_t)row * ldo;
 #pragma unroll
     for (int k = 0; k < K; k++) {
 #pragma unroll
@@ -372,6 +383,7 @@
       row_end = __ldg(off + row + 1);
     } while (ee >= row_end);
     row_started_inside = true;
+    prefetch_row();
   };
 
   if (bulk_bytes)
@@ -431,19 +443,19 @@
 template <class T, int K, int U, int OUTV, int MINB, int G = 1>
 __global__ void __launch_bounds__(kPlanWarps * 32, MINB)
     planned_gather_sum_kernel(const typename GatherT<T>::chunk *__restrict__ in, uint32_t ldc, float *__restrict__ out,
-                              uint32_t F, const uint2 *__restrict__ pairs, const uint32_t *__restrict__ off,
-                              uint32_t n_rows, uint32_t e_begin, uint32_t e_end, uint32_t Q, uint32_t tiles,
-                              uint32_t tile_vecs) {
+                              uint32_t ldo, uint32_t F, const uint2 *__restrict__ pairs,
+                              const uint32_t *__restrict__ off, uint32_t n_rows, uint32_t e_begin, uint32_t e_end,
+                              uint32_t Q, uint32_t tiles, uint32_t tile_vecs, uint32_t prefetch) {
   extern __shared__ __align__(16) unsigned char smem_raw[];
-  planned_gather_body<T, K, U, OUTV, G>(smem_raw, blockIdx.x, in, ldc, out, F, pairs, off, n_rows, e_begin, e_end, Q,
-                                        tiles, tile_vecs);
+  planned_gather_body<T, K, U, OUTV, G>(smem_raw, blockIdx.x, in, ldc, out, ldo, F, pairs, off, n_rows, e_begin, e_end,
+                                        Q, tiles, tile_vecs, prefetch);
 }
 
 struct PlanShape;
 template <int K, int STAGES, int OUTV, int MINB>
 __global__ void __launch_bounds__(kPlanWarps * 32, MINB)
-    planned_gather_sum_tma_kernel(const float4 *__restrict__ in, uint32_t ld4, float *__restrict__ out, uint32_t F,
-                                  const uint2 *__restrict__ pairs, const uint32_t *__restrict__ off, uint32_t n_rows,
+    planned_gather_sum_tma_kernel(const float4 *__restrict__ in, uint32_t ld4, float *__restrict__ out, uint32_t ldo,
+                                  uint32_t F, const uint2 *__restrict__ pairs, const uint32_t *__restrict__ off, uint32_t n_rows,
                                   uint32_t e_begin, uint32_t e_end, uint32_t Q, uint32_t tiles, uint32_t tile_vecs,
                                   uint32_t pair_bytes) {
   const uint32_t lane = threadIdx.x & 31;
@@ -509,7 +521,7 @@
   for (int k = 0; k < K; k++)
     acc[k] = make_float4(0.f, 0.f, 0.f, 0.f);
   auto flush = [&](bool whole) {
-    float *orow = out + (size_t)row * F;
+    float *orow = out + (size_t)row * ldo;
 #pragma unroll
     for (int k = 0; k < K; k++) {
       const uint32_t col = (c0 + k * 32) * 4;
@@ -579,6 +591,8 @@
 struct PlanShape {
   int k, u, outv, minb, g;
   uint32_t tiles, tile_vecs;
+  uint32_t ldo;
+  uint32_t prefetch;
 };
 
 template <class T, int K, int U, int OUTV, int MINB, int G = 1>
@@ -596,9 +610,9 @@
     const uint64_t quanta = (ee - eb + Q - 1) / Q;
     const uint64_t blocks = (quanta * sh.tiles + kPlanWarps * G - 1) / (kPlanWarps * G);
     NTS_ARG_CHECK(blocks <= 0x7fffffffull, "aggregation grid too large");
-    kern<<<(unsigned)blocks, kPlanWarps * 32, smem, st>>>(in, ldc, out, F, pl->pairs, pl->voff + (size_t)s * pl->n_rows,
-                                                          pl->n_rows, (uint32_t)eb, (uint32_t)ee, Q, sh.tiles,
-                                                          sh.tile_vecs);
+    kern<<<(unsigned)blocks, kPlanWarps * 32, smem, st>>>(in, ldc, out, sh.ldo, F, pl->pairs,
+                                                          pl->voff + (size_t)s * pl->n_rows, pl->n_rows, (uint32_t)eb,
+                                                          (uint32_t)ee, Q, sh.tiles, sh.tile_vecs, sh.prefetch);
     NTS_LAUNCH_CHECK();
     pl->last_grid = (int)blocks;
     pl->last_launches++;
@@ -623,9 +637,9 @@
     const uint64_t quanta = (ee - eb + Q - 1) / Q;
     const uint64_t blocks = (quanta * sh.tiles + kPlanWarps - 1) / kPlanWarps;
     NTS_ARG_CHECK(blocks <= 0x7fffffffull, "aggregation grid too large");
-    kern<<<(unsigned)blocks, kPlanWarps * 32, smem, st>>>(in, ld4, out, F, pl->pairs, pl->voff + (size_t)s * pl->n_rows,
-                                                          pl->n_rows, (uint32_t)eb, (uint32_t)ee, Q, sh.tiles,
-                                                          sh.tile_vecs, pair_bytes);
+    kern<<<(unsigned)blocks, kPlanWarps * 32, smem, st>>>(in, ld4, out, sh.ldo, F, pl->pairs,
+                                                          pl->voff + (size_t)s * pl->n_rows, pl->n_rows, (uint32_t)eb,
+                                                          (uint32_t)ee, Q, sh.tiles, sh.tile_vecs, pair_bytes);
     NTS_LAUNCH_CHECK();
     pl->last_grid = (int)blocks;
     pl->last_launches++;
@@ -678,8 +692,9 @@
 __device__ __forceinline__ void hub_gemm_tile(HubSmem<TN, TB> &sm, uint32_t tile, const float *__restrict__ At,
                                               uint32_t lda, uint32_t M, uint32_t k_lo, uint32_t k_hi, uint32_t k_split,
                                               const TB *__restrict__ B, uint32_t ldb,
-                                              const uint32_t *__restrict__ colmap, float *__restrict__ out, uint32_t F,
-                                              const uint32_t *__restrict__ rowmap, uint32_t m_tiles, uint32_t n_tiles) {
+                                              const uint32_t *__restrict__ colmap, float *__restrict__ out, uint32_t ldo,
+                                              uint32_t F, const uint32_t *__restrict__ rowmap, uint32_t m_tiles,
+                                              uint32_t n_tiles) {
   static_assert(!(SPLIT && STORE), "split-K partials must be added, not stored");
   constexpr bool kBf16 = std::is_same<TB, __nv_bfloat16>::value;
   constexpr uint32_t kBV = 16 / sizeof(TB);
@@ -770,7 +785,7 @@
     const uint32_t m = m0 + (i >> 2) * 64 + ty * 4 + (i & 3);
     if (m >= M)
       continue;
-    float *orow = out + (size_t)(rowmap ? __ldg(rowmap + m) : m) * F;
+    float *orow = out + (size_t)(rowmap ? __ldg(rowmap + m) : m) * ldo;
 #pragma unroll
     for (int j = 0; j < TN / 4; j++) {
       const uint32_t col = n0 + j * 64 + tx * 4;
@@ -789,11 +804,11 @@
 __global__ void __launch_bounds__(kHubThreads, 2)
     hub_block_gemm_kernel(const float *__restrict__ At, uint32_t lda, uint32_t M, uint32_t K, uint32_t k_split,
                           const TB *__restrict__ B, uint32_t ldb, const uint32_t *__restrict__ colmap,
-                          float *__restrict__ out, uint32_t F, const uint32_t *__restrict__ rowmap, uint32_t m_tiles,
-                          uint32_t n_tiles) {
+                          float *__restrict__ out, uint32_t ldo, uint32_t F, const uint32_t *__restrict__ rowmap,
+                          uint32_t m_tiles, uint32_t n_tiles) {
   __shared__ __align__(16) HubSmem<8, TB> sm;
-  hub_gemm_tile<TB, OUTV, SPLIT, STORE, 8, kHubBK>(sm, blockIdx.x, At, lda, M, 0, K, k_split, B, ldb, colmap, out, F,
-                                                   rowmap, m_tiles, n_tiles);
+  hub_gemm_tile<TB, OUTV, SPLIT, STORE, 8, kHubBK>(sm, blockIdx.x, At, lda, M, 0, K, k_split, B, ldb, colmap, out, ldo,
+                                                   F, rowmap, m_tiles, n_tiles);
 }
 
 static uint32_t hub_row_k_split(uint32_t K, uint32_t m_tiles, uint32_t n_tiles) {
@@ -804,8 +819,8 @@
 }
 
 template <class TB, int OUTV>
-static int launch_hub_blocks(nts_gather_plan *pl, const TB *in, uint32_t ldb, float *out, uint32_t F, bool rows,
-                             bool overwrite, cudaStream_t st) {
+static int launch_hub_blocks(nts_gather_plan *pl, const TB *in, uint32_t ldb, float *out, uint32_t ldo, uint32_t F,
+                             bool rows, bool overwrite, cudaStream_t st) {
   const uint32_t n_tiles = (F + kHubBN - 1) / kHubBN;
   if (pl->hub_cols) {
     const uint32_t m_tiles = (pl->n_rows + kHubBM - 1) / kHubBM;
@@ -813,8 +828,8 @@
     NTS_ARG_CHECK(blocks <= 0x7fffffffull, "hub column block grid too large");
     auto kern = overwrite ? hub_block_gemm_kernel<TB, OUTV, false, true> : hub_block_gemm_kernel<TB, OUTV, false, false>;
     kern<<<(unsigned)blocks, kHubThreads, 0, st>>>(pl->dense, pl->lda_c, pl->n_rows, (uint32_t)pl->hub_cols,
-                                                   (uint32_t)pl->hub_cols, in, ldb, pl->hub_col_ids, out, F, nullptr,
-                                                   m_tiles, n_tiles);
+                                                   (uint32_t)pl->hub_cols, in, ldb, pl->hub_col_ids, out, ldo, F,
+                                                   nullptr, m_tiles, n_tiles);
     NTS_LAUNCH_CHECK();
   }
   if (pl->hub_rows && rows) {
@@ -824,7 +839,7 @@
     const uint64_t splits = (K + k_split - 1) / k_split;
     hub_block_gemm_kernel<TB, OUTV, true, false><<<(unsigned)(splits * m_tiles * n_tiles), kHubThreads, 0, st>>>(
         pl->dense + (size_t)pl->hub_cols * pl->lda_c, pl->lda_r, (uint32_t)pl->hub_rows, K, k_split, in, ldb, nullptr,
-        out, F, pl->hub_row_ids, m_tiles, n_tiles);
+        out, ldo, F, pl->hub_row_ids, m_tiles, n_tiles);
     NTS_LAUNCH_CHECK();
   }
   return 0;
@@ -842,9 +857,9 @@
 template <class T, int K, int U, int OUTV, int MINB, int G>
 __global__ void __launch_bounds__(kPlanWarps * 32, MINB)
     planned_slab_hub_kernel(const typename GatherT<T>::chunk *__restrict__ in, uint32_t ldc, float *__restrict__ out,
-                            uint32_t F, const uint2 *__restrict__ pairs, const uint32_t *__restrict__ off,
-                            uint32_t n_rows, uint32_t e_begin, uint32_t e_end, uint32_t Q, uint32_t tiles,
-                            uint32_t tile_vecs, const HubRowArgs hub) {
+                            uint32_t ldo, uint32_t F, const uint2 *__restrict__ pairs,
+                            const uint32_t *__restrict__ off, uint32_t n_rows, uint32_t e_begin, uint32_t e_end,
+                            uint32_t Q, uint32_t tiles, uint32_t tile_vecs, uint32_t prefetch, const HubRowArgs hub) {
   static_assert(kPlanWarps * 32 == kHubThreads, "both bodies run 256 threads");
   constexpr int TN = MINB <= 2 ? 8 : 4;
   extern __shared__ __align__(16) unsigned char smem_raw[];
@@ -852,10 +867,11 @@
   if (grp < hub.n_gemm && b - grp * hub.period == hub.period - 1)
     hub_gemm_tile<T, OUTV, true, false, TN, TN == 8 ? kHubBK : 4>(
         *reinterpret_cast<HubSmem<TN, T> *>(smem_raw), grp, hub.At, hub.lda, hub.M, hub.k_lo, hub.k_hi, hub.k_split,
-        reinterpret_cast<const T *>(in), ldc * GatherT<T>::V, nullptr, out, F, hub.rowmap, hub.m_tiles, hub.n_tiles);
+        reinterpret_cast<const T *>(in), ldc * GatherT<T>::V, nullptr, out, ldo, F, hub.rowmap, hub.m_tiles,
+        hub.n_tiles);
   else
-    planned_gather_body<T, K, U, OUTV, G>(smem_raw, b - min(grp, hub.n_gemm), in, ldc, out, F, pairs, off, n_rows,
-                                          e_begin, e_end, Q, tiles, tile_vecs);
+    planned_gather_body<T, K, U, OUTV, G>(smem_raw, b - min(grp, hub.n_gemm), in, ldc, out, ldo, F, pairs, off, n_rows,
+                                          e_begin, e_end, Q, tiles, tile_vecs, prefetch);
 }
 
 template <class T, int K, int U, int OUTV, int MINB, int G = 1>
@@ -889,9 +905,9 @@
     NTS_ARG_CHECK(blocks <= 0x7fffffffull, "aggregation grid too large");
     hub.n_gemm = (uint32_t)n_gemm;
     hub.period = n_gemm ? (uint32_t)(blocks / n_gemm) : 1;
-    kern<<<(unsigned)blocks, kPlanWarps * 32, smem, st>>>(in, ldc, out, F, pl->pairs, pl->voff + (size_t)s * pl->n_rows,
-                                                          pl->n_rows, (uint32_t)eb, (uint32_t)ee, Q, sh.tiles,
-                                                          sh.tile_vecs, hub);
+    kern<<<(unsigned)blocks, kPlanWarps * 32, smem, st>>>(in, ldc, out, sh.ldo, F, pl->pairs,
+                                                          pl->voff + (size_t)s * pl->n_rows, pl->n_rows, (uint32_t)eb,
+                                                          (uint32_t)ee, Q, sh.tiles, sh.tile_vecs, sh.prefetch, hub);
     NTS_LAUNCH_CHECK();
     pl->last_grid = (int)blocks;
     pl->last_launches++;
@@ -908,10 +924,18 @@
     return launch_fused<T, K_, U_, 1, B_, G_>(pl, sh, in, ldc, out, F, Q, st);                                      \
   }
 
+static cudaError_t zero_rows(float *output, uint32_t ldo, uint32_t F, uint32_t n_rows, cudaStream_t st) {
+  if (ldo == F)
+    return cudaMemsetAsync(output, 0, (size_t)n_rows * F * sizeof(float), st);
+  return cudaMemset2DAsync(output, (size_t)ldo * sizeof(float), 0, (size_t)F * sizeof(float), n_rows, st);
+}
+
 template <class T>
-static int run_gather(nts_gather_plan *pl, const T *in, uint32_t ld, float *output, uint32_t F, bool overwrite,
-                      cudaStream_t st) {
+static int run_gather(nts_gather_plan *pl, const T *in, uint32_t ld, float *output, uint32_t ldo, uint32_t F,
+                      bool overwrite, bool pad_output, cudaStream_t st) {
   constexpr bool kBf16 = std::is_same<T, __nv_bfloat16>::value;
+  if (pad_output)
+    F = (F + 3u) & ~3u;
   PlanShape sh;
   const uint32_t ldc = ld / GatherT<T>::V;
   const uint32_t chunks = (ldc + 31) / 32;
@@ -920,15 +944,22 @@
   sh.tile_vecs = (ldc + sh.tiles - 1) / sh.tiles;
   sh.k = (int)((sh.tile_vecs + 31) / 32);
   sh.tiles = (ldc + sh.tile_vecs - 1) / sh.tile_vecs;
-  sh.outv = (F % 4 == 0 && aligned_to(output, 16)) ? 4 : ((F % 2 == 0 && aligned_to(output, 8)) ? 2 : 1);
+  sh.outv = (F % 4 == 0 && ldo % 4 == 0 && aligned_to(output, 16))
+                ? 4
+                : ((F % 2 == 0 && ldo % 2 == 0 && aligned_to(output, 8)) ? 2 : 1);
+  sh.ldo = ldo;
+  {
+    const char *pf_env = getenv("NTS_PLAN_PREFETCH");
+    sh.prefetch = (pf_env && strcmp(pf_env, "0") == 0) ? 0u : sh.tile_vecs * GatherT<T>::V * 4u;
+  }
   const bool fused = pl->overlap && pl->hub_rows;
   NTS_ARG_CHECK(!fused || g_plan_variant == 0, "the fused slab launches use the register-staging gather (variant 0)");
   if (overwrite && !pl->hub_cols)
-    NTS_CUDA_OK(cudaMemsetAsync(output, 0, (size_t)pl->n_rows * F * sizeof(float), st));
+    NTS_CUDA_OK(zero_rows(output, ldo, F, pl->n_rows, st));
   if (pl->hub_cols || pl->hub_rows) {
-    const int rc = sh.outv == 4   ? launch_hub_blocks<T, 4>(pl, in, ld, output, F, !fused, overwrite, st)
-                   : sh.outv == 2 ? launch_hub_blocks<T, 2>(pl, in, ld, output, F, !fused, overwrite, st)
-                                  : launch_hub_blocks<T, 1>(pl, in, ld, output, F, !fused, overwrite, st);
+    const int rc = sh.outv == 4   ? launch_hub_blocks<T, 4>(pl, in, ld, output, ldo, F, !fused, overwrite, st)
+                   : sh.outv == 2 ? launch_hub_blocks<T, 2>(pl, in, ld, output, ldo, F, !fused, overwrite, st)
+                                  : launch_hub_blocks<T, 1>(pl, in, ld, output, ldo, F, !fused, overwrite, st);
     if (rc)
       return rc;
   }
@@ -1060,16 +1091,20 @@
   return 0;
 }
 
-static int run_prologue(nts_gather_plan *pl, const void *input, uint32_t lds, float *output, uint32_t F, int flags,
-                        bool *done, cudaStream_t st) {
+static int run_prologue(nts_gather_plan *pl, const void *input, uint32_t lds, float *output, uint32_t ldo, uint32_t F,
+                        int flags, bool *done, cudaStream_t st) {
   *done = true;
-  NTS_ARG_CHECK((flags & ~(NTS_PLAN_OVERWRITE | NTS_PLAN_COPY_INPUT)) == 0, "unknown plan run flags");
+  NTS_ARG_CHECK((flags & ~(NTS_PLAN_OVERWRITE | NTS_PLAN_COPY_INPUT | NTS_PLAN_PAD_OUTPUT)) == 0,
+                "unknown plan run flags");
+  NTS_ARG_CHECK(ldo >= F, "output row pitch below the feature width");
+  NTS_ARG_CHECK(!(flags & NTS_PLAN_PAD_OUTPUT) || ldo >= ((F + 3u) & ~3u),
+                "NTS_PLAN_PAD_OUTPUT needs an output row pitch of at least F rounded up to 4");
   if (pl->n_rows == 0 || F == 0)
     return 0;
   if (pl->n_edges == 0) {
     if (flags & NTS_PLAN_OVERWRITE) {
       NTS_ARG_CHECK(output != nullptr, "null output pointer");
-      NTS_CUDA_OK(cudaMemsetAsync(output, 0, (size_t)pl->n_rows * F * sizeof(float), st));
+      NTS_CUDA_OK(zero_rows(output, ldo, F, pl->n_rows, st));
     }
     return 0;
   }
@@ -1079,15 +1114,16 @@
   return 0;
 }
 
-int run_plan(nts_gather_plan *pl, const float *input, uint32_t lds, float *output, uint32_t F, int flags,
+int run_plan(nts_gather_plan *pl, const float *input, uint32_t lds, float *output, uint32_t ldo, uint32_t F, int flags,
              cudaStream_t st) {
   bool done = false;
-  if (const int rc = run_prologue(pl, input, lds, output, F, flags, &done, st))
+  if (const int rc = run_prologue(pl, input, lds, output, ldo, F, flags, &done, st))
     return rc;
   if (done)
     return 0;
   if (lds % 4 == 0 && aligned_to(input, 16) && !(flags & NTS_PLAN_COPY_INPUT))
-    return run_gather<float>(pl, input, lds, output, F, flags & NTS_PLAN_OVERWRITE, st);
+    return run_gather<float>(pl, input, lds, output, ldo, F, flags & NTS_PLAN_OVERWRITE,
+                             flags & NTS_PLAN_PAD_OUTPUT, st);
   const uint32_t ld = (F + 3u) & ~3u;
   if (const int rc = ensure_workspace(pl->workspace, pl->workspace_floats, (size_t)pl->gather_rows * ld))
     return rc;
@@ -1095,7 +1131,8 @@
   const unsigned blocks = (unsigned)std::min<uint64_t>((total + 255) / 256, (uint64_t)sm_count() * 32);
   pad_rows_kernel<<<blocks, 256, 0, st>>>(input, lds, pl->workspace, pl->gather_rows, F, ld);
   NTS_LAUNCH_CHECK();
-  return run_gather<float>(pl, pl->workspace, ld, output, F, flags & NTS_PLAN_OVERWRITE, st);
+  return run_gather<float>(pl, pl->workspace, ld, output, ldo, F, flags & NTS_PLAN_OVERWRITE,
+                           flags & NTS_PLAN_PAD_OUTPUT, st);
 }
 
 int to_bf16_rows(const void *src, int dtype, uint32_t lds, void *dst, uint32_t n_rows, uint32_t F, uint32_t ld,
@@ -1116,24 +1153,26 @@
   return 0;
 }
 
-int run_plan_bf16(nts_gather_plan *pl, const void *input, int dtype, uint32_t lds, float *output, uint32_t F,
-                  cudaStream_t st, int flags) {
+int run_plan_bf16(nts_gather_plan *pl, const void *input, int dtype, uint32_t lds, float *output, uint32_t ldo,
+                  uint32_t F, cudaStream_t st, int flags) {
   NTS_ARG_CHECK(dtype == NTS_DTYPE_F32 || dtype == NTS_DTYPE_BF16, "input dtype must be NTS_DTYPE_F32 or NTS_DTYPE_BF16");
   NTS_ARG_CHECK(g_plan_variant == 0, "the TMA row-staging variant (nts_gather_plan_set_variant(1)) gathers FP32 rows only");
   bool done = false;
-  if (const int rc = run_prologue(pl, input, lds, output, F, flags, &done, st))
+  if (const int rc = run_prologue(pl, input, lds, output, ldo, F, flags, &done, st))
     return rc;
   if (done)
     return 0;
   const bool overwrite = flags & NTS_PLAN_OVERWRITE;
   if (dtype == NTS_DTYPE_BF16 && lds % 8 == 0 && aligned_to(input, 16) && !(flags & NTS_PLAN_COPY_INPUT))
-    return run_gather<__nv_bfloat16>(pl, static_cast<const __nv_bfloat16 *>(input), lds, output, F, overwrite, st);
+    return run_gather<__nv_bfloat16>(pl, static_cast<const __nv_bfloat16 *>(input), lds, output, ldo, F, overwrite,
+                                     flags & NTS_PLAN_PAD_OUTPUT, st);
   const uint32_t ld = (F + 7u) & ~7u;
   if (const int rc = ensure_workspace(pl->workspace_bf16, pl->workspace_bf16_elems, (size_t)pl->gather_rows * ld))
     return rc;
   if (const int rc = to_bf16_rows(input, dtype, lds, pl->workspace_bf16, pl->gather_rows, F, ld, st))
     return rc;
-  return run_gather<__nv_bfloat16>(pl, pl->workspace_bf16, ld, output, F, overwrite, st);
+  return run_gather<__nv_bfloat16>(pl, pl->workspace_bf16, ld, output, ldo, F, overwrite, flags & NTS_PLAN_PAD_OUTPUT,
+                                   st);
 }
 
 static int pick_slabs_for_rows(nts_vid_t gather_rows, uint64_t n_edges, nts_vid_t n_rows, uint64_t row_bytes,
@@ -1370,16 +1409,17 @@
   nts_gather_plan *best = build_plan(parts, n_parts, n_rows, gather_rows, 1, 0, 0, st);
   if (!best || (s_max <= 1 && !try_hubs) || n_edges == 0 || feature_size == 0)
     return best;
+  const uint32_t ldo = feature_size;
   float *x = nullptr, *y = nullptr;
   const size_t xb = (size_t)gather_rows * feature_size * (bf16 ? 2 : sizeof(float)),
-               yb = (size_t)n_rows * feature_size * sizeof(float);
+               yb = (size_t)n_rows * ldo * sizeof(float);
   bool ok = cudaMalloc(reinterpret_cast<void **>(&x), xb) == cudaSuccess &&
             cudaMalloc(reinterpret_cast<void **>(&y), yb) == cudaSuccess &&
             cudaMemsetAsync(x, 0, xb, st) == cudaSuccess && cudaMemsetAsync(y, 0, yb, st) == cudaSuccess;
   auto time_plan = [&](nts_gather_plan *pl, float *ms) {
     return time_min_of_two([&] {
-      return bf16 ? run_plan_bf16(pl, x, NTS_DTYPE_BF16, feature_size, y, feature_size, st, run_flags)
-                  : run_plan(pl, x, feature_size, y, feature_size, run_flags, st);
+      return bf16 ? run_plan_bf16(pl, x, NTS_DTYPE_BF16, feature_size, y, ldo, feature_size, st, run_flags)
+                  : run_plan(pl, x, feature_size, y, ldo, feature_size, run_flags, st);
     }, st, ms) == 0;
   };
   float best_ms = 0.f;
@@ -1575,20 +1615,37 @@
   return 0;
 }
 
+int nts_gather_plan_run_ld(nts_gather_plan *pl, const float *input, nts_vid_t input_ld, float *output,
+                           nts_vid_t output_ld, nts_vid_t feature_size, int flags, void *stream) {
+  if (output_ld == 0)
+    output_ld = feature_size;
+  NTS_ARG_CHECK(input_ld >= feature_size, "input row pitch below the feature width");
+  NTS_ARG_CHECK(output_ld >= feature_size, "output row pitch below the feature width");
+  NTS_ARG_CHECK(output != nullptr || feature_size == 0, "null output pointer");
+  NTS_ARG_CHECK(pl != nullptr, "null plan");
+  return run_plan(pl, input, input_ld, output, output_ld, feature_size, flags, as_stream(stream));
+}
+
 int nts_gather_plan_run_ex(nts_gather_plan *pl, const float *input, nts_vid_t input_ld, float *output,
                            nts_vid_t feature_size, int flags, void *stream) {
+  return nts_gather_plan_run_ld(pl, input, input_ld, output, feature_size, feature_size, flags, stream);
+}
+
+int nts_gather_plan_run_bf16_ld(nts_gather_plan *pl, const void *input, int input_dtype, nts_vid_t input_ld,
+                                float *output, nts_vid_t output_ld, nts_vid_t feature_size, int flags, void *stream) {
+  if (output_ld == 0)
+    output_ld = feature_size;
   NTS_ARG_CHECK(input_ld >= feature_size, "input row pitch below the feature width");
+  NTS_ARG_CHECK(output_ld >= feature_size, "output row pitch below the feature width");
   NTS_ARG_CHECK(output != nullptr || feature_size == 0, "null output pointer");
   NTS_ARG_CHECK(pl != nullptr, "null plan");
-  return run_plan(pl, input, input_ld, output, feature_size, flags, as_stream(stream));
+  return run_plan_bf16(pl, input, input_dtype, input_ld, output, output_ld, feature_size, as_stream(stream), flags);
 }
 
 int nts_gather_plan_run_bf16_ex(nts_gather_plan *pl, const void *input, int input_dtype, nts_vid_t input_ld,
                                 float *output, nts_vid_t feature_size, int flags, void *stream) {
-  NTS_ARG_CHECK(input_ld >= feature_size, "input row pitch below the feature width");
-  NTS_ARG_CHECK(output != nullptr || feature_size == 0, "null output pointer");
-  NTS_ARG_CHECK(pl != nullptr, "null plan");
-  return run_plan_bf16(pl, input, input_dtype, input_ld, output, feature_size, as_stream(stream), flags);
+  return nts_gather_plan_run_bf16_ld(pl, input, input_dtype, input_ld, output, feature_size, feature_size, flags,
+                                     stream);
 }
 
 int nts_rows_to_bf16(const void *src, int src_dtype, nts_vid_t lds, void *dst, nts_vid_t n_rows, nts_vid_t feature_size,
diff --git a/neutronstarlite_b200/ops.py b/neutronstarlite_b200/ops.py
--- a/neutronstarlite_b200/ops.py
+++ b/neutronstarlite_b200/ops.py
@@ -45,7 +45,7 @@
 
 
 _DTYPE_CODE = {torch.float32: 0, torch.bfloat16: 1}
-PLAN_OVERWRITE, PLAN_COPY_INPUT = 1, 2
+PLAN_OVERWRITE, PLAN_COPY_INPUT, PLAN_PAD_OUTPUT = 1, 2, 4
 
 
 def _ptr(t):
@@ -141,23 +141,26 @@
         return ((self.slabs,) + ((self.hub_cols, self.hub_rows) if self.hub_cols or self.hub_rows else ())
                 + (("overlap",) if self.overlap else ()))
 
-    def run(self, x, out, gather_dtype=None, accumulate=True):
+    def run(self, x, out, gather_dtype=None, accumulate=True, pad_output=False):
         if not row_pitched(x):
             raise _lib.NtsError("the gathered input must have contiguous rows (unit column stride)")
+        if not row_pitched(out):
+            raise _lib.NtsError("the output must have contiguous rows (unit column stride)")
         F = int(x.shape[1])
         ld = F if x.is_contiguous() else int(x.stride(0))
-        flags = 0 if accumulate else PLAN_OVERWRITE
+        ldo = F if out.is_contiguous() else int(out.stride(0))
+        flags = (0 if accumulate else PLAN_OVERWRITE) | (PLAN_PAD_OUTPUT if pad_output else 0)
         if ld != F and (x.storage_offset() + x.shape[0] * ld) * x.element_size() > x.untyped_storage().nbytes():
             flags |= PLAN_COPY_INPUT
         if _check_gather_dtype(gather_dtype) is not None:
             if x.dtype not in _DTYPE_CODE:
                 raise _lib.NtsError("BF16 gathers take a float32 or bfloat16 input, not %s" % x.dtype)
-            _lib.call("nts_gather_plan_run_bf16_ex", self.handle, _ptr(x), _DTYPE_CODE[x.dtype], ld, _ptr(out), F,
-                      flags, _stream())
+            _lib.call("nts_gather_plan_run_bf16_ld", self.handle, _ptr(x), _DTYPE_CODE[x.dtype], ld, _ptr(out), ldo,
+                      F, flags, _stream())
             return out
         if x.dtype == torch.bfloat16:
             raise _lib.NtsError("a bfloat16 input needs gather_dtype=torch.bfloat16")
-        _lib.call("nts_gather_plan_run_ex", self.handle, _ptr(x), ld, _ptr(out), F, flags, _stream())
+        _lib.call("nts_gather_plan_run_ld", self.handle, _ptr(x), ld, _ptr(out), ldo, F, flags, _stream())
         return out
 
     def bytes(self):
@@ -231,37 +234,56 @@
     return x.contiguous()
 
 
-def gather_by_dst_from_src(chunk, out, x, with_weight=True, gather_dtype=None, accumulate=True):
+def _op_output(chunk, direction, n, F, device, gather_dtype):
+    if F % 4 == 0 or _bf16_plan(chunk, direction, F, True, gather_dtype) is None:
+        return torch.empty((n, F), dtype=torch.float32, device=device), False
+    return torch.empty((n, (F + 3) // 4 * 4), dtype=torch.float32, device=device)[:, :F], True
+
+
+def _plain_call(out, accumulate, launch):
+    if out.is_contiguous():
+        launch(out)
+        return
+    tmp = out.contiguous() if accumulate else torch.empty(out.shape, dtype=out.dtype, device=out.device)
+    launch(tmp)
+    out.copy_(tmp)
+
+
+def gather_by_dst_from_src(chunk, out, x, with_weight=True, gather_dtype=None, accumulate=True, pad_output=False):
     plan = _bf16_plan(chunk, "fwd", x.shape[1], with_weight, gather_dtype)
     ev = _timer.bracket("fwd", x.shape[1], chunk.edge_size, chunk.batch_size_forward) if _timer else None
     if ev:
         ev[0].record()
     if plan is not None:
-        plan.run(x, out, gather_dtype, accumulate)
+        plan.run(x, out, gather_dtype, accumulate, pad_output)
     else:
-        x = _plain_operands(out, x, accumulate)
-        _lib.call("nts_gather_by_dst_from_src", _ptr(x), _ptr(out), _ptr(chunk.edge_weight_forward_gpu),
-                  _ptr(chunk.row_indices_gpu), _ptr(chunk.column_offset_gpu), chunk.src_range[0], chunk.src_range[1],
-                  chunk.dst_range[0], chunk.dst_range[1], chunk.edge_size, chunk.batch_size_forward,
-                  int(x.shape[1]), 1 if with_weight else 0, _stream())
+        def launch(o):
+            xc = _plain_operands(o, x, accumulate)
+            _lib.call("nts_gather_by_dst_from_src", _ptr(xc), _ptr(o), _ptr(chunk.edge_weight_forward_gpu),
+                      _ptr(chunk.row_indices_gpu), _ptr(chunk.column_offset_gpu), chunk.src_range[0],
+                      chunk.src_range[1], chunk.dst_range[0], chunk.dst_range[1], chunk.edge_size,
+                      chunk.batch_size_forward, int(xc.shape[1]), 1 if with_weight else 0, _stream())
+        _plain_call(out, accumulate, launch)
     if ev:
         ev[1].record()
     return out
 
 
-def gather_by_src_from_dst(chunk, out, grad, with_weight=True, gather_dtype=None, accumulate=True):
+def gather_by_src_from_dst(chunk, out, grad, with_weight=True, gather_dtype=None, accumulate=True, pad_output=False):
     plan = _bf16_plan(chunk, "bwd", grad.shape[1], with_weight, gather_dtype)
     ev = _timer.bracket("bwd", grad.shape[1], chunk.edge_size, chunk.batch_size_backward) if _timer else None
     if ev:
         ev[0].record()
     if plan is not None:
-        plan.run(grad, out, gather_dtype, accumulate)
+        plan.run(grad, out, gather_dtype, accumulate, pad_output)
     else:
-        grad = _plain_operands(out, grad, accumulate)
-        _lib.call("nts_gather_by_src_from_dst", _ptr(grad), _ptr(out), _ptr(chunk.edge_weight_backward_gpu),
-                  _ptr(chunk.row_offset_gpu), _ptr(chunk.column_indices_gpu), chunk.src_range[0], chunk.src_range[1],
-                  chunk.dst_range[0], chunk.dst_range[1], chunk.edge_size, chunk.batch_size_backward,
-                  int(grad.shape[1]), 1 if with_weight else 0, _stream())
+        def launch(o):
+            gc = _plain_operands(o, grad, accumulate)
+            _lib.call("nts_gather_by_src_from_dst", _ptr(gc), _ptr(o), _ptr(chunk.edge_weight_backward_gpu),
+                      _ptr(chunk.row_offset_gpu), _ptr(chunk.column_indices_gpu), chunk.src_range[0],
+                      chunk.src_range[1], chunk.dst_range[0], chunk.dst_range[1], chunk.edge_size,
+                      chunk.batch_size_backward, int(gc.shape[1]), 1 if with_weight else 0, _stream())
+        _plain_call(out, accumulate, launch)
     if ev:
         ev[1].record()
     return out
@@ -292,14 +314,14 @@
     def forward(self, f_input, f_input1=None):
         x = _check_gathered(f_input, "input", self.gather_dtype, pitched=True)
         c = self.partitioned_graph_.graph_chunks[0]
-        y = torch.empty((c.batch_size_forward, x.shape[1]), dtype=torch.float32, device=x.device)
-        return gather_by_dst_from_src(c, y, x, gather_dtype=self.gather_dtype, accumulate=False)
+        y, pad = _op_output(c, "fwd", c.batch_size_forward, x.shape[1], x.device, self.gather_dtype)
+        return gather_by_dst_from_src(c, y, x, gather_dtype=self.gather_dtype, accumulate=False, pad_output=pad)
 
     def backward(self, f_output_grad):
         g = _check_input(f_output_grad, "output_grad", pitched=True)
         c = self.partitioned_graph_.graph_chunks[0]
-        dx = torch.empty((c.batch_size_backward, g.shape[1]), dtype=torch.float32, device=g.device)
-        return gather_by_src_from_dst(c, dx, g, gather_dtype=self.gather_dtype, accumulate=False)
+        dx, pad = _op_output(c, "bwd", c.batch_size_backward, g.shape[1], g.device, self.gather_dtype)
+        return gather_by_src_from_dst(c, dx, g, gather_dtype=self.gather_dtype, accumulate=False, pad_output=pad)
 
 
 class MiniBatchFuseOp(ntsGraphOp):
```
